# NVlabs/WarpConvNet

Hardware: AMD Instinct MI355X
Metric: M active voxels/sec fwd+bwd, SparseConv3d 64→128 k=3, 1/2/4/8 MI355X (higher is better)
Workload: dtype bf16; 1 GPU; configs[1]: one 1000000-voxel uniform (U) scene per GPU, SparseConv3d 64->128 k=3, bf16 autocast, kernel-map build + AB fwd + ABt dgrad + AtB wgrad per step; voxels_per_gpu=1000000, coord_order=generator, parallelism=dp1 (scene-sharded, grad all-reduce)

## Files before the change

### include/wcn.h

```cpp
#ifndef WCN_H_
#define WCN_H_

#include <stddef.h>
#include <stdint.h>

#ifdef __cplusplus
extern "C" {
#endif

typedef void* wcn_stream_t;

enum wcn_status {
  WCN_SUCCESS = 0,
  WCN_ERROR_PROBLEM_NOT_SUPPORTED = -1,
  WCN_ERROR_KERNEL_INITIALIZATION = -2,
  WCN_ERROR_KERNEL_EXECUTION = -3,
  WCN_ERROR_UNSUPPORTED_CONFIG = -4,
  WCN_ERROR_INVALID_PARAMETERS = -5,
  WCN_ERROR_MIXED_INPUT_UNSUPPORTED = -6
};

enum wcn_dtype { WCN_F32 = 0, WCN_F16 = 1, WCN_BF16 = 2 };

enum wcn_kmap_flag {
  WCN_FLAG_TABLE_FULL = 1,
  WCN_FLAG_COORD_RANGE = 2,
  WCN_FLAG_PAIR_OVERFLOW = 4,
  WCN_FLAG_DUPLICATE_COORD = 8,
  WCN_FLAG_NEED_STRICT = 16,
  WCN_FLAG_ROW_OVERFLOW = 32
};

int wcn_abi_version(void);
const char* wcn_status_string(int status);

int wcn_hash_prepare(void* slots, int64_t capacity, wcn_stream_t stream);
int wcn_hash_insert(void* slots, int64_t capacity, const int32_t* coords, int64_t n, int32_t* status,
                    wcn_stream_t stream);
int wcn_hash_search(const void* slots, int64_t capacity, const int32_t* queries, int64_t m,
                    int32_t* results, wcn_stream_t stream);

int32_t wcn_kmap_row_pitch(int32_t num_offsets);
int32_t wcn_kmap_mask_words(int32_t num_offsets);
int64_t wcn_kmap_num_blocks(int64_t m);
size_t wcn_kmap_counts_bytes(int64_t m, int32_t num_offsets);

int wcn_kmap_probe(const void* slots, int64_t capacity, const int32_t* query, int64_t m,
                   const int32_t ksize[3], const int32_t stride[3], const int32_t dilation[3],
                   int32_t* nbr, uint32_t* mask, wcn_stream_t stream);
int wcn_batch_indexed_coords(const int32_t* coords, int64_t n, int32_t num_dims, const int32_t* offsets,
                             int32_t num_batches, int32_t* out, wcn_stream_t stream);

int wcn_morton_code(const int32_t* coords, int64_t n, int32_t num_dims, const int32_t* origin, const int32_t axis[3],
                    int64_t* codes, wcn_stream_t stream);

size_t wcn_kmap_binned_workspace(int64_t n, int64_t max_blocks);
int wcn_kmap_binned_supported(const int32_t ksize[3], const int32_t dilation[3]);
int wcn_kmap_compact_supported(int32_t num_offsets);
int wcn_kmap_build_binned(const int32_t* coords, int64_t n, const int32_t ksize[3], const int32_t dilation[3],
                          int64_t max_blocks, int32_t strict, int32_t compact, void* workspace, size_t workspace_bytes,
                          int32_t* nbr, uint32_t* mask, int32_t* status, wcn_stream_t stream);
int wcn_kmap_densify(const int32_t* nbr_compact, int64_t m, int32_t num_offsets, int32_t* nbr, wcn_stream_t stream);
size_t wcn_kmap_tally_sort_workspace(int64_t m);
int wcn_kmap_tally_sort(uint32_t* mask, int32_t* nbr, int64_t m, int32_t num_offsets, int32_t* counts, int32_t* offsets,
                        int32_t* status, int32_t* host_mirror, int32_t* perm, void* sort_workspace,
                        size_t sort_workspace_bytes, const int32_t* coords, void* binned_workspace, int64_t binned_n,
                        int64_t max_blocks, int32_t compact, int32_t* in_maps, int32_t* out_maps, int64_t pair_capacity,
                        wcn_stream_t stream);
int wcn_kmap_count(const uint32_t* mask, int64_t m, int32_t num_offsets, int32_t* counts, wcn_stream_t stream);
int wcn_kmap_scan(int32_t* counts, int64_t num_blocks, int32_t num_offsets, int32_t* offsets,
                  wcn_stream_t stream);
int wcn_kmap_scan_to_host(int32_t* counts, int64_t num_blocks, int32_t num_offsets, int32_t* offsets, const int32_t* status,
                          int32_t* host_mirror, wcn_stream_t stream);
int wcn_kmap_scatter(const int32_t* nbr, const uint32_t* mask, int64_t m, int32_t num_offsets,
                     const int32_t* counts, const int32_t* offsets, int32_t* in_maps, int32_t* out_maps, int64_t pair_capacity,
                     int32_t* status, int32_t compact, wcn_stream_t stream);
int wcn_kmap_cells_build(const int32_t* coords, int64_t n, int64_t max_blocks, void* workspace, size_t workspace_bytes,
                         uint32_t* scratch, int32_t* status, wcn_stream_t stream);
int wcn_cells_stride_supported(const int32_t stride[3]);
int64_t wcn_cells_stride_tiles(int64_t n);
int wcn_cells_stride_count(const void* cells_workspace, int64_t n, int64_t max_blocks, const int32_t* coords,
                           const int32_t stride[3], uint64_t* flags, int32_t* counts, int32_t num_batches,
                           int32_t* out_offsets, wcn_stream_t stream);
int wcn_cells_stride_emit(const void* cells_workspace, int64_t n, int64_t max_blocks, const int32_t* coords,
                          const int32_t stride[3], const uint64_t* flags, const int32_t* counts, int32_t* out_coords,
                          int32_t* first_rows, int32_t* nbr, uint32_t* mask, wcn_stream_t stream);
int wcn_kmap_probe_cells(const void* cells_workspace, int64_t n_in, int64_t max_blocks, const int32_t* query, int64_t m,
                         const int32_t ksize[3], const int32_t stride[3], const int32_t dilation[3], int32_t* nbr,
                         uint32_t* mask, wcn_stream_t stream);
int wcn_kmap_transpose(const int32_t* nbr, int64_t m, int32_t num_offsets, int32_t* pair_table,
                       wcn_stream_t stream);
int wcn_kmap_reverse(const int32_t* in_maps, const int32_t* out_maps, const int32_t* offsets,
                     int32_t num_offsets, int64_t max_pairs, int64_t n_in, int32_t* rev_nbr,
                     uint32_t* rev_mask, wcn_stream_t stream);
int wcn_kmap_from_csr(const int32_t* in_maps, const int32_t* out_maps, const int32_t* offsets,
                      int32_t num_offsets, int64_t max_pairs, int64_t n_out, int32_t* nbr, uint32_t* mask,
                      wcn_stream_t stream);
size_t wcn_mask_argsort_workspace(int64_t n);
int wcn_mask_argsort(const uint32_t* mask, int32_t mask_words, int32_t num_bits, int64_t n, int32_t* perm,
                     void* workspace, size_t workspace_bytes, wcn_stream_t stream);
int wcn_mask_tile_order(const uint32_t* mask, int32_t mask_words, int32_t num_offsets, int64_t n, int32_t* perm,
                        void* workspace, size_t workspace_bytes, wcn_stream_t stream);

enum wcn_algo { WCN_ALGO_AUTO = 0, WCN_ALGO_REF = 1, WCN_ALGO_MFMA = 2 };

int wcn_mfma_gather_supported(int32_t cin, int32_t cout, int32_t num_offsets, int32_t dtype);
int wcn_mfma_wgrad_supported(int32_t cin, int32_t cout, int32_t dtype);
int wcn_conv_identity_supported(int32_t cin, int32_t cout, int32_t dtype);
int wcn_dense_rows_supported(int32_t cin, int32_t cout, int32_t dtype);
int wcn_dense_rows(const void* x, int32_t x_is_f32, const void* w, int32_t w_is_f32, int32_t w_transposed, const float* bias,
                   void* y, int64_t n, int32_t cin, int32_t cout, int32_t dtype, wcn_stream_t stream);

size_t wcn_packed_weight_bytes(int32_t num_offsets, int32_t cin, int32_t cout, int32_t dtype, int32_t transpose);
int wcn_pack_weight(const void* w, int32_t num_offsets, int32_t cin, int32_t cout, int32_t dtype,
                    int32_t transpose, int32_t flip, void* packed, size_t packed_bytes, wcn_stream_t stream);
int wcn_pack_weight_f32(const float* w, int32_t num_offsets, int32_t cin, int32_t cout, int32_t dtype, int32_t transpose,
                        int32_t flip, void* packed, size_t packed_bytes, wcn_stream_t stream);
int wcn_pack_weight_pair_supported(int32_t num_offsets, int32_t cin, int32_t cout, int32_t dtype);
int wcn_pack_weight_f32_pair(const float* w, int32_t num_offsets, int32_t cin, int32_t cout, int32_t dtype, int32_t flip_dgrad,
                             void* packed_fwd, size_t packed_fwd_bytes, void* packed_dgrad, size_t packed_dgrad_bytes,
                             wcn_stream_t stream);

int wcn_conv_compact_table_supported(int32_t cin, int32_t cout, int32_t num_offsets, int32_t dtype);
int wcn_conv_gather_gemm(const void* in, const void* w, void* out, const int32_t* nbr,
                         const uint32_t* mask, const int32_t* perm, const float* bias, int64_t n_in,
                         int64_t n_out, int32_t cin, int32_t cout, int32_t num_offsets, int32_t dtype,
                         int32_t algo, int32_t w_transposed, int32_t k_flip, wcn_stream_t stream);

int wcn_mfma_grouped_supported(int32_t cin_g, int32_t cout_g, int32_t num_offsets, int32_t dtype);
int wcn_pack_weight_grouped(const void* w, int32_t w_is_f32, int32_t num_offsets, int32_t groups, int32_t cin_g,
                            int32_t cout_g, int32_t dtype, int32_t transpose, int32_t flip, void* packed, wcn_stream_t stream);
int wcn_conv_gather_gemm_grouped(const void* in, const void* w_packed, void* out, const int32_t* nbr, const uint32_t* mask,
                                 const int32_t* perm, const float* bias, int64_t n_in, int64_t n_out, int32_t cin_g,
                                 int32_t cout_g, int32_t groups, int32_t num_offsets, int32_t dtype, wcn_stream_t stream);
int wcn_conv_gather_gemm_f32out(const void* in, const void* w_packed, float* out, const int32_t* nbr,
                                const uint32_t* mask, const int32_t* perm, const float* bias, int64_t n_in,
                                int64_t n_out, int32_t cin, int32_t cout, int32_t num_offsets, int32_t dtype,
                                wcn_stream_t stream);

int wcn_conv_gather_gemm_fused(const void* in, const void* w_packed, void* out, const int32_t* nbr, const uint32_t* mask,
                               const int32_t* perm, const float* bias, const float* scale, const float* shift,
                               const void* residual, int32_t relu, int64_t n_in, int64_t n_out, int32_t cin, int32_t cout,
                               int32_t num_offsets, int32_t dtype, wcn_stream_t stream);

size_t wcn_colsum_workspace(int32_t channels);
int wcn_colsum(const void* in, int64_t n, int32_t channels, int32_t dtype, float* out, void* workspace,
               size_t workspace_bytes, wcn_stream_t stream);

size_t wcn_conv_wgrad_workspace(int32_t num_offsets, int32_t cin, int32_t cout, int32_t algo);
int wcn_conv_wgrad(const void* x, const void* dy, float* dw, const int32_t* in_maps,
                   const int32_t* out_maps, const int32_t* offsets, int64_t n_in, int64_t n_out,
                   int32_t cin, int32_t cout, int32_t num_offsets, int32_t dtype, int32_t algo,
                   void* workspace, size_t workspace_bytes, wcn_stream_t stream);

int wcn_mfma_wgrad_bias_supported(int32_t cin, int32_t cout, int32_t dtype);
int wcn_conv_wgrad_bias(const void* x, const void* dy, float* dw, const int32_t* in_maps, const int32_t* out_maps,
                        const int32_t* offsets, int64_t n_in, int64_t n_out, int32_t cin, int32_t cout,
                        int32_t num_offsets, int32_t dtype, int32_t self_offset, float* bias_grad, void* workspace,
                        size_t workspace_bytes, wcn_stream_t stream);

int wcn_dwconv_gather(const void* in, const void* w, void* out, const int32_t* nbr, const float* bias, int64_t n_in,
                      int64_t n_out, int32_t channels, int32_t num_offsets, int32_t dtype, int32_t k_flip,
                      wcn_stream_t stream);
size_t wcn_dwconv_wgrad_workspace(int32_t num_offsets, int32_t channels);
int wcn_dwconv_wgrad(const void* x, const void* dy, float* dw, const int32_t* in_maps, const int32_t* out_maps,
                     const int32_t* offsets, int64_t n_in, int64_t n_out, int32_t channels, int32_t num_offsets,
                     int32_t dtype, void* workspace, size_t workspace_bytes, wcn_stream_t stream);

int wcn_knn_grid(const float* ref_sorted, const int32_t* ref_ids, const int32_t* cell_start, const float origin[3],
                 float cell_size, const int32_t dims[3], const float* query, int64_t num_query, int32_t k,
                 int64_t* out_index, float* out_dist2, wcn_stream_t stream);
int wcn_radius_grid_count(const float* ref_sorted, const int32_t* ref_ids, const int32_t* cell_start, const float origin[3],
                          float cell_size, const int32_t dims[3], const float* query, int64_t num_query, float radius,
                          int32_t* counts, wcn_stream_t stream);
int wcn_radius_grid_write(const float* ref_sorted, const int32_t* ref_ids, const int32_t* cell_start, const float origin[3],
                          float cell_size, const int32_t dims[3], const float* query, int64_t num_query, float radius,
                          const int64_t* splits, int32_t* out_index, float* out_dist, wcn_stream_t stream);
int wcn_segment_reduce(const void* in, const int64_t* row_splits, int64_t num_segments, int32_t channels, int32_t dtype,
                       int32_t op, void* out, int64_t* arg_rows, wcn_stream_t stream);

int wcn_pointconv_supported(int32_t cin, int32_t cq, int32_t nrel, int32_t hidden, int32_t cout, int32_t k,
                            int32_t linear_shortcut);
int64_t wcn_pointconv_packed_floats(int32_t ein, int32_t hidden, int32_t cout);
int64_t wcn_pointconv_grad_floats(int32_t ein, int32_t hidden, int32_t cout, int32_t linear_shortcut);
size_t wcn_pointconv_backward_workspace(int64_t n_query, int32_t k, int32_t ein, int32_t hidden, int32_t cout,
                                        int32_t linear_shortcut);
int wcn_pointconv_pack(const float* w1, const float* b1, const float* g1, const float* be1, const float* w2,
                       const float* b2, const float* g2, const float* be2, const float* ws, const float* bs, int32_t ein,
                       int32_t hidden, int32_t cout, float* packed, wcn_stream_t stream);
int wcn_pointconv_edge_forward(const float* in_feats, const float* q_feats, const float* in_xyz, const float* q_xyz,
                               const int32_t* nbr, int64_t n_query, int32_t k, int32_t cin, int32_t cq, int32_t nrel,
                               const float* packed, int32_t hidden, int32_t cout, float eps1, float eps2, int32_t mean,
                               int32_t linear_shortcut, float* out, wcn_stream_t stream);
int wcn_pointconv_edge_backward(const float* in_feats, const float* q_feats, const float* in_xyz, const float* q_xyz,
                                const int32_t* nbr, int64_t n_query, int32_t k, int32_t cin, int32_t cq, int32_t nrel,
                                const float* packed, int32_t hidden, int32_t cout, float eps1, float eps2, int32_t mean,
                                int32_t linear_shortcut, const float* grad_out, float* d_in, float* d_q, float* d_params,
                                void* workspace, size_t workspace_bytes, wcn_stream_t stream);
int wcn_pointconv_edge_backward_peredge(const float* in_feats, const float* q_feats, const float* in_xyz, const float* q_xyz,
                                        const int32_t* nbr, int64_t n_query, int32_t k, int32_t cin, int32_t cq, int32_t nrel,
                                        const float* packed, int32_t hidden, int32_t cout, float eps1, float eps2, int32_t mean,
                                        int32_t linear_shortcut, const float* grad_out, float* d_edge, float* d_q,
                                        float* d_params, void* workspace, size_t workspace_bytes, wcn_stream_t stream);

int wcn_pointconv_edge_forward_ragged(const float* in_feats, const float* q_feats, const float* in_xyz, const float* q_xyz,
                                      const int32_t* nbr, const int32_t* edge_q, const float* q_scale, int64_t n_edges,
                                      int64_t n_query, int32_t cin, int32_t cq, int32_t nrel, const float* packed,
                                      int32_t hidden, int32_t cout, float eps1, float eps2, int32_t linear_shortcut,
                                      float* out, wcn_stream_t stream);
int wcn_pointconv_edge_backward_ragged(const float* in_feats, const float* q_feats, const float* in_xyz, const float* q_xyz,
                                       const int32_t* nbr, const int32_t* edge_q, const float* q_scale, int64_t n_edges,
                                       int64_t n_query, int32_t cin, int32_t cq, int32_t nrel, const float* packed,
                                       int32_t hidden, int32_t cout, float eps1, float eps2, int32_t linear_shortcut,
                                       const float* grad_out, float* d_in, float* d_q, float* d_params, void* workspace,
                                       size_t workspace_bytes, wcn_stream_t stream);

int wcn_pool_gather(const void* in, const int32_t* tbl, int64_t n_in, int64_t n_out, int32_t channels, int32_t num_offsets,
                    int32_t dtype, int32_t op, void* out, int32_t* arg, int32_t* count, wcn_stream_t stream);
int wcn_pool_select(const void* dy, const int32_t* arg, const int32_t* tbl, int64_t n_in, int64_t n_out, int32_t channels,
                    int32_t num_offsets, int32_t dtype, void* dx, wcn_stream_t stream);

size_t wcn_bn_workspace(int32_t channels);
int wcn_bn_stats_fold(const void* x, int64_t n, int32_t channels, int32_t dtype, const float* gamma, const float* beta,
                      float* running_mean, float* running_var, float momentum, float eps, float* mean, float* var,
                      float* rstd, float* scale, float* shift, int64_t* num_batches_tracked, void* workspace,
                      size_t workspace_bytes, wcn_stream_t stream);
int wcn_bn_fold(const float* running_mean, const float* running_var, const float* gamma, const float* beta, float eps,
                int32_t channels, float* mean, float* rstd, float* scale, float* shift, wcn_stream_t stream);
int wcn_bn_stats(const void* x, int64_t n, int32_t channels, int32_t dtype, float* mean, float* var, void* workspace,
                 size_t workspace_bytes, wcn_stream_t stream);
int wcn_bn_apply(const void* x, int64_t n, int32_t channels, int32_t dtype, const float* scale, const float* shift,
                 int32_t relu, void* y, wcn_stream_t stream);
int wcn_bn_backward_reduce(const void* dy, const void* x, const float* relu_scale, const float* relu_shift, int64_t n,
                           int32_t channels, int32_t dtype, const float* mean, const float* rstd, float* sum_dy,
                           float* sum_dy_xhat, void* workspace, size_t workspace_bytes, wcn_stream_t stream);
int wcn_bn_backward_apply(const void* dy, const void* x, const float* relu_scale, const float* relu_shift, int64_t n,
                          int32_t channels, int32_t dtype, const float* mean, const float* rstd, const float* gamma,
                          const float* sum_dy, const float* sum_dy_xhat, void* dx, wcn_stream_t stream);
int wcn_bn_apply_residual(const void* x, const void* residual, int64_t n, int32_t channels, int32_t dtype, const float* scale,
                          const float* shift, int32_t relu, void* y, wcn_stream_t stream);
int wcn_bn_backward_reduce_masked(const void* dy, const void* x, const void* z, int64_t n, int32_t channels, int32_t dtype,
                                  const float* mean, const float* rstd, float* sum_dy, float* sum_dy_xhat, void* workspace,
                                  size_t workspace_bytes, wcn_stream_t stream);
int wcn_bn_backward_apply_masked(const void* dy, const void* x, const void* z, int64_t n, int32_t channels, int32_t dtype,
                                 const float* mean, const float* rstd, const float* gamma, const float* sum_dy,
                                 const float* sum_dy_xhat, void* dx, void* dres, wcn_stream_t stream);

int wcn_bn_train_forward(const void* x, const void* residual, int64_t n, int32_t channels, int32_t dtype, const float* gamma,
                         const float* beta, float* running_mean, float* running_var, float momentum, float eps,
                         int64_t* num_batches_tracked, int32_t relu, float* stats, void* y, void* workspace,
                         size_t workspace_bytes, wcn_stream_t stream);
int wcn_bn_train_backward(const void* dy, const void* x, const void* z, int32_t relu, int64_t n, int32_t channels, int32_t dtype,
                          const float* stats, const float* gamma, int32_t training, float* sums, void* dx, void* dres,
                          void* workspace, size_t workspace_bytes, wcn_stream_t stream);
int wcn_bn_train_backward_ld(const void* dy, int64_t dy_ld, const void* x, const void* z, int32_t relu, int64_t n, int32_t channels,
                             int32_t dtype, const float* stats, const float* gamma, int32_t training, float* sums, void* dx,
                             void* dres, void* workspace, size_t workspace_bytes, wcn_stream_t stream);

int wcn_conv_bn_backward(const void* grad_out, const void* x, const void* y, const void* z, int32_t relu, const float* stats,
                         const float* gamma, int32_t training, float* sums, void* dy_conv, void* dres, const void* w_packed_dgrad,
                         const int32_t* rev_nbr, const uint32_t* rev_mask, const int32_t* rev_perm, int32_t flip, void* dx,
                         const int32_t* in_maps, const int32_t* out_maps, const int32_t* offsets, float* dw, void* wgrad_workspace,
                         size_t wgrad_workspace_bytes, int64_t n_in, int64_t n_out, int32_t cin, int32_t cout, int32_t num_offsets,
                         int32_t dtype, void* bn_workspace, size_t bn_workspace_bytes, wcn_stream_t stream);
int wcn_conv_bn_backward_ld(const void* grad_out, int64_t grad_out_ld, const void* x, const void* y, const void* z, int32_t relu,
                            const float* stats, const float* gamma, int32_t training, float* sums, void* dy_conv, void* dres,
                            const void* w_packed_dgrad, const int32_t* rev_nbr, const uint32_t* rev_mask, const int32_t* rev_perm,
                            int32_t flip, void* dx, const int32_t* in_maps, const int32_t* out_maps, const int32_t* offsets,
                            float* dw, void* wgrad_workspace, size_t wgrad_workspace_bytes, int64_t n_in, int64_t n_out,
                            int32_t cin, int32_t cout, int32_t num_offsets, int32_t dtype, void* bn_workspace,
                            size_t bn_workspace_bytes, wcn_stream_t stream);

int wcn_attn_varlen_supported(int32_t head_dim, int32_t dtype);
size_t wcn_attn_varlen_workspace_bytes(int64_t total, int32_t heads);
int wcn_attn_varlen_fwd(const void* qkv, const int32_t* cu_seqlens, int64_t num_seqs, int64_t total, int32_t heads,
                        int32_t head_dim, int32_t max_seqlen, float softmax_scale, int32_t dtype, void* out, float* lse,
                        wcn_stream_t stream);
int wcn_attn_varlen_bwd(const void* dout, const void* qkv, const void* out, const float* lse, const int32_t* cu_seqlens,
                        int64_t num_seqs, int64_t total, int32_t heads, int32_t head_dim, int32_t max_seqlen,
                        float softmax_scale, int32_t dtype, void* dqkv, void* workspace, size_t workspace_bytes,
                        wcn_stream_t stream);

int32_t wcn_attn_varlen_kv_splits(int64_t num_seqs, int32_t max_seqlen_q, int32_t max_seqlen_k, int32_t heads);
size_t wcn_attn_varlen_kv_workspace_bytes(int64_t total_q, int64_t total_k, int32_t heads, int32_t head_dim, int32_t q_splits);
int wcn_attn_varlen_kv_fwd(const void* q, int64_t q_stride, const void* k, const void* v, int64_t kv_stride,
                           const int32_t* cu_q, const int32_t* cu_k, int64_t num_seqs, int64_t total_q, int64_t total_k,
                           int32_t heads, int32_t head_dim, int32_t max_seqlen_q, int32_t max_seqlen_k, float softmax_scale,
                           int32_t dtype, void* out, float* lse, wcn_stream_t stream);
int wcn_attn_varlen_kv_bwd(const void* dout, const void* q, int64_t q_stride, const void* k, const void* v, int64_t kv_stride,
                           const void* out, const float* lse, const int32_t* cu_q, const int32_t* cu_k, int64_t num_seqs,
                           int64_t total_q, int64_t total_k, int32_t heads, int32_t head_dim, int32_t max_seqlen_q,
                           int32_t max_seqlen_k, float softmax_scale, int32_t dtype, void* dq, int64_t dq_stride, void* dk,
                           void* dv, int64_t dkv_stride, int32_t q_splits, void* workspace, size_t workspace_bytes,
                           wcn_stream_t stream);

enum wcn_slot_order { WCN_SLOT_X_FASTEST = 0, WCN_SLOT_Z_FASTEST = 1 };
int wcn_resample_pack(const void* src, const int32_t* tbl, int64_t n_src, int64_t n_parent, int32_t channels, int32_t n_per,
                      int32_t factor, int32_t pitch, int32_t slot_order, int32_t dtype, void* dst, wcn_stream_t stream);
int wcn_resample_unpack(const void* src, const int32_t* tbl, int64_t n_parent, int64_t n_dst, int32_t channels, int32_t n_per,
                        int32_t factor, int32_t pitch, int32_t slot_order, int32_t broadcast, int32_t dtype, void* dst,
                        wcn_stream_t stream);
size_t wcn_resample_expand_workspace(int64_t n_parent);
int wcn_resample_expand(const int32_t* parents, const void* mask, int32_t mask_dtype, int64_t n_parent, int32_t n_per,
                        int32_t factor, int32_t slot_order, int32_t num_batches, void* workspace, size_t workspace_bytes,
                        int32_t* out_offsets, int64_t capacity, int32_t* child_coords, int32_t* tbl, int32_t pitch,
                        wcn_stream_t stream);

int wcn_rope_table(const void* coords, int32_t coords_float, int64_t total, const float* origin, float bias,
                   const float* freqs, int32_t num_freqs, float* table, wcn_stream_t stream);
int wcn_qk_prologue_supported(int32_t head_dim, int32_t in_dtype, int32_t out_dtype);
size_t wcn_qk_prologue_workspace_bytes(int64_t total, int32_t heads, int32_t head_dim);
int wcn_qk_prologue_fwd(const void* qkv, int32_t in_dtype, int64_t total, int32_t heads, int32_t head_dim, const float* table,
                        int32_t rot_pairs, int32_t conjugate, const float* gamma_q, const float* gamma_k, void* out,
                        int32_t out_dtype, float* inv_norm, wcn_stream_t stream);
int wcn_qk_prologue_bwd(const void* dout, int32_t dout_dtype, const void* qkv, int32_t in_dtype, int64_t total, int32_t heads,
                        int32_t head_dim, const float* table, int32_t rot_pairs, const float* gamma_q, const float* gamma_k,
                        const float* inv_norm, void* dqkv, float* dgamma_q, float* dgamma_k, void* workspace,
                        size_t workspace_bytes, wcn_stream_t stream);

int wcn_adaln_supported(int32_t channels, int32_t dtype);
size_t wcn_adaln_workspace_bytes(int64_t rows, int64_t num_segs, int32_t channels);
int wcn_adaln_fwd(const void* x, const void* h, const float* gate, const float* shift, const float* scale, int64_t mod_ld,
                  const int32_t* cu, int64_t num_segs, int64_t rows, int32_t channels, float eps, int32_t dtype, void* x1,
                  void* y, float* stats, wcn_stream_t stream);
int wcn_adaln_bwd(const void* dx1, const void* dy, const void* x, const void* h, const float* gate, const float* scale,
                  int64_t mod_ld, const float* stats, const int32_t* cu, int64_t num_segs, int64_t rows, int32_t channels,
                  int32_t dtype, void* dx, void* dh, float* dgate, float* dshift, float* dscale, int64_t dmod_ld,
                  void* workspace, size_t workspace_bytes, wcn_stream_t stream);

int wcn_ln_act_supported(int32_t channels, int32_t dtype);
size_t wcn_ln_act_workspace_bytes(int64_t rows, int32_t channels);
int wcn_ln_act_fwd(const void* x, const float* weight, const float* bias, int64_t rows, int32_t channels, float eps,
                   int32_t act, int32_t dtype, void* y, float* stats, wcn_stream_t stream);
int wcn_ln_act_bwd(const void* dy, const void* x, const float* weight, const float* bias, const float* stats, int64_t rows,
                   int32_t channels, int32_t act, int32_t dtype, void* dx, float* dweight, float* dbias, void* workspace,
                   size_t workspace_bytes, wcn_stream_t stream);
int wcn_channel_spread(const void* x, const void* h, int64_t rows, int32_t cx, int32_t r, float alpha, int32_t dtype,
                       void* out, wcn_stream_t stream);
int wcn_channel_fold(const void* x, const void* h, int64_t rows, int32_t cout, int32_t g, float alpha, int32_t dtype,
                     void* out, wcn_stream_t stream);

int32_t wcn_window_group_max_segment(void);
size_t wcn_window_group_workspace_bytes(int64_t n, int64_t num_bins);
int wcn_window_group(const int32_t* coords, int64_t n, const int32_t* batch_offsets, int32_t num_batches,
                     const int32_t window[3], const int32_t shift[3], const int32_t min_coord[3], const int32_t grid_shape[3],
                     int64_t* codes, int64_t* perm, int64_t* inverse_perm, int32_t* cu_seqlens, int64_t* counts,
                     int32_t* summary, void* workspace, size_t workspace_bytes, wcn_stream_t stream);

int32_t wcn_csr_chunk_rows(void);
int wcn_voxel_keys(const float* points, int64_t n, const int32_t* batch_offsets, int32_t num_batches, float inv_voxel_size,
                   int64_t* keys, int32_t* status, wcn_stream_t stream);
size_t wcn_voxel_map_workspace_bytes(int64_t n);
int wcn_voxel_map(const int64_t* sorted_keys, const int64_t* perm, int64_t n, int32_t num_batches, int64_t* unique_keys,
                  int32_t* unique_coords, int64_t* csr_offsets, int64_t* to_orig, int64_t* to_unique,
                  int32_t* batch_voxel_offsets, int32_t* summary, void* workspace, size_t workspace_bytes,
                  wcn_stream_t stream);
size_t wcn_csr_gather_reduce_workspace_bytes(int64_t nnz, int32_t c, int32_t op);
int wcn_csr_gather_reduce(const void* in, int64_t ld_in, int64_t n_in, const int64_t* indices, const int64_t* offsets,
                          int64_t m, int64_t nnz, int32_t c, int32_t dtype, int32_t op, int64_t max_segment, void* out,
                          int64_t* arg, void* workspace, size_t workspace_bytes, wcn_stream_t stream);
int wcn_row_spread(const void* src, const int64_t* to_orig, int64_t n, int64_t m, int32_t c, const void* skip, int32_t cs,
                   int64_t ld_out, int32_t mode, const int64_t* offsets, const int64_t* arg, int32_t dtype, void* out,
                   wcn_stream_t stream);

int32_t wcn_lattice_chunk_rows(void);
int wcn_hash128_insert(int64_t* table_keys, int32_t* table_values, int64_t capacity, const int32_t* coords, int64_t n,
                       int32_t key_dim, int32_t* status, wcn_stream_t stream);
int wcn_hash128_search(const int64_t* table_keys, const int32_t* table_values, int64_t capacity, const int32_t* queries,
                       const int32_t* offsets, int64_t m, int32_t k, int32_t key_dim, int32_t* out, wcn_stream_t stream);
int wcn_permuto_simplex(const float* positions, int64_t n, int32_t d, const float* scale, int64_t* key_hi, int64_t* key_lo,
                        int32_t* keys, float* bary, int32_t* status, wcn_stream_t stream);
int wcn_grid_corners(const float* positions, int64_t n, int32_t d, int64_t* floors, int64_t* key_hi, int64_t* key_lo,
                     int32_t* keys, float* weights, int32_t* status, wcn_stream_t stream);
size_t wcn_lattice_map_workspace_bytes(int64_t nnz);
int wcn_lattice_map(const int64_t* sorted_hi, const int64_t* sorted_lo, const int64_t* perm, int64_t nnz, int32_t key_dim,
                    int32_t* unique_keys, int64_t* inverse, int64_t* row_offsets, int32_t* summary, void* workspace,
                    size_t workspace_bytes, wcn_stream_t stream);
int64_t wcn_lattice_plan_items(int64_t nnz);
int64_t wcn_lattice_plan_ints(int64_t nnz);
int wcn_lattice_plan(const int64_t* row_offsets, int64_t v, int64_t nnz, int32_t* plan, wcn_stream_t stream);
int wcn_lattice_splat(const float* f, const float* w, const int64_t* row_offsets, const int64_t* row_entries, int64_t v,
                      int64_t nnz, int32_t k, int32_t pitch, float alpha, const int32_t* plan, float* partials, float* out,
                      wcn_stream_t stream);
int wcn_lattice_blur(const float* x, const int32_t* n1, const int32_t* n2, float s0, float s1, float s2, int64_t v,
                     int32_t pitch, float* y, wcn_stream_t stream);
int wcn_lattice_slice(const float* x, const int64_t* idx, const float* w, int64_t n, int32_t k, int64_t v, int32_t pitch,
                      float alpha, float* out, wcn_stream_t stream);

int32_t wcn_lattice_max_grid(void);
int32_t wcn_lattice_row_grid(int64_t rows, int32_t pitch);
int wcn_bilateral_matvec(const int32_t* neighbours, int32_t d, int64_t v, int32_t pitch, float tap_a, float tap_b, float tap_c,
                         const float* nvec, const float* dc, float lam, const float* p, float* spare, float* ap,
                         double* partials, wcn_stream_t stream);
int wcn_bilateral_pcg(const int32_t* neighbours, int32_t d, int64_t v, int32_t pitch, float tap_a, float tap_b, float tap_c,
                      const float* nvec, const float* dc, const float* minv, float lam, const float* tbar, float* y, float* work,
                      double* partials, double* state, int32_t max_iters, double tol, wcn_stream_t stream);
int wcn_bilateral_knn_weights(const float* src_xyz, const float* src_feat, const float* query_xyz, const float* query_feat,
                              const int64_t* nbr, int64_t n, int64_t m, int32_t k, int32_t dx, int32_t df, float sigma_xyz,
                              float sigma_feat, float* weights, wcn_stream_t stream);

#ifdef __cplusplus
}
#endif
#endif
```

### warpconvnet_amd/_lib.py

```python
import ctypes
import os
import subprocess
import threading
from ctypes import c_char_p, c_int, c_int32, c_int64, c_size_t, c_void_p
from typing import Optional

import torch

_CSRC = os.path.join(os.path.dirname(os.path.abspath(__file__)), "csrc")
LIB_PATH = os.environ.get("WARPCONVNET_AMD_LIB") or os.path.join(_CSRC, "libwcn_hip.so")

WCN_F32, WCN_F16, WCN_BF16 = 0, 1, 2
WCN_ALGO_AUTO, WCN_ALGO_REF, WCN_ALGO_MFMA = 0, 1, 2
WCN_FLAG_TABLE_FULL, WCN_FLAG_COORD_RANGE, WCN_FLAG_PAIR_OVERFLOW, WCN_FLAG_DUPLICATE_COORD = 1, 2, 4, 8
WCN_FLAG_NEED_STRICT = 16
WCN_FLAG_ROW_OVERFLOW = 32
WCN_SLOT_X_FASTEST, WCN_SLOT_Z_FASTEST = 0, 1
WCN_MASK_U8 = 3

_I32P = c_void_p
_3I = c_int32 * 3

SIGNATURES = {
    "wcn_abi_version": (c_int, []),
    "wcn_status_string": (c_char_p, [c_int]),
    "wcn_hash_prepare": (c_int, [c_void_p, c_int64, c_void_p]),
    "wcn_hash_insert": (c_int, [c_void_p, c_int64, c_void_p, c_int64, c_void_p, c_void_p]),
    "wcn_hash_search": (c_int, [c_void_p, c_int64, c_void_p, c_int64, c_void_p, c_void_p]),
    "wcn_kmap_row_pitch": (c_int32, [c_int32]),
    "wcn_kmap_mask_words": (c_int32, [c_int32]),
    "wcn_kmap_num_blocks": (c_int64, [c_int64]),
    "wcn_kmap_probe": (
        c_int,
        [c_void_p, c_int64, c_void_p, c_int64, _3I, _3I, _3I, c_void_p, c_void_p, c_void_p],
    ),
    "wcn_batch_indexed_coords": (c_int, [c_void_p, c_int64, c_int32, c_void_p, c_int32, c_void_p, c_void_p]),
    "wcn_bn_workspace": (c_size_t, [c_int32]),
    "wcn_bn_stats": (c_int, [c_void_p, c_int64, c_int32, c_int32, c_void_p, c_void_p, c_void_p, c_size_t, c_void_p]),
    "wcn_bn_stats_fold": (c_int, [c_void_p, c_int64, c_int32, c_int32, c_void_p, c_void_p, c_void_p, c_void_p, ctypes.c_float,
                                  ctypes.c_float, c_void_p, c_void_p, c_void_p, c_void_p, c_void_p, c_void_p, c_void_p, c_size_t,
                                  c_void_p]),
    "wcn_bn_fold": (c_int, [c_void_p, c_void_p, c_void_p, c_void_p, ctypes.c_float, c_int32, c_void_p, c_void_p, c_void_p,
                            c_void_p, c_void_p]),
    "wcn_bn_apply": (c_int, [c_void_p, c_int64, c_int32, c_int32, c_void_p, c_void_p, c_int32, c_void_p, c_void_p]),
    "wcn_bn_backward_reduce": (c_int, [c_void_p, c_void_p, c_void_p, c_void_p, c_int64, c_int32, c_int32, c_void_p, c_void_p,
                                       c_void_p, c_void_p, c_void_p, c_size_t, c_void_p]),
    "wcn_bn_backward_apply": (c_int, [c_void_p, c_void_p, c_void_p, c_void_p, c_int64, c_int32, c_int32, c_void_p, c_void_p,
                                      c_void_p, c_void_p, c_void_p, c_void_p, c_void_p]),
    "wcn_bn_apply_residual": (c_int, [c_void_p, c_void_p, c_int64, c_int32, c_int32, c_void_p, c_void_p, c_int32, c_void_p,
                                      c_void_p]),
    "wcn_bn_backward_reduce_masked": (c_int, [c_void_p, c_void_p, c_void_p, c_int64, c_int32, c_int32, c_void_p, c_void_p,
                                              c_void_p, c_void_p, c_void_p, c_size_t, c_void_p]),
    "wcn_bn_backward_apply_masked": (c_int, [c_void_p, c_void_p, c_void_p, c_int64, c_int32, c_int32, c_void_p, c_void_p,
                                             c_void_p, c_void_p, c_void_p, c_void_p, c_void_p, c_void_p]),
    "wcn_bn_train_forward": (c_int, [c_void_p, c_void_p, c_int64, c_int32, c_int32, c_void_p, c_void_p, c_void_p, c_void_p,
                                     ctypes.c_float, ctypes.c_float, c_void_p, c_int32, c_void_p, c_void_p, c_void_p, c_size_t,
                                     c_void_p]),
    "wcn_bn_train_backward": (c_int, [c_void_p, c_void_p, c_void_p, c_int32, c_int64, c_int32, c_int32, c_void_p, c_void_p,
                                      c_int32, c_void_p, c_void_p, c_void_p, c_void_p, c_size_t, c_void_p]),
    "wcn_bn_train_backward_ld": (c_int, [c_void_p, c_int64, c_void_p, c_void_p, c_int32, c_int64, c_int32, c_int32, c_void_p, c_void_p,
                                         c_int32, c_void_p, c_void_p, c_void_p, c_void_p, c_size_t, c_void_p]),
    "wcn_conv_bn_backward_ld": (c_int, [c_void_p, c_int64, c_void_p, c_void_p, c_void_p, c_int32, c_void_p, c_void_p, c_int32, c_void_p,
                                        c_void_p, c_void_p, c_void_p, c_void_p, c_void_p, c_void_p, c_int32, c_void_p, c_void_p, c_void_p,
                                        c_void_p, c_void_p, c_void_p, c_size_t, c_int64, c_int64, c_int32, c_int32, c_int32, c_int32,
                                        c_void_p, c_size_t, c_void_p]),
    "wcn_conv_bn_backward": (c_int, [c_void_p, c_void_p, c_void_p, c_void_p, c_int32, c_void_p, c_void_p, c_int32, c_void_p, c_void_p,
                                     c_void_p, c_void_p, c_void_p, c_void_p, c_void_p, c_int32, c_void_p, c_void_p, c_void_p, c_void_p,
                                     c_void_p, c_void_p, c_size_t, c_int64, c_int64, c_int32, c_int32, c_int32, c_int32, c_void_p,
                                     c_size_t, c_void_p]),
    "wcn_pool_gather": (c_int, [c_void_p, c_void_p, c_int64, c_int64, c_int32, c_int32, c_int32, c_int32, c_void_p, c_void_p,
                                c_void_p, c_void_p]),
    "wcn_pool_select": (c_int, [c_void_p, c_void_p, c_void_p, c_int64, c_int64, c_int32, c_int32, c_int32, c_void_p, c_void_p]),
    "wcn_morton_code": (c_int, [c_void_p, c_int64, c_int32, c_void_p, c_void_p, c_void_p, c_void_p]),
    "wcn_kmap_counts_bytes": (c_size_t, [c_int64, c_int32]),
    "wcn_kmap_binned_workspace": (c_size_t, [c_int64, c_int64]),
    "wcn_kmap_binned_supported": (c_int, [_3I, _3I]),
    "wcn_kmap_build_binned": (
        c_int,
        [c_void_p, c_int64, _3I, _3I, c_int64, c_int32, c_int32, c_void_p, c_size_t, c_void_p, c_void_p, c_void_p, c_void_p],
    ),
    "wcn_kmap_compact_supported": (c_int, [c_int32]),
    "wcn_kmap_densify": (c_int, [c_void_p, c_int64, c_int32, c_void_p, c_void_p]),
    "wcn_kmap_tally_sort_workspace": (c_size_t, [c_int64]),
    "wcn_kmap_tally_sort": (
        c_int,
        [c_void_p, c_void_p, c_int64, c_int32, c_void_p, c_void_p, c_void_p, c_void_p, c_void_p, c_void_p, c_size_t,
         c_void_p, c_void_p, c_int64, c_int64, c_int32, c_void_p, c_void_p, c_int64, c_void_p],
    ),
    "wcn_kmap_count": (c_int, [c_void_p, c_int64, c_int32, c_void_p, c_void_p]),
    "wcn_kmap_scan": (c_int, [c_void_p, c_int64, c_int32, c_void_p, c_void_p]),
    "wcn_kmap_scan_to_host": (c_int, [c_void_p, c_int64, c_int32, c_void_p, c_void_p, c_void_p, c_void_p]),
    "wcn_kmap_scatter": (
        c_int,
        [c_void_p, c_void_p, c_int64, c_int32, c_void_p, c_void_p, c_void_p, c_void_p, c_int64, c_void_p, c_int32, c_void_p],
    ),
    "wcn_kmap_cells_build": (c_int, [c_void_p, c_int64, c_int64, c_void_p, c_size_t, c_void_p, c_void_p, c_void_p]),
    "wcn_cells_stride_supported": (c_int, [_3I]),
    "wcn_cells_stride_tiles": (c_int64, [c_int64]),
    "wcn_cells_stride_count": (c_int, [c_void_p, c_int64, c_int64, c_void_p, _3I, c_void_p, c_void_p, c_int32, c_void_p,
                                       c_void_p]),
    "wcn_cells_stride_emit": (c_int, [c_void_p, c_int64, c_int64, c_void_p, _3I, c_void_p, c_void_p, c_void_p, c_void_p,
                                      c_void_p, c_void_p, c_void_p]),
    "wcn_kmap_probe_cells": (c_int, [c_void_p, c_int64, c_int64, c_void_p, c_int64, _3I, _3I, _3I, c_void_p, c_void_p,
                                     c_void_p]),
    "wcn_kmap_transpose": (c_int, [c_void_p, c_int64, c_int32, c_void_p, c_void_p]),
    "wcn_kmap_reverse": (
        c_int,
        [c_void_p, c_void_p, c_void_p, c_int32, c_int64, c_int64, c_void_p, c_void_p, c_void_p],
    ),
    "wcn_kmap_from_csr": (
        c_int,
        [c_void_p, c_void_p, c_void_p, c_int32, c_int64, c_int64, c_void_p, c_void_p, c_void_p],
    ),
    "wcn_mask_argsort_workspace": (c_size_t, [c_int64]),
    "wcn_mask_argsort": (c_int, [c_void_p, c_int32, c_int32, c_int64, c_void_p, c_void_p, c_size_t, c_void_p]),
    "wcn_mask_tile_order": (c_int, [c_void_p, c_int32, c_int32, c_int64, c_void_p, c_void_p, c_size_t, c_void_p]),
    "wcn_mfma_gather_supported": (c_int, [c_int32, c_int32, c_int32, c_int32]),
    "wcn_mfma_wgrad_supported": (c_int, [c_int32, c_int32, c_int32]),
    "wcn_conv_identity_supported": (c_int, [c_int32, c_int32, c_int32]),
    "wcn_dense_rows_supported": (c_int, [c_int32, c_int32, c_int32]),
    "wcn_dense_rows": (
        c_int,
        [c_void_p, c_int32, c_void_p, c_int32, c_int32, c_void_p, c_void_p, c_int64, c_int32, c_int32, c_int32, c_void_p],
    ),
    "wcn_packed_weight_bytes": (c_size_t, [c_int32, c_int32, c_int32, c_int32, c_int32]),
    "wcn_pack_weight": (
        c_int,
        [c_void_p, c_int32, c_int32, c_int32, c_int32, c_int32, c_int32, c_void_p, c_size_t, c_void_p],
    ),
    "wcn_pack_weight_f32": (
        c_int,
        [c_void_p, c_int32, c_int32, c_int32, c_int32, c_int32, c_int32, c_void_p, c_size_t, c_void_p],
    ),
    "wcn_pack_weight_pair_supported": (c_int, [c_int32, c_int32, c_int32, c_int32]),
    "wcn_conv_compact_table_supported": (c_int, [c_int32, c_int32, c_int32, c_int32]),
    "wcn_pack_weight_f32_pair": (c_int, [c_void_p, c_int32, c_int32, c_int32, c_int32, c_int32, c_void_p, c_size_t, c_void_p, c_size_t,
                                         c_void_p]),
    "wcn_conv_gather_gemm": (
        c_int,
        [c_void_p, c_void_p, c_void_p, c_void_p, c_void_p, c_void_p, c_void_p, c_int64, c_int64, c_int32, c_int32,
         c_int32, c_int32, c_int32, c_int32, c_int32, c_void_p],
    ),
    "wcn_mfma_grouped_supported": (c_int, [c_int32, c_int32, c_int32, c_int32]),
    "wcn_pack_weight_grouped": (
        c_int,
        [c_void_p, c_int32, c_int32, c_int32, c_int32, c_int32, c_int32, c_int32, c_int32, c_void_p, c_void_p],
    ),
    "wcn_conv_gather_gemm_grouped": (
        c_int,
        [c_void_p, c_void_p, c_void_p, c_void_p, c_void_p, c_void_p, c_void_p, c_int64, c_int64, c_int32, c_int32,
         c_int32, c_int32, c_int32, c_void_p],
    ),
    "wcn_conv_gather_gemm_f32out": (
        c_int,
        [c_void_p, c_void_p, c_void_p, c_void_p, c_void_p, c_void_p, c_void_p, c_int64, c_int64, c_int32, c_int32,
         c_int32, c_int32, c_void_p],
    ),
    "wcn_conv_gather_gemm_fused": (
        c_int,
        [c_void_p, c_void_p, c_void_p, c_void_p, c_void_p, c_void_p, c_void_p, c_void_p, c_void_p, c_void_p, c_int32,
         c_int64, c_int64, c_int32, c_int32, c_int32, c_int32, c_void_p],
    ),
    "wcn_colsum_workspace": (c_size_t, [c_int32]),
    "wcn_colsum": (c_int, [c_void_p, c_int64, c_int32, c_int32, c_void_p, c_void_p, c_size_t, c_void_p]),
    "wcn_conv_wgrad_workspace": (c_size_t, [c_int32, c_int32, c_int32, c_int32]),
    "wcn_conv_wgrad": (
        c_int,
        [c_void_p, c_void_p, c_void_p, c_void_p, c_void_p, c_void_p, c_int64, c_int64, c_int32, c_int32, c_int32,
         c_int32, c_int32, c_void_p, c_size_t, c_void_p],
    ),
    "wcn_dwconv_gather": (
        c_int,
        [c_void_p, c_void_p, c_void_p, c_void_p, c_void_p, c_int64, c_int64, c_int32, c_int32, c_int32, c_int32, c_void_p],
    ),
    "wcn_dwconv_wgrad_workspace": (c_size_t, [c_int32, c_int32]),
    "wcn_dwconv_wgrad": (
        c_int,
        [c_void_p, c_void_p, c_void_p, c_void_p, c_void_p, c_void_p, c_int64, c_int64, c_int32, c_int32, c_int32,
         c_void_p, c_size_t, c_void_p],
    ),
    "wcn_radius_grid_count": (
        c_int,
        [c_void_p, c_void_p, c_void_p, ctypes.c_float * 3, ctypes.c_float, c_int32 * 3, c_void_p, c_int64, ctypes.c_float,
         c_void_p, c_void_p],
    ),
    "wcn_radius_grid_write": (
        c_int,
        [c_void_p, c_void_p, c_void_p, ctypes.c_float * 3, ctypes.c_float, c_int32 * 3, c_void_p, c_int64, ctypes.c_float,
         c_void_p, c_void_p, c_void_p, c_void_p],
    ),
    "wcn_knn_grid": (
        c_int,
        [c_void_p, c_void_p, c_void_p, ctypes.c_float * 3, ctypes.c_float, c_int32 * 3, c_void_p, c_int64, c_int32, c_void_p,
         c_void_p, c_void_p],
    ),
    "wcn_segment_reduce": (c_int, [c_void_p, c_void_p, c_int64, c_int32, c_int32, c_int32, c_void_p, c_void_p, c_void_p]),
    "wcn_pointconv_supported": (c_int, [c_int32] * 7),
    "wcn_pointconv_packed_floats": (c_int64, [c_int32] * 3),
    "wcn_pointconv_grad_floats": (c_int64, [c_int32] * 4),
    "wcn_pointconv_backward_workspace": (c_size_t, [c_int64, c_int32, c_int32, c_int32, c_int32, c_int32]),
    "wcn_pointconv_pack": (c_int, [c_void_p] * 10 + [c_int32] * 3 + [c_void_p, c_void_p]),
    "wcn_pointconv_edge_forward": (
        c_int,
        [c_void_p] * 5 + [c_int64] + [c_int32] * 4 + [c_void_p, c_int32, c_int32, ctypes.c_float, ctypes.c_float, c_int32,
                                                      c_int32, c_void_p, c_void_p],
    ),
    "wcn_pointconv_edge_backward": (
        c_int,
        [c_void_p] * 5 + [c_int64] + [c_int32] * 4 + [c_void_p, c_int32, c_int32, ctypes.c_float, ctypes.c_float, c_int32,
                                                      c_int32, c_void_p, c_void_p, c_void_p, c_void_p, c_void_p, c_size_t,
                                                      c_void_p],
    ),
    "wcn_pointconv_edge_backward_peredge": (
        c_int,
        [c_void_p] * 5 + [c_int64] + [c_int32] * 4 + [c_void_p, c_int32, c_int32, ctypes.c_float, ctypes.c_float, c_int32,
                                                      c_int32, c_void_p, c_void_p, c_void_p, c_void_p, c_void_p, c_size_t,
                                                      c_void_p],
    ),
    "wcn_pointconv_edge_forward_ragged": (
        c_int,
        [c_void_p] * 7 + [c_int64, c_int64] + [c_int32] * 3 + [c_void_p, c_int32, c_int32, ctypes.c_float, ctypes.c_float,
                                                               c_int32, c_void_p, c_void_p],
    ),
    "wcn_pointconv_edge_backward_ragged": (
        c_int,
        [c_void_p] * 7 + [c_int64, c_int64] + [c_int32] * 3 + [c_void_p, c_int32, c_int32, ctypes.c_float, ctypes.c_float,
                                                               c_int32, c_void_p, c_void_p, c_void_p, c_void_p, c_void_p,
                                                               c_size_t, c_void_p],
    ),
    "wcn_attn_varlen_supported": (c_int, [c_int32, c_int32]),
    "wcn_attn_varlen_workspace_bytes": (c_size_t, [c_int64, c_int32]),
    "wcn_attn_varlen_fwd": (
        c_int,
        [c_void_p, c_void_p, c_int64, c_int64, c_int32, c_int32, c_int32, ctypes.c_float, c_int32, c_void_p, c_void_p,
         c_void_p],
    ),
    "wcn_attn_varlen_bwd": (
        c_int,
        [c_void_p, c_void_p, c_void_p, c_void_p, c_void_p, c_int64, c_int64, c_int32, c_int32, c_int32, ctypes.c_float,
         c_int32, c_void_p, c_void_p, c_size_t, c_void_p],
    ),
    "wcn_attn_varlen_kv_splits": (c_int32, [c_int64, c_int32, c_int32, c_int32]),
    "wcn_attn_varlen_kv_workspace_bytes": (c_size_t, [c_int64, c_int64, c_int32, c_int32, c_int32]),
    "wcn_attn_varlen_kv_fwd": (
        c_int,
        [c_void_p, c_int64, c_void_p, c_void_p, c_int64, c_void_p, c_void_p, c_int64, c_int64, c_int64, c_int32, c_int32,
         c_int32, c_int32, ctypes.c_float, c_int32, c_void_p, c_void_p, c_void_p],
    ),
    "wcn_attn_varlen_kv_bwd": (
        c_int,
        [c_void_p, c_void_p, c_int64, c_void_p, c_void_p, c_int64, c_void_p, c_void_p, c_void_p, c_void_p, c_int64, c_int64,
         c_int64, c_int32, c_int32, c_int32, c_int32, ctypes.c_float, c_int32, c_void_p, c_int64, c_void_p, c_void_p, c_int64,
         c_int32, c_void_p, c_size_t, c_void_p],
    ),
    "wcn_rope_table": (c_int, [c_void_p, c_int32, c_int64, c_void_p, ctypes.c_float, c_void_p, c_int32, c_void_p, c_void_p]),
    "wcn_qk_prologue_supported": (c_int, [c_int32, c_int32, c_int32]),
    "wcn_qk_prologue_workspace_bytes": (c_size_t, [c_int64, c_int32, c_int32]),
    "wcn_qk_prologue_fwd": (
        c_int,
        [c_void_p, c_int32, c_int64, c_int32, c_int32, c_void_p, c_int32, c_int32, c_void_p, c_void_p, c_void_p, c_int32,
         c_void_p, c_void_p],
    ),
    "wcn_qk_prologue_bwd": (
        c_int,
        [c_void_p, c_int32, c_void_p, c_int32, c_int64, c_int32, c_int32, c_void_p, c_int32, c_void_p, c_void_p, c_void_p,
         c_void_p, c_void_p, c_void_p, c_void_p, c_size_t, c_void_p],
    ),
    "wcn_adaln_supported": (c_int, [c_int32, c_int32]),
    "wcn_adaln_workspace_bytes": (c_size_t, [c_int64, c_int64, c_int32]),
    "wcn_adaln_fwd": (
        c_int,
        [c_void_p] * 5 + [c_int64, c_void_p, c_int64, c_int64, c_int32, ctypes.c_float, c_int32, c_void_p, c_void_p, c_void_p,
                          c_void_p],
    ),
    "wcn_adaln_bwd": (
        c_int,
        [c_void_p] * 6 + [c_int64, c_void_p, c_void_p, c_int64, c_int64, c_int32, c_int32] + [c_void_p] * 5 +
        [c_int64, c_void_p, c_size_t, c_void_p],
    ),
    "wcn_ln_act_supported": (c_int, [c_int32, c_int32]),
    "wcn_ln_act_workspace_bytes": (c_size_t, [c_int64, c_int32]),
    "wcn_ln_act_fwd": (c_int, [c_void_p] * 3 + [c_int64, c_int32, ctypes.c_float, c_int32, c_int32, c_void_p, c_void_p,
                                                 c_void_p]),
    "wcn_ln_act_bwd": (c_int, [c_void_p] * 5 + [c_int64, c_int32, c_int32, c_int32] + [c_void_p] * 4 + [c_size_t, c_void_p]),
    "wcn_channel_spread": (c_int, [c_void_p, c_void_p, c_int64, c_int32, c_int32, ctypes.c_float, c_int32, c_void_p,
                                   c_void_p]),
    "wcn_channel_fold": (c_int, [c_void_p, c_void_p, c_int64, c_int32, c_int32, ctypes.c_float, c_int32, c_void_p, c_void_p]),
    "wcn_window_group_max_segment": (c_int32, []),
    "wcn_window_group_workspace_bytes": (c_size_t, [c_int64, c_int64]),
    "wcn_window_group": (c_int, [c_void_p, c_int64, c_void_p, c_int32, _3I, _3I, _3I, _3I] + [c_void_p] * 7 +
                         [c_size_t, c_void_p]),
    "wcn_csr_chunk_rows": (c_int32, []),
    "wcn_voxel_keys": (c_int, [c_void_p, c_int64, c_void_p, c_int32, ctypes.c_float, c_void_p, c_void_p, c_void_p]),
    "wcn_voxel_map_workspace_bytes": (c_size_t, [c_int64]),
    "wcn_voxel_map": (c_int, [c_void_p, c_void_p, c_int64, c_int32] + [c_void_p] * 7 + [c_void_p, c_size_t, c_void_p]),
    "wcn_csr_gather_reduce_workspace_bytes": (c_size_t, [c_int64, c_int32, c_int32]),
    "wcn_csr_gather_reduce": (
        c_int,
        [c_void_p, c_int64, c_int64, c_void_p, c_void_p, c_int64, c_int64, c_int32, c_int32, c_int32, c_int64, c_void_p,
         c_void_p, c_void_p, c_size_t, c_void_p],
    ),
    "wcn_row_spread": (c_int, [c_void_p, c_void_p, c_int64, c_int64, c_int32, c_void_p, c_int32, c_int64, c_int32, c_void_p,
                               c_void_p, c_int32, c_void_p, c_void_p]),
    "wcn_resample_pack": (c_int, [c_void_p, c_void_p, c_int64, c_int64, c_int32, c_int32, c_int32, c_int32, c_int32, c_int32,
                                  c_void_p, c_void_p]),
    "wcn_resample_unpack": (c_int, [c_void_p, c_void_p, c_int64, c_int64, c_int32, c_int32, c_int32, c_int32, c_int32, c_int32,
                                    c_int32, c_void_p, c_void_p]),
    "wcn_resample_expand_workspace": (c_size_t, [c_int64]),
    "wcn_resample_expand": (c_int, [c_void_p, c_void_p, c_int32, c_int64, c_int32, c_int32, c_int32, c_int32, c_void_p, c_size_t,
                                    c_void_p, c_int64, c_void_p, c_void_p, c_int32, c_void_p]),
    "wcn_mfma_wgrad_bias_supported": (c_int, [c_int32, c_int32, c_int32]),
    "wcn_conv_wgrad_bias": (
        c_int,
        [c_void_p, c_void_p, c_void_p, c_void_p, c_void_p, c_void_p, c_int64, c_int64, c_int32, c_int32, c_int32,
         c_int32, c_int32, c_void_p, c_void_p, c_size_t, c_void_p],
    ),
    "wcn_lattice_chunk_rows": (c_int32, []),
    "wcn_hash128_insert": (c_int, [c_void_p, c_void_p, c_int64, c_void_p, c_int64, c_int32, c_void_p, c_void_p]),
    "wcn_hash128_search": (c_int, [c_void_p, c_void_p, c_int64, c_void_p, c_void_p, c_int64, c_int32, c_int32, c_void_p,
                                   c_void_p]),
    "wcn_permuto_simplex": (c_int, [c_void_p, c_int64, c_int32, ctypes.c_float * 6] + [c_void_p] * 6),
    "wcn_grid_corners": (c_int, [c_void_p, c_int64, c_int32] + [c_void_p] * 7),
    "wcn_lattice_map_workspace_bytes": (c_size_t, [c_int64]),
    "wcn_lattice_map": (c_int, [c_void_p, c_void_p, c_void_p, c_int64, c_int32] + [c_void_p] * 5 + [c_size_t, c_void_p]),
    "wcn_lattice_plan_items": (c_int64, [c_int64]),
    "wcn_lattice_plan_ints": (c_int64, [c_int64]),
    "wcn_lattice_plan": (c_int, [c_void_p, c_int64, c_int64, c_void_p, c_void_p]),
    "wcn_lattice_splat": (c_int, [c_void_p] * 4 + [c_int64, c_int64, c_int32, c_int32, ctypes.c_float] + [c_void_p] * 4),
    "wcn_lattice_blur": (c_int, [c_void_p] * 3 + [ctypes.c_float] * 3 + [c_int64, c_int32, c_void_p, c_void_p]),
    "wcn_lattice_slice": (c_int, [c_void_p] * 3 + [c_int64, c_int32, c_int64, c_int32, ctypes.c_float, c_void_p, c_void_p]),
    "wcn_lattice_max_grid": (c_int32, []),
    "wcn_lattice_row_grid": (c_int32, [c_int64, c_int32]),
    "wcn_bilateral_matvec": (c_int, [c_void_p, c_int32, c_int64, c_int32] + [ctypes.c_float] * 3 + [c_void_p, c_void_p,
                                                                                                   ctypes.c_float] + [c_void_p] * 5),
    "wcn_bilateral_pcg": (c_int, [c_void_p, c_int32, c_int64, c_int32] + [ctypes.c_float] * 3 + [c_void_p] * 3 + [ctypes.c_float] +
                          [c_void_p] * 5 + [c_int32, ctypes.c_double, c_void_p]),
    "wcn_bilateral_knn_weights": (c_int, [c_void_p] * 5 + [c_int64, c_int64, c_int32, c_int32, c_int32, ctypes.c_float,
                                                           ctypes.c_float, c_void_p, c_void_p]),
}

_LIB = None


class _GuardedLib:

    def __init__(self, handle: ctypes.CDLL):
        self._h = handle

    def __getattr__(self, name):
        fn = getattr(self._h, name)
        argtypes = fn.argtypes or []
        if not argtypes or argtypes[-1] is not c_void_p or name in _HOST_ONLY or _single_gpu():
            setattr(self, name, fn)
            return fn

        def guarded(*args, _fn=fn):
            dev = getattr(_CALL_DEVICE, "dev", None)
            if dev is None or dev == torch.cuda.current_device():
                return _fn(*args)
            with torch.cuda.device(dev):
                return _fn(*args)

        guarded.__name__ = name
        setattr(self, name, guarded)
        return guarded


def _single_gpu() -> bool:
    try:
        return torch.cuda.is_available() and torch.cuda.device_count() == 1
    except Exception:
        return False


_HOST_ONLY = {"wcn_status_string"}
_CALL_DEVICE = threading.local()


def build(verbose: bool = False) -> str:
    cmd = ["make", "-C", _CSRC, "-j", str(min(8, os.cpu_count() or 1))]
    res = subprocess.run(cmd, capture_output=True, text=True)
    if res.returncode != 0:
        raise RuntimeError(f"building libwcn_hip.so failed:\n{res.stdout[-4000:]}\n{res.stderr[-4000:]}")
    if verbose:
        print(res.stdout[-2000:])
    return LIB_PATH


def lib() -> ctypes.CDLL:
    global _LIB
    if _LIB is None:
        if not os.path.exists(LIB_PATH):
            raise RuntimeError(
                f"{LIB_PATH} not found: the HIP extension is not built. Run "
                "`python -c 'import __graft_entry__ as g; g.build()'` (or `make -C warpconvnet_amd/csrc`). "
                "There is no CPU fallback for the HIP paths."
            )
        handle = ctypes.CDLL(LIB_PATH)
        for name, (restype, argtypes) in SIGNATURES.items():
            fn = getattr(handle, name)
            fn.restype = restype
            fn.argtypes = argtypes
        _LIB = _GuardedLib(handle)
    return _LIB


def status_string(code: int) -> str:
    return lib().wcn_status_string(int(code)).decode()


def check(code: int, what: str) -> None:
    if code != 0:
        raise RuntimeError(f"{what} error: {status_string(code)} ({code})")


def ptr(t: Optional[torch.Tensor]) -> Optional[int]:
    if t is None:
        return None
    return t.data_ptr()


_RAW_STREAM = getattr(torch._C, "_cuda_getCurrentRawStream", None)


def stream_handle(device: torch.device) -> int:
    idx = device.index
    if idx is None:
        idx = torch.cuda.current_device()
    _CALL_DEVICE.dev = idx
    if _RAW_STREAM is not None:
        return _RAW_STREAM(idx)
    return torch.cuda.current_stream(device).cuda_stream


def dtype_code(dtype: torch.dtype) -> int:
    if dtype == torch.float32:
        return WCN_F32
    if dtype == torch.float16:
        return WCN_F16
    if dtype == torch.bfloat16:
        return WCN_BF16
    raise TypeError(f"unsupported feature dtype {dtype} (supported: float32, float16, bfloat16)")


def torch_dtype(code: int) -> torch.dtype:
    return {WCN_F32: torch.float32, WCN_F16: torch.float16, WCN_BF16: torch.bfloat16}[code]


def i3(v) -> "ctypes.Array":
    return _3I(int(v[0]), int(v[1]), int(v[2]))


def require_gpu_tensor(t: torch.Tensor, name: str) -> None:
    if not t.is_cuda:
        raise RuntimeError(f"{name} must live on a GPU for the HIP path (got {t.device}); there is no CPU fallback")
    if not t.is_contiguous():
        raise RuntimeError(f"{name} must be contiguous")
```

### warpconvnet_amd/csrc/kmap.hip

```cpp
#include "kmap_cells.h"

namespace wcn {

constexpr int kBlockRows = 256;
constexpr int kThreads = 256;

__global__ void hash_prepare_kernel(uint4* __restrict__ slots, int64_t capacity) {
  const int64_t i = (int64_t)blockIdx.x * blockDim.x + threadIdx.x;
  if (i < capacity) slots[i] = make_uint4(0u, 0u, 0xFFFFFFFFu, 0u);
}

__global__ void hash_insert_kernel(Slot* __restrict__ slots, uint32_t capacity_mask, const int4* __restrict__ coords,
                                   int64_t n, int32_t* __restrict__ status) {
  const int64_t i = (int64_t)blockIdx.x * blockDim.x + threadIdx.x;
  if (i >= n) return;
  const int4 c = coords[i];
  if (!coord_in_range(c.x, c.y, c.z, c.w)) {
    atomicOr(status, (int)WCN_FLAG_COORD_RANGE);
    return;
  }
  const uint64_t key = pack_key(c.x, c.y, c.z, c.w);
  uint32_t s = hash_slot(key, capacity_mask);
  for (uint32_t attempts = 0; attempts <= capacity_mask; ++attempts) {
    unsigned long long* kp = reinterpret_cast<unsigned long long*>(&slots[s].key);
    const unsigned long long prev = atomicCAS(kp, 0ull, (unsigned long long)key);
    if (prev == 0ull || prev == key) {
      atomicMin(reinterpret_cast<unsigned int*>(&slots[s].value), (unsigned int)i);
      if (prev == key) atomicOr(status, (int)WCN_FLAG_DUPLICATE_COORD);
      return;
    }
    s = (s + 1) & capacity_mask;
  }
  atomicOr(status, (int)WCN_FLAG_TABLE_FULL);
}

__global__ void hash_search_kernel(const Slot* __restrict__ slots, uint32_t capacity_mask,
                                   const int4* __restrict__ queries, int64_t m, int32_t* __restrict__ results) {
  const int64_t i = (int64_t)blockIdx.x * blockDim.x + threadIdx.x;
  if (i >= m) return;
  const int4 q = queries[i];
  results[i] = slot_lookup(slots, capacity_mask, pack_key(q.x, q.y, q.z, q.w));
}

struct HashLookup {
  const Slot* slots;
  uint32_t cmask;
  __device__ __forceinline__ int operator()(int b, int x, int y, int z) const {
    return slot_lookup(slots, cmask, pack_key(b, x, y, z));
  }
};

struct CellLookup {
  const BSlot* slots;
  uint32_t cmask;
  CellTable t;
  __device__ __forceinline__ int operator()(int b, int x, int y, int z) const {
    const int xx = (x << (32 - kCoordBits)) >> (32 - kCoordBits);
    const int yy = (y << (32 - kCoordBits)) >> (32 - kCoordBits);
    const int zz = (z << (32 - kCoordBits)) >> (32 - kCoordBits);
    const int id = block_id_of(slots, cmask, make_int4(b, xx, yy, zz));
    int found = -1;
    if (id >= 0)
      found = t.cells[(int64_t)id * kCells + (((xx & (kBlk - 1)) * kBlk + (yy & (kBlk - 1))) * kBlk + (zz & (kBlk - 1)))];
    return found;
  }
};

template <int LPR, typename Lookup>
__global__ __launch_bounds__(kThreads) void kmap_probe_kernel(Lookup lookup, const int4* __restrict__ query, int64_t m,
                                                              KernelGeom g, int K, int kp, int mw, int32_t* __restrict__ nbr,
                                                              uint32_t* __restrict__ mask) {
  const int tid = threadIdx.x;
  constexpr int kRowsPerIter = 64 / LPR;
  const int lane = tid & 63;
  const int wave = tid >> 6;
  const int sub = lane % LPR;
  const int rsel = lane / LPR;
  const int64_t wave_row0 = (int64_t)blockIdx.x * kBlockRows + wave * 64;
  const int num_chunks = (kp + LPR - 1) / LPR;

  for (int kc = 0; kc < num_chunks; ++kc) {
    const int k = kc * LPR + sub;
    const bool k_real = k < K;
    const bool k_store = k < kp;
    const int l = k % g.kz;
    const int j = (k / g.kz) % g.ky;
    const int i = k / (g.kz * g.ky);
    const int ox = (i - g.cx) * g.dx, oy = (j - g.cy) * g.dy, oz = (l - g.cz) * g.dz;
#pragma unroll 4
    for (int it = 0; it < 64 / kRowsPerIter; ++it) {
      const int64_t row = wave_row0 + it * kRowsPerIter + rsel;
      int found = -1;
      if (row < m && k_real) {
        const int4 q = query[row];
        found = lookup(q.x, q.y * g.sx + ox, q.z * g.sy + oy, q.w * g.sz + oz);
      }
      if (row < m && k_store) nbr[row * kp + k] = found;
      const unsigned long long ball = __ballot(found >= 0);
      if (row < m && sub == 0) {
        const unsigned long long bits = (LPR == 64) ? ball : ((ball >> (rsel * LPR)) & ((1ull << (LPR & 63)) - 1ull));
        const int w0 = (kc * LPR) >> 5;
        if (w0 < mw) mask[row * mw + w0] = (uint32_t)bits;
        if (LPR == 64 && w0 + 1 < mw) mask[row * mw + w0 + 1] = (uint32_t)(bits >> 32);
      }
    }
  }
}

template <typename Lookup>
static int launch_probe(const Lookup& lookup, const void* table, const int32_t* query, int64_t m, const int32_t ksize[3],
                        const int32_t stride[3], const int32_t dilation[3], int32_t* nbr, uint32_t* mask, hipStream_t s) {
  if (m < 0 || !ksize || !stride || !dilation) return WCN_ERROR_INVALID_PARAMETERS;
  for (int d = 0; d < 3; ++d)
    if (ksize[d] < 1 || stride[d] < 1 || dilation[d] < 1) return WCN_ERROR_INVALID_PARAMETERS;
  const int64_t K64 = (int64_t)ksize[0] * ksize[1] * ksize[2];
  if (!valid_k(K64)) return WCN_ERROR_PROBLEM_NOT_SUPPORTED;
  if (m == 0) return WCN_SUCCESS;
  if (!table || !query || !nbr || !mask) return WCN_ERROR_INVALID_PARAMETERS;
  const int K = (int)K64, kp = wcn_kmap_row_pitch(K), mw = wcn_kmap_mask_words(K);
  const KernelGeom g = make_kernel_geom(ksize, stride, dilation);
  const dim3 grid((unsigned)ceil_div(m, kBlockRows)), block(kThreads);
#define WCN_PROBE(L) \
  hipLaunchKernelGGL((kmap_probe_kernel<L, Lookup>), grid, block, 0, s, lookup, (const int4*)query, m, g, K, kp, mw, nbr, mask)
  switch (lanes_per_row(kp)) {
    case 8: WCN_PROBE(8); break;
    case 16: WCN_PROBE(16); break;
    case 32: WCN_PROBE(32); break;
    default: WCN_PROBE(64); break;
  }
#undef WCN_PROBE
  return launch_status();
}

__global__ __launch_bounds__(256) void batch_indexed_coords_kernel(const int32_t* __restrict__ coords, int64_t n, int d,
                                                                   const int32_t* __restrict__ offsets, int num_batches,
                                                                   int32_t* __restrict__ out) {
  const int64_t i = (int64_t)blockIdx.x * blockDim.x + threadIdx.x;
  if (i >= n) return;
  const int b = last_offset_not_above(offsets, num_batches, i);
  if (d == 3) {
    const int32_t* c = coords + i * 3;
    *reinterpret_cast<int4*>(out + i * 4) = make_int4(b, c[0], c[1], c[2]);
  } else {
    out[i * (d + 1)] = b;
    for (int j = 0; j < d; ++j) out[i * (d + 1) + 1 + j] = coords[i * d + j];
  }
}

__device__ __forceinline__ uint64_t spread3(uint64_t v) {
  v &= 0x1FFFFFull;
  v = (v | (v << 32)) & 0x001F00000000FFFFull;
  v = (v | (v << 16)) & 0x001F0000FF0000FFull;
  v = (v | (v << 8)) & 0x100F00F00F00F00Full;
  v = (v | (v << 4)) & 0x10C30C30C30C30C3ull;
  v = (v | (v << 2)) & 0x1249249249249249ull;
  return v;
}

__global__ __launch_bounds__(256) void morton_code_kernel(const int32_t* __restrict__ coords, int64_t n, int d,
                                                          const int32_t* __restrict__ origin, int a0, int a1, int a2,
                                                          int64_t* __restrict__ codes) {
  const int64_t i = (int64_t)blockIdx.x * blockDim.x + threadIdx.x;
  if (i >= n) return;
  const int32_t* c = coords + i * d;
  const int sp = d - 3;
  int64_t v[3];
  const int ax[3] = {a0, a1, a2};
#pragma unroll
  for (int j = 0; j < 3; ++j) v[j] = (int64_t)c[sp + ax[j]] - (origin ? (int64_t)origin[sp + ax[j]] : 0);
  uint64_t m = spread3((uint64_t)v[0]) | (spread3((uint64_t)v[1]) << 1) | (spread3((uint64_t)v[2]) << 2);
  if (d == 4) {
    const int64_t b = (int64_t)c[0] - (origin ? (int64_t)origin[0] : 0);
    m = (m & 0x0000FFFFFFFFFFFFull) | ((uint64_t)b << 48);
  }
  codes[i] = (int64_t)m;
}

__global__ __launch_bounds__(kThreads) void kmap_transpose_kernel(const int32_t* __restrict__ nbr, int64_t m, int K,
                                                                  int kp, int tr, int32_t* __restrict__ pair_table) {
  extern __shared__ int s_tile[];
  const int64_t row0 = (int64_t)blockIdx.x * tr;
  const int pitch = kp + 1;
  for (int e = threadIdx.x; e < tr * kp; e += kThreads) {
    const int r = e / kp, k = e % kp;
    s_tile[r * pitch + k] = (row0 + r < m) ? nbr[(row0 + r) * kp + k] : -1;
  }
  __syncthreads();
  for (int e = threadIdx.x; e < tr * K; e += kThreads) {
    const int k = e / tr, r = e % tr;
    if (row0 + r < m) pair_table[(int64_t)k * m + row0 + r] = s_tile[r * pitch + k];
  }
}

__global__ void fill_i32_kernel(int32_t* __restrict__ p, int64_t n, int32_t v) {
  const int64_t i = (int64_t)blockIdx.x * blockDim.x + threadIdx.x;
  if (i < n) p[i] = v;
}

__global__ void kmap_pairs_to_table_kernel(const int32_t* __restrict__ in_maps, const int32_t* __restrict__ out_maps,
                                           const int32_t* __restrict__ offsets, int K, int kp, int mw, int64_t max_pairs,
                                           int by_in, int32_t* __restrict__ tbl, uint32_t* __restrict__ mask) {
  const int64_t p = (int64_t)blockIdx.x * blockDim.x + threadIdx.x;
  if (p >= max_pairs || p >= offsets[K]) return;
  const int k = last_offset_not_above(offsets, K, p);
  const int i = in_maps[p], o = out_maps[p];
  const int64_t row = by_in ? i : o;
  tbl[row * kp + k] = by_in ? o : i;
  atomicOr(&mask[row * mw + (k >> 5)], 1u << (k & 31));
}

}

using namespace wcn;

extern "C" {

int wcn_abi_version(void) { return 14; }

const char* wcn_status_string(int status) {
  switch (status) {
    case WCN_SUCCESS: return "Success";
    case WCN_ERROR_PROBLEM_NOT_SUPPORTED: return "Problem size not supported";
    case WCN_ERROR_KERNEL_INITIALIZATION: return "Kernel initialization failed";
    case WCN_ERROR_KERNEL_EXECUTION: return "Kernel execution failed";
    case WCN_ERROR_UNSUPPORTED_CONFIG: return "Unsupported precision/configuration";
    case WCN_ERROR_INVALID_PARAMETERS: return "Invalid parameters";
    case WCN_ERROR_MIXED_INPUT_UNSUPPORTED: return "Mixed input precision unsupported";
    default: return "Unknown error";
  }
}

static inline bool is_pow2(int64_t v) { return v > 0 && (v & (v - 1)) == 0; }

int wcn_hash_prepare(void* slots, int64_t capacity, wcn_stream_t stream) {
  if (!slots || !is_pow2(capacity) || capacity > (1ll << 31)) return WCN_ERROR_INVALID_PARAMETERS;
  hipLaunchKernelGGL(hash_prepare_kernel, dim3((unsigned)ceil_div(capacity, 256)), dim3(256), 0, (hipStream_t)stream,
                     (uint4*)slots, capacity);
  return launch_status();
}

int wcn_hash_insert(void* slots, int64_t capacity, const int32_t* coords, int64_t n, int32_t* status,
                    wcn_stream_t stream) {
  if (!slots || !is_pow2(capacity) || capacity > (1ll << 31) || n < 0 || !status) return WCN_ERROR_INVALID_PARAMETERS;
  if (n == 0) return WCN_SUCCESS;
  if (!coords) return WCN_ERROR_INVALID_PARAMETERS;
  hipLaunchKernelGGL(hash_insert_kernel, dim3((unsigned)ceil_div(n, 256)), dim3(256), 0, (hipStream_t)stream,
                     (Slot*)slots, (uint32_t)(capacity - 1), (const int4*)coords, n, status);
  return launch_status();
}

int wcn_hash_search(const void* slots, int64_t capacity, const int32_t* queries, int64_t m, int32_t* results,
                    wcn_stream_t stream) {
  if (!slots || !is_pow2(capacity) || m < 0) return WCN_ERROR_INVALID_PARAMETERS;
  if (m == 0) return WCN_SUCCESS;
  if (!queries || !results) return WCN_ERROR_INVALID_PARAMETERS;
  hipLaunchKernelGGL(hash_search_kernel, dim3((unsigned)ceil_div(m, 256)), dim3(256), 0, (hipStream_t)stream,
                     (const Slot*)slots, (uint32_t)(capacity - 1), (const int4*)queries, m, results);
  return launch_status();
}

int32_t wcn_kmap_row_pitch(int32_t num_offsets) { return (num_offsets + 7) & ~7; }
int32_t wcn_kmap_mask_words(int32_t num_offsets) { return (num_offsets + 31) / 32; }
int wcn_kmap_probe(const void* slots, int64_t capacity, const int32_t* query, int64_t m, const int32_t ksize[3],
                   const int32_t stride[3], const int32_t dilation[3], int32_t* nbr, uint32_t* mask,
                   wcn_stream_t stream) {
  if (!slots || !is_pow2(capacity)) return WCN_ERROR_INVALID_PARAMETERS;
  return launch_probe(HashLookup{(const Slot*)slots, (uint32_t)(capacity - 1)}, slots, query, m, ksize, stride, dilation, nbr,
                      mask, (hipStream_t)stream);
}

int wcn_kmap_probe_cells(const void* cells_workspace, int64_t n_in, int64_t max_blocks, const int32_t* query, int64_t m,
                         const int32_t ksize[3], const int32_t stride[3], const int32_t dilation[3], int32_t* nbr,
                         uint32_t* mask, wcn_stream_t stream) {
  if (n_in < 0 || max_blocks < 1) return WCN_ERROR_INVALID_PARAMETERS;
  const CellTable t = carve_cells(const_cast<void*>(cells_workspace), n_in, max_blocks);
  return launch_probe(CellLookup{t.slots, (uint32_t)(t.capacity - 1), t}, cells_workspace, query, m, ksize, stride, dilation,
                      nbr, mask, (hipStream_t)stream);
}

int wcn_batch_indexed_coords(const int32_t* coords, int64_t n, int32_t num_dims, const int32_t* offsets,
                             int32_t num_batches, int32_t* out, wcn_stream_t stream) {
  if (n < 0 || num_dims < 1 || num_dims > 8 || num_batches < 1) return WCN_ERROR_INVALID_PARAMETERS;
  if (n == 0) return WCN_SUCCESS;
  if (!coords || !out || (num_batches > 1 && !offsets)) return WCN_ERROR_INVALID_PARAMETERS;
  hipLaunchKernelGGL(batch_indexed_coords_kernel, dim3((unsigned)ceil_div(n, 256)), dim3(256), 0, (hipStream_t)stream, coords,
                     n, (int)num_dims, offsets, (int)num_batches, out);
  return launch_status();
}

int wcn_morton_code(const int32_t* coords, int64_t n, int32_t num_dims, const int32_t* origin, const int32_t axis[3],
                    int64_t* codes, wcn_stream_t stream) {
  if (n < 0 || (num_dims != 3 && num_dims != 4) || !axis) return WCN_ERROR_INVALID_PARAMETERS;
  int seen = 0;
  for (int j = 0; j < 3; ++j) {
    if (axis[j] < 0 || axis[j] > 2) return WCN_ERROR_INVALID_PARAMETERS;
    seen |= 1 << axis[j];
  }
  if (seen != 7) return WCN_ERROR_INVALID_PARAMETERS;
  if (n == 0) return WCN_SUCCESS;
  if (!coords || !codes) return WCN_ERROR_INVALID_PARAMETERS;
  hipLaunchKernelGGL(morton_code_kernel, dim3((unsigned)ceil_div(n, 256)), dim3(256), 0, (hipStream_t)stream, coords, n,
                     (int)num_dims, origin, (int)axis[0], (int)axis[1], (int)axis[2], codes);
  return launch_status();
}

int wcn_kmap_transpose(const int32_t* nbr, int64_t m, int32_t num_offsets, int32_t* pair_table, wcn_stream_t stream) {
  if (m < 0 || !valid_k(num_offsets)) return WCN_ERROR_INVALID_PARAMETERS;
  if (m == 0) return WCN_SUCCESS;
  if (!nbr || !pair_table) return WCN_ERROR_INVALID_PARAMETERS;
  const int kp = wcn_kmap_row_pitch(num_offsets);
  int tr = 64;
  while (tr > 1 && (size_t)tr * (kp + 1) * sizeof(int) > 64 * 1024) tr >>= 1;
  hipLaunchKernelGGL(kmap_transpose_kernel, dim3((unsigned)ceil_div(m, tr)), dim3(kThreads),
                     (size_t)tr * (kp + 1) * sizeof(int), (hipStream_t)stream, nbr, m, (int)num_offsets, kp, tr, pair_table);
  return launch_status();
}

static int pairs_to_table(const int32_t* in_maps, const int32_t* out_maps, const int32_t* offsets, int32_t K,
                          int64_t max_pairs, int64_t rows, int by_in, int32_t* tbl, uint32_t* mask, hipStream_t s) {
  if (!valid_k(K) || rows < 0 || max_pairs < 0 || !offsets) return WCN_ERROR_INVALID_PARAMETERS;
  if (rows == 0) return WCN_SUCCESS;
  if (!tbl || !mask) return WCN_ERROR_INVALID_PARAMETERS;
  const int kp = wcn_kmap_row_pitch(K), mw = wcn_kmap_mask_words(K);
  hipLaunchKernelGGL(fill_i32_kernel, dim3((unsigned)ceil_div(rows * kp, 256)), dim3(256), 0, s, tbl, rows * kp, -1);
  hipLaunchKernelGGL(fill_i32_kernel, dim3((unsigned)ceil_div(rows * mw, 256)), dim3(256), 0, s, (int32_t*)mask,
                     rows * mw, 0);
  if (max_pairs > 0) {
    if (!in_maps || !out_maps) return WCN_ERROR_INVALID_PARAMETERS;
    hipLaunchKernelGGL(kmap_pairs_to_table_kernel, dim3((unsigned)ceil_div(max_pairs, 256)), dim3(256), 0, s, in_maps,
                       out_maps, offsets, (int)K, kp, mw, max_pairs, by_in, tbl, mask);
  }
  return launch_status();
}

int wcn_kmap_reverse(const int32_t* in_maps, const int32_t* out_maps, const int32_t* offsets, int32_t num_offsets,
                     int64_t max_pairs, int64_t n_in, int32_t* rev_nbr, uint32_t* rev_mask, wcn_stream_t stream) {
  return pairs_to_table(in_maps, out_maps, offsets, num_offsets, max_pairs, n_in, 1, rev_nbr, rev_mask,
                        (hipStream_t)stream);
}

int wcn_kmap_from_csr(const int32_t* in_maps, const int32_t* out_maps, const int32_t* offsets, int32_t num_offsets,
                      int64_t max_pairs, int64_t n_out, int32_t* nbr, uint32_t* mask, wcn_stream_t stream) {
  return pairs_to_table(in_maps, out_maps, offsets, num_offsets, max_pairs, n_out, 0, nbr, mask, (hipStream_t)stream);
}

}
```

### warpconvnet_amd/csrc/kmap_binned.hip

```cpp
#include "kmap_cells.h"

namespace wcn {

constexpr int kInsertSample = 8;
constexpr int kInsertThreads = 512;
constexpr int kRowBufPitch = 66;
constexpr int kRowBufInts = (kCompactPitch + 1) * kRowBufPitch;
#ifndef WCN_NB_WPE
#define WCN_NB_WPE 3
#endif
constexpr int kNbWavesPerSimd = WCN_NB_WPE;
constexpr int kNbThreads = 256;

__device__ __forceinline__ int wrap_blk(int v) {
  const int bits = kBlkCoordBits;
  v &= (1 << bits) - 1;
  return (v ^ (1 << (bits - 1))) - (1 << (bits - 1));
}

__global__ void cell_prepare_kernel(uint4* __restrict__ slots, int64_t capacity, int32_t* __restrict__ ctr,
                                    uint32_t* __restrict__ halo, CellGeom g, int32_t* __restrict__ status) {
  const int64_t i = (int64_t)blockIdx.x * blockDim.x + threadIdx.x;
  if (i < capacity) slots[i] = make_uint4(0u, 0u, 0xFFFFFFFFu, 0u);
  if (i < 64) ctr[i] = 0;
  if (i == 0) *status = 0;
  if (i < g.halo_cells) {
    const int h3[3] = {g.hx, g.hy, g.hz};
    int t = (int)i, dir = 0;
    int sx = 0, sy = 0, sz = 0;
    for (; dir < 27; ++dir) {
      if (dir == 13) continue;
      const int dd[3] = {dir / 9 - 1, (dir / 3) % 3 - 1, dir % 3 - 1};
      sx = dd[0] ? h3[0] : kBlk; sy = dd[1] ? h3[1] : kBlk; sz = dd[2] ? h3[2] : kBlk;
      const int cells = sx * sy * sz;
      if (t < cells) break;
      t -= cells;
    }
    const int ddx = dir / 9 - 1, ddy = (dir / 3) % 3 - 1, ddz = dir % 3 - 1;
    const int tz = t % sz, ty = (t / sz) % sy, tx = t / (sz * sy);
    const int lx = ddx < 0 ? kBlk - g.hx + tx : tx;
    const int ly = ddy < 0 ? kBlk - g.hy + ty : ty;
    const int lz = ddz < 0 ? kBlk - g.hz + tz : tz;
    const int X = lx + kBlk * ddx + g.hx, Y = ly + kBlk * ddy + g.hy, Z = lz + kBlk * ddz + g.hz;
    halo[i] = ((uint32_t)dir << 27) | ((uint32_t)cell_index(lx, ly, lz) << 16) | (uint32_t)(X * g.px + Y * g.py + Z);
  }
}

__device__ __forceinline__ void store_cell(int32_t* cell, int row, bool strict) {
  if (strict) __hip_atomic_fetch_min(reinterpret_cast<uint32_t*>(cell), (uint32_t)row, __ATOMIC_RELAXED, __HIP_MEMORY_SCOPE_AGENT);
  else *cell = row;
}

template <int PHASE>
__global__ __launch_bounds__(kInsertThreads) void cell_insert_kernel(BSlot* __restrict__ slots, uint32_t cmask,
                                                          const int4* __restrict__ coords, int64_t n, CellTable t,
                                                          int32_t* __restrict__ status, int kp, int mw,
                                                          int32_t* __restrict__ nbr, uint32_t* __restrict__ mask,
                                                          int strict) {
  const bool compact = kp < 0;
  kp &= 0x7FFFFFFF;
  const int64_t tid = (int64_t)blockIdx.x * blockDim.x + threadIdx.x;
  const int64_t i = PHASE == 0 ? tid * kInsertSample : tid;
  const int lane = threadIdx.x & 63;
  bool live = i < n;
  int4 c = make_int4(0, 0, 0, 0);
  if (live) {
    c = coords[i];
    if (!coord_in_range(c.x, c.y, c.z, c.w)) {
      live = false;
      if (PHASE == 1) {
        atomicOr(status, (int)WCN_FLAG_COORD_RANGE);
        for (int k = 0; k < kp; ++k) nbr[i * kp + k] = compact ? 0 : -1;
        for (int w = 0; w < mw; ++w) mask[i * mw + w] = 0u;
      }
    }
  }
  int found = -1;
  int id = -1;
  bool created = false;
  uint64_t key = 0;
  if (live) {
    key = pack_key(c.x, c.y >> kBlkShift, c.z >> kBlkShift, c.w >> kBlkShift);
    uint32_t s = hash_slot(key, cmask);
    int idv = -1;
    for (uint32_t a = 0; a <= cmask; ++a) {
      unsigned long long* kptr = reinterpret_cast<unsigned long long*>(&slots[s].key);
      const uint4 v = *reinterpret_cast<const uint4*>(slots + s);
      unsigned long long cur = ((unsigned long long)v.y << 32) | v.x;
      if (cur == key) { found = (int)s; idv = (int)v.z; break; }
      if (cur == 0ull) {
        if (PHASE == 1) cur = __hip_atomic_load(kptr, __ATOMIC_RELAXED, __HIP_MEMORY_SCOPE_AGENT);
        if (cur == 0ull) {
          cur = atomicCAS(kptr, 0ull, (unsigned long long)key);
          if (cur == 0ull) {
            created = true;
            found = (int)s;
            break;
          }
        }
        if (cur == key) { found = (int)s; break; }
      }
      s = (s + 1) & cmask;
    }
    if (found < 0) atomicOr(status, (int)WCN_FLAG_TABLE_FULL);
    if (PHASE == 1 && idv >= 0 && !(idv & kIdLateBit)) id = idv;
  }
  __shared__ int s_made[kInsertThreads / 64 + 1];
  const int wave = threadIdx.x >> 6;
  const unsigned long long makers = __ballot(created);
  if (PHASE == 0) {
    if (lane == 0) s_made[wave] = __popcll(makers);
    __syncthreads();
    if (threadIdx.x == 0) {
      int tot = 0;
      for (int w = 0; w < kInsertThreads / 64; ++w) {
        const int c = s_made[w];
        s_made[w] = tot;
        tot += c;
      }
      s_made[kInsertThreads / 64] = tot > 0 ? atomicAdd(&t.ctr[0], tot) : 0;
    }
    __syncthreads();
  }
  if (makers != 0ull) {
    int base;
    if (PHASE == 0) {
      base = s_made[kInsertThreads / 64] + s_made[wave];
    } else {
      const int leader = __ffsll((long long)makers) - 1;
      base = 0;
      if (lane == leader) base = atomicAdd(&t.ctr[0], __popcll(makers));
      base = __shfl(base, leader);
    }
    int my_id = base + __popcll(makers & ((1ull << lane) - 1ull));
    if (!created) my_id = -1;
    if (my_id >= t.max_blocks) {
      atomicOr(status, (int)WCN_FLAG_TABLE_FULL);
      my_id = -1;
    }
    if (my_id >= 0) {
      t.blk_key[my_id] = key;
      slots[found].id = my_id | (PHASE == 1 ? kIdLateBit : 0);
    }
    unsigned long long todo = makers;
    while (todo != 0ull) {
      const int src = __ffsll((long long)todo) - 1;
      todo &= todo - 1ull;
      const int bid = __shfl(my_id, src);
      if (bid >= 0) {
        int4* gcells = reinterpret_cast<int4*>(t.cells + (int64_t)bid * kCells);
        gcells[lane] = make_int4(-1, -1, -1, -1);
        gcells[lane + 64] = make_int4(-1, -1, -1, -1);
      }
    }
  }
  if (PHASE == 0) return;
  if (live) mask[i * mw + (mw - 1)] = (id >= 0 || found < 0) ? kMaskUnwritten : kMaskDeferred;
  if (id >= 0) store_cell(t.cells + (int64_t)id * kCells + cell_of(c), (int)i, strict != 0);
}

__global__ __launch_bounds__(256) void cell_finish_kernel(const BSlot* __restrict__ slots, uint32_t cmask,
                                                          const int4* __restrict__ coords, int64_t n, CellTable t,
                                                          CellGeom g, int mw, const uint32_t* __restrict__ mask,
                                                          int strict) {
  const int64_t tid = (int64_t)blockIdx.x * blockDim.x + threadIdx.x;
  const int64_t nthreads = (int64_t)gridDim.x * blockDim.x;
  for (int64_t i = tid; i < n; i += nthreads) {
    if (mask[i * mw + (mw - 1)] != kMaskDeferred) continue;
    const int4 c = coords[i];
    const int id = block_id_of(slots, cmask, c);
    if (id < 0) continue;
    store_cell(t.cells + (int64_t)id * kCells + cell_of(c), (int)i, strict != 0);
  }
  const int lane = threadIdx.x & 63;
  int nblocks = t.ctr[0];
  if (nblocks > t.max_blocks) nblocks = (int)t.max_blocks;
  for (int64_t seq = tid >> 6; seq < nblocks; seq += nthreads >> 6) {
    const int id = (int)seq;
    int nid = -1;
    if (lane < 27) {
      const int ddx = lane / 9 - 1, ddy = (lane / 3) % 3 - 1, ddz = lane % 3 - 1;
      const bool needed = (ddx == 0 || g.hx > 0) && (ddy == 0 || g.hy > 0) && (ddz == 0 || g.hz > 0);
      if (lane == 13) nid = id;
      else if (needed) {
        const uint64_t key = t.blk_key[id];
        const int b = (int)((key >> 54) & kBatchMask);
        const int bx = wrap_blk((int)((key >> 36) & kCoordMask));
        const int by = wrap_blk((int)((key >> 18) & kCoordMask));
        const int bz = wrap_blk((int)(key & kCoordMask));
        const int s = block_find(slots, cmask, pack_key(b, wrap_blk(bx + ddx), wrap_blk(by + ddy), wrap_blk(bz + ddz)));
        if (s >= 0) {
          nid = slots[s].id;
          if (nid >= 0) nid &= ~kIdLateBit;
        }
      }
    }
    if (lane < 32) t.nbtab[(int64_t)id * 32 + lane] = nid;
  }
}

#ifdef WCN_PROF
__device__ unsigned long long g_bprof[4096 * 12];
#define BSTAMP(i) do { const unsigned long long now_ = wall_clock64(); prof_acc[i] += now_ - prof_prev; prof_prev = now_; } while (0)
#else
#define BSTAMP(i)
#endif

template <int LPR, bool FAST, bool COMPACT>
__global__ __launch_bounds__(kNbThreads) __attribute__((amdgpu_waves_per_eu(kNbWavesPerSimd))) void cell_neighbors_kernel(CellTable t, const uint32_t* __restrict__ halo,
                                                                    CellGeom g, int K, int kp, int mw,
                                                                    int32_t* __restrict__ nbr,
                                                                    uint32_t* __restrict__ mask,
                                                                    int32_t* __restrict__ status) {
  extern __shared__ int s_mem[];
  const int lane = threadIdx.x & 63, wave = threadIdx.x >> 6;
  uint32_t* s_halo = reinterpret_cast<uint32_t*>(s_mem);
  const int rounds = (g.halo_cells + 63) >> 6;
  const bool halo_regs = COMPACT && rounds <= 8;
  const int halo_pad = halo_regs ? 0 : rounds * 64;
  const int per_wave = g.cells + 4 + kCells / 2 + 8 + (COMPACT ? kRowBufInts : 0);
  int* s_grid = s_mem + halo_pad + wave * per_wave;
  unsigned short* s_own = reinterpret_cast<unsigned short*>(s_grid + g.cells + 4);
  const int null_cell = g.cells;
  for (int h = threadIdx.x; h < halo_pad; h += blockDim.x) s_halo[h] = h < g.halo_cells ? halo[h] : 0xFFFFFFFFu;
  if (lane == 0) s_grid[null_cell] = -1;
  __syncthreads();

  int nblocks = t.ctr[0];
  if (nblocks > t.max_blocks) nblocks = (int)t.max_blocks;
  const int gwave = blockIdx.x * (blockDim.x / 64) + wave;
  const int nwaves = gridDim.x * (blockDim.x / 64);
  constexpr int kVoxPerIter = 64 / LPR;
  const int sub = lane % LPR, vsel = lane / LPR;
  const int num_chunks = (kp + LPR - 1) / LPR;
  uint32_t he[8];
#pragma unroll
  for (int u = 0; u < 8; ++u) {
    const int idx = u * 64 + lane;
    uint32_t e = COMPACT && idx < g.halo_cells ? halo[idx] : 0xFFFFFFFFu;
    if (e == 0xFFFFFFFFu) e = (31u << 27) | (uint32_t)(g.cells + 1);
    he[u] = e;
  }
  auto load_head = [&](int seq, int& nb, int4& v0, int4& v1) {
    nb = -1;
    v0 = make_int4(-1, -1, -1, -1);
    v1 = v0;
    if (seq < nblocks) {
      if (lane < 27) nb = t.nbtab[(int64_t)seq * 32 + lane];
      const int4* own = reinterpret_cast<const int4*>(t.cells + (int64_t)seq * kCells) + lane * 2;
      v0 = own[0];
      v1 = own[1];
    }
  };
  int seq = gwave;
  int nb_c, nb_n;
  int4 c0, c1, n0, n1;
  load_head(seq, nb_c, c0, c1);
  load_head(seq + nwaves, nb_n, n0, n1);
  int hv[8];
  auto gather = [&](int nb, int r0) {
#pragma unroll
    for (int u = 0; u < 8; ++u) {
      hv[u] = -1;
      if (r0 + u < rounds) {
        const uint32_t e = s_halo[(r0 + u) * 64 + lane];
        const int nid = __shfl(nb, (int)((e >> 27) & 31u));
        if (e != 0xFFFFFFFFu && nid >= 0) hv[u] = t.cells[(int64_t)nid * kCells + ((e >> 16) & (kCells - 1))];
      }
    }
  };
  int nidv[8];
  auto gather8 = [&](int nb) {
#pragma unroll
    for (int u = 0; u < 8; ++u) nidv[u] = __shfl(nb, (int)(he[u] >> 27));
#pragma unroll
    for (int u = 0; u < 8; ++u)
      if (u < rounds) {
        const int safe = nidv[u] < 0 ? 0 : nidv[u];
        hv[u] = t.cells[(int64_t)safe * kCells + ((he[u] >> 16) & (kCells - 1))];
      }
  };
  auto scatter8 = [&]() {
#pragma unroll
    for (int u = 0; u < 8; ++u)
      if (u < rounds) s_grid[he[u] & 0xFFFFu] = nidv[u] >= 0 ? hv[u] : -1;
  };
  auto scatter_halo = [&](int r0) {
#pragma unroll
    for (int u = 0; u < 8; ++u)
      if (r0 + u < rounds) {
        const uint32_t e = s_halo[(r0 + u) * 64 + lane];
        if (e != 0xFFFFFFFFu) s_grid[e & 0xFFFFu] = hv[u];
      }
  };
  int* s_rows = s_grid + g.cells + 4 + kCells / 2 + 8;
  int pend_row = -1;
  auto flush_rows = [&](int row) {
    __builtin_amdgcn_fence(__ATOMIC_RELEASE, "wavefront");
    __builtin_amdgcn_wave_barrier();
    if (row >= 0) mask[row] = (uint32_t)s_rows[lane];
    const int piece = lane & 3;
    int rid[4];
    int4 v[4];
#pragma unroll
    for (int q = 0; q < 4; ++q) rid[q] = __shfl(row, (lane >> 2) + 16 * q);
#pragma unroll
    for (int q = 0; q < 4; ++q) {
      const int r = (lane >> 2) + 16 * q;
      v[q].x = s_rows[(piece * 4 + 0) * kRowBufPitch + r];
      v[q].y = s_rows[(piece * 4 + 1) * kRowBufPitch + r];
      v[q].z = s_rows[(piece * 4 + 2) * kRowBufPitch + r];
      v[q].w = s_rows[(piece * 4 + 3) * kRowBufPitch + r];
    }
#pragma unroll
    for (int q = 0; q < 4; ++q)
      if (rid[q] >= 0 && __popc((uint32_t)s_rows[(lane >> 2) + 16 * q]) >= 4 * piece) {
        if (FAST)
          *reinterpret_cast<int4*>(reinterpret_cast<char*>(nbr) + (__umul24((uint32_t)rid[q], kCompactPitch * 4u) + (uint32_t)piece * 16u)) = v[q];
        else
          *reinterpret_cast<int4*>(nbr + (int64_t)rid[q] * kCompactPitch + piece * 4) = v[q];
      }
    __builtin_amdgcn_fence(__ATOMIC_ACQUIRE, "wavefront");
    __builtin_amdgcn_wave_barrier();
  };
#ifdef WCN_PROF
  if (lane == 0 && gwave < 4096) g_bprof[gwave * 12 + 9] = wall_clock64();
#endif
  if (seq < nblocks) {
    if (halo_regs) gather8(nb_c);
    else gather(nb_c, 0);
  }
#ifdef WCN_PROF
  unsigned long long prof_prev = wall_clock64(), prof_acc[8] = {0, 0, 0, 0, 0, 0, 0, 0}, prof_blocks = 0;
  const unsigned long long prof_loop0 = prof_prev;
#endif
  for (; seq < nblocks; seq += nwaves) {
    BSTAMP(0);
#ifdef WCN_PROF
    ++prof_blocks;
#endif
    if (halo_regs) scatter8();
    else scatter_halo(0);
    for (int r0 = 8; r0 < rounds; r0 += 8) {
      gather(nb_c, r0);
      scatter_halo(r0);
    }
    BSTAMP(1);
    const int vals[8] = {c0.x, c0.y, c0.z, c0.w, c1.x, c1.y, c1.z, c1.w};
    const int cell0 = ((lane >> 3) + g.hx) * g.px + ((lane & 7) + g.hy) * g.py + g.hz;
    int mine = 0;
#pragma unroll
    for (int z = 0; z < 8; ++z) {
      s_grid[cell0 + z] = vals[z];
      mine += vals[z] >= 0;
    }
    int incl = mine;
#pragma unroll
    for (int d = 1; d < 64; d <<= 1) {
      const int up = __shfl_up(incl, d);
      if (lane >= d) incl += up;
    }
    const int own_cnt = __shfl(incl, 63);
    int at = incl - mine;
#pragma unroll
    for (int z = 0; z < 8; ++z)
      if (vals[z] >= 0) s_own[at++] = (unsigned short)((cell0 + z) * 4);
    if (lane < 2 * kVoxPerIter) s_own[own_cnt + lane] = (unsigned short)(null_cell * 4);
    BSTAMP(4);
    if (COMPACT) {
      flush_rows(pend_row);
      pend_row = -1;
    }
    BSTAMP(5);
    nb_c = nb_n; c0 = n0; c1 = n1;
    if (seq + nwaves < nblocks) {
      if (halo_regs) gather8(nb_c);
      else gather(nb_c, 0);
    }
    BSTAMP(6);
    load_head(seq + 2 * nwaves, nb_n, n0, n1);
    __builtin_amdgcn_fence(__ATOMIC_RELEASE, "wavefront");
    __builtin_amdgcn_wave_barrier();
    BSTAMP(2);
    const char* grid_bytes = reinterpret_cast<const char*>(s_grid);
    if (COMPACT) {
      int delta_lane = 0;
      if (lane < K) {
        const int l = lane % g.kz, j = (lane / g.kz) % g.ky, i = lane / (g.kz * g.ky);
        delta_lane = ((i - g.cx) * g.dx * g.px + (j - g.cy) * g.dy * g.py + (l - g.cz) * g.dz) * 4;
      }
      bool over = false;
      char* rows_bytes = reinterpret_cast<char*>(s_rows);
      const int origin4 = (g.hx * g.px + g.hy * g.py + g.hz) * 4;
      const uint32_t wp0 = (uint32_t)(kRowBufPitch + lane) * 4u, wp_max = (uint32_t)(kCompactPitch * kRowBufPitch + lane) * 4u;
      for (int e0 = 0; e0 < own_cnt; e0 += 64) {
        const bool live = e0 + lane < own_cnt;
        const int cell = live ? (int)s_own[e0 + lane] : origin4;
        const int row = live ? *reinterpret_cast<const int*>(grid_bytes + cell) : -1;
        uint32_t wp = wp0, rev = 0;
        auto answer = [&](int f) {
          *reinterpret_cast<int*>(rows_bytes + wp) = f;
          const uint32_t h = f >= 0 ? 1u : 0u;
          rev = (rev << 1) | h;
          wp = min(wp + h * (uint32_t)(kRowBufPitch * 4), wp_max);
        };
        int k = 0;
        for (; k + 4 <= K; k += 4) {
          int f[4];
#pragma unroll
          for (int u = 0; u < 4; ++u)
            f[u] = *reinterpret_cast<const int*>(grid_bytes + cell + __builtin_amdgcn_readlane(delta_lane, k + u));
#pragma unroll
          for (int u = 0; u < 4; ++u) answer(f[u]);
        }
        for (; k < K; ++k) answer(*reinterpret_cast<const int*>(grid_bytes + cell + __builtin_amdgcn_readlane(delta_lane, k)));
        const uint32_t m = __brev(rev) >> (32 - K);
        over = over || (live && __popc(m) > kCompactIds);
        s_rows[lane] = (int)m;
        if (e0 + 64 < own_cnt) flush_rows(row);
        else pend_row = row;
      }
      if (__any(over) && lane == 0) atomicOr(status, (int)WCN_FLAG_ROW_OVERFLOW);
    } else
    for (int kc = 0; kc < num_chunks; ++kc) {
      const int k = kc * LPR + sub;
      const bool k_real = k < K, k_store = k < kp;
      const int l = k % g.kz, j = (k / g.kz) % g.ky, i = k / (g.kz * g.ky);
      const int ox = (i - g.cx) * g.dx, oy = (j - g.cy) * g.dy, oz = (l - g.cz) * g.dz;
      const int delta4 = k_real ? (ox * g.px + oy * g.py + oz) * 4 : 0;
      const int w0 = (kc * LPR) >> 5;
      for (int e0 = 0; e0 < own_cnt; e0 += 2 * kVoxPerIter) {
        const int cell_a = s_own[e0 + vsel], cell_b = s_own[e0 + kVoxPerIter + vsel];
        const int row_a = *reinterpret_cast<const int*>(grid_bytes + cell_a);
        const int row_b = *reinterpret_cast<const int*>(grid_bytes + cell_b);
        int found_a = *reinterpret_cast<const int*>(grid_bytes + cell_a + delta4);
        int found_b = *reinterpret_cast<const int*>(grid_bytes + cell_b + delta4);
        if (!k_real) { found_a = -1; found_b = -1; }
        const unsigned long long ball_a = __ballot(found_a >= 0), ball_b = __ballot(found_b >= 0);
        uint32_t bits_a, bits_b, hi_a = 0, hi_b = 0;
        if (LPR == 64) {
          bits_a = (uint32_t)ball_a; hi_a = (uint32_t)(ball_a >> 32);
          bits_b = (uint32_t)ball_b; hi_b = (uint32_t)(ball_b >> 32);
        } else if (LPR == 32) {
          bits_a = vsel ? (uint32_t)(ball_a >> 32) : (uint32_t)ball_a;
          bits_b = vsel ? (uint32_t)(ball_b >> 32) : (uint32_t)ball_b;
        } else {
          bits_a = (uint32_t)(ball_a >> (vsel * LPR)) & ((1u << LPR) - 1u);
          bits_b = (uint32_t)(ball_b >> (vsel * LPR)) & ((1u << LPR) - 1u);
        }
        if (FAST) {
          char* nbr_b = reinterpret_cast<char*>(nbr);
          char* mask_b = reinterpret_cast<char*>(mask);
          const uint32_t kp4 = (uint32_t)kp * 4u, mw4 = (uint32_t)mw * 4u, k4 = (uint32_t)k * 4u, w4 = (uint32_t)w0 * 4u;
          if (row_a >= 0 && k_store) *reinterpret_cast<int*>(nbr_b + (__umul24((uint32_t)row_a, kp4) + k4)) = found_a;
          if (row_b >= 0 && k_store) *reinterpret_cast<int*>(nbr_b + (__umul24((uint32_t)row_b, kp4) + k4)) = found_b;
          if (sub == 0 && w0 < mw) {
            if (row_a >= 0) *reinterpret_cast<uint32_t*>(mask_b + (__umul24((uint32_t)row_a, mw4) + w4)) = bits_a;
            if (row_b >= 0) *reinterpret_cast<uint32_t*>(mask_b + (__umul24((uint32_t)row_b, mw4) + w4)) = bits_b;
            if (LPR == 64 && w0 + 1 < mw) {
              if (row_a >= 0) *reinterpret_cast<uint32_t*>(mask_b + (__umul24((uint32_t)row_a, mw4) + w4 + 4u)) = hi_a;
              if (row_b >= 0) *reinterpret_cast<uint32_t*>(mask_b + (__umul24((uint32_t)row_b, mw4) + w4 + 4u)) = hi_b;
            }
          }
        } else {
          if (row_a >= 0 && k_store) nbr[(int64_t)row_a * kp + k] = found_a;
          if (row_b >= 0 && k_store) nbr[(int64_t)row_b * kp + k] = found_b;
          if (sub == 0 && w0 < mw) {
            if (row_a >= 0) mask[(int64_t)row_a * mw + w0] = bits_a;
            if (row_b >= 0) mask[(int64_t)row_b * mw + w0] = bits_b;
            if (LPR == 64 && w0 + 1 < mw) {
              if (row_a >= 0) mask[(int64_t)row_a * mw + w0 + 1] = hi_a;
              if (row_b >= 0) mask[(int64_t)row_b * mw + w0 + 1] = hi_b;
            }
          }
        }
      }
    }
    BSTAMP(3);

    __builtin_amdgcn_fence(__ATOMIC_ACQUIRE, "wavefront");
    __builtin_amdgcn_wave_barrier();
  }
  if (COMPACT) flush_rows(pend_row);
#ifdef WCN_PROF
  if (lane == 0 && gwave < 4096) {
    for (int i = 0; i < 8; ++i) g_bprof[gwave * 12 + i] = prof_acc[i];
    g_bprof[gwave * 12 + 8] = prof_blocks;
    g_bprof[gwave * 12 + 10] = prof_loop0;
    g_bprof[gwave * 12 + 11] = wall_clock64();
  }
#endif
}

static void launch_cell_table(const CellTable& t, const CellGeom& g, const int4* coords, int64_t n, int kp, int mw, int32_t* nbr,
                              uint32_t* mask, int32_t* status, int strict, hipStream_t s) {
  const int64_t capacity = t.capacity;
  const uint32_t cmask = (uint32_t)(capacity - 1);
  const int64_t max_blocks = t.max_blocks;
  const int64_t prep = capacity > g.halo_cells ? capacity : g.halo_cells;
  hipLaunchKernelGGL(cell_prepare_kernel, dim3((unsigned)ceil_div(prep, 256)), dim3(256), 0, s, (uint4*)t.slots, capacity,
                     t.ctr, t.halo, g, status);
  const int64_t n_first = ceil_div(n, kInsertSample);
  hipLaunchKernelGGL(cell_insert_kernel<0>, dim3((unsigned)ceil_div(n_first, kInsertThreads)), dim3(kInsertThreads), 0, s, t.slots, cmask,
                     coords, n, t, status, kp, mw, nbr, mask, strict);
  hipLaunchKernelGGL(cell_insert_kernel<1>, dim3((unsigned)ceil_div(n, kInsertThreads)), dim3(kInsertThreads), 0, s, t.slots, cmask,
                     coords, n, t, status, kp, mw, nbr, mask, strict);
  {
    const int64_t work = n > 64 * max_blocks ? n : 64 * max_blocks;
    int64_t wgs = ceil_div(work, 256);
    if (wgs > 8192) wgs = 8192;
    hipLaunchKernelGGL(cell_finish_kernel, dim3((unsigned)wgs), dim3(256), 0, s, (const BSlot*)t.slots, cmask,
                       coords, n, t, g, mw, (const uint32_t*)mask, strict);
  }
}

}

using namespace wcn;

extern "C" {

size_t wcn_kmap_binned_workspace(int64_t n, int64_t max_blocks) {
  if (n < 0) n = 0;
  if (max_blocks < 1) max_blocks = 1;
  return carve_cells(nullptr, n, max_blocks).bytes;
}

int wcn_kmap_binned_supported(const int32_t ksize[3], const int32_t dilation[3]) {
  if (!ksize || !dilation) return 0;
  for (int d = 0; d < 3; ++d) {
    if (ksize[d] < 1 || dilation[d] < 1) return 0;
  }
  const int32_t unit[3] = {1, 1, 1};
  const KernelGeom g = make_kernel_geom(ksize, unit, dilation);
  if (kernel_halo(g.kx, g.cx, g.dx) > kMaxHalo || kernel_halo(g.ky, g.cy, g.dy) > kMaxHalo ||
      kernel_halo(g.kz, g.cz, g.dz) > kMaxHalo)
    return 0;
  const int64_t K = (int64_t)ksize[0] * ksize[1] * ksize[2];
  return (valid_k(K) && (K & 31) != 0) ? 1 : 0;
}

int wcn_kmap_compact_supported(int32_t num_offsets) {
  return (num_offsets >= 17 && num_offsets <= 31) ? 1 : 0;
}

int wcn_kmap_build_binned(const int32_t* coords, int64_t n, const int32_t ksize[3], const int32_t dilation[3],
                          int64_t max_blocks, int32_t strict, int32_t compact, void* workspace, size_t workspace_bytes,
                          int32_t* nbr, uint32_t* mask, int32_t* status, wcn_stream_t stream) {
  if (n < 0 || !status || max_blocks < 1 || max_blocks > (1ll << 29)) return WCN_ERROR_INVALID_PARAMETERS;
  if (!wcn_kmap_binned_supported(ksize, dilation)) return WCN_ERROR_PROBLEM_NOT_SUPPORTED;
  if (compact && (!ksize || !wcn_kmap_compact_supported(ksize[0] * ksize[1] * ksize[2]))) return WCN_ERROR_PROBLEM_NOT_SUPPORTED;
  if (n == 0) return WCN_SUCCESS;
  if (n >= (1ll << 31) || !coords || !nbr || !mask || !workspace ||
      workspace_bytes < wcn_kmap_binned_workspace(n, max_blocks))
    return WCN_ERROR_INVALID_PARAMETERS;
  hipStream_t s = (hipStream_t)stream;
  const CellTable t = carve_cells(workspace, n, max_blocks);
  const int K = ksize[0] * ksize[1] * ksize[2];
  const int kp = wcn_kmap_row_pitch(K), mw = wcn_kmap_mask_words(K);
  const CellGeom g = make_cell_geom(ksize, dilation);
  const int64_t capacity = t.capacity;
  const uint32_t cmask = (uint32_t)(capacity - 1);

  launch_cell_table(t, g, (const int4*)coords, n, compact ? (kCompactPitch | kCompactFlag) : kp, mw, nbr, mask, status, (int)strict, s);
  const int halo_rounds = (g.halo_cells + 63) >> 6;
  const int halo_pad = compact && halo_rounds <= 8 ? 0 : halo_rounds * 64;
  int nb_waves = kNbThreads / 64;
  auto shm_for = [&](int waves) {
    return ((size_t)halo_pad + (size_t)waves * (g.cells + 4 + kCells / 2 + 8 + (compact ? kRowBufInts : 0))) * 4;
  };
  while (nb_waves > 1 && shm_for(nb_waves) > 156 * 1024) nb_waves >>= 1;
  const size_t shm = shm_for(nb_waves);
  if (shm > 160 * 1024) return WCN_ERROR_PROBLEM_NOT_SUPPORTED;
  int per_cu = (int)((160 * 1024) / (shm + 512));
  if (per_cu > 8) per_cu = 8;
  if (compact && per_cu * nb_waves > 4 * kNbWavesPerSimd) per_cu = 4 * kNbWavesPerSimd / nb_waves;
  if (per_cu < 1) per_cu = 1;
  int64_t want = ceil_div(max_blocks < n ? max_blocks : n, nb_waves);
  if (want > 256 * per_cu) want = 256 * per_cu;
  const dim3 grid((unsigned)want), block(nb_waves * 64);
  if (shm > 64 * 1024) {
    static unsigned long long attr_done = 0ull;
    const int rc = once_per_device(attr_done, [] {
      bool ok = true;
      for (const void* f : {reinterpret_cast<const void*>(cell_neighbors_kernel<8, true, false>), reinterpret_cast<const void*>(cell_neighbors_kernel<8, false, false>),
                            reinterpret_cast<const void*>(cell_neighbors_kernel<16, true, false>), reinterpret_cast<const void*>(cell_neighbors_kernel<16, false, false>),
                            reinterpret_cast<const void*>(cell_neighbors_kernel<32, true, false>), reinterpret_cast<const void*>(cell_neighbors_kernel<32, false, false>),
                            reinterpret_cast<const void*>(cell_neighbors_kernel<32, true, true>), reinterpret_cast<const void*>(cell_neighbors_kernel<32, false, true>),
                            reinterpret_cast<const void*>(cell_neighbors_kernel<64, true, false>), reinterpret_cast<const void*>(cell_neighbors_kernel<64, false, false>)})
        ok = ok && hipFuncSetAttribute(f, hipFuncAttributeMaxDynamicSharedMemorySize, 160 * 1024) == hipSuccess;
      return ok;
    });
    if (rc != WCN_SUCCESS) return rc;
  }
  const bool fast = n < (1ll << 24) && n * kp * 4 < (1ll << 31);
#define WCN_CELL_NB(L, C)                                                                                                 \
  do {                                                                                                                    \
    if (fast)                                                                                                             \
      hipLaunchKernelGGL((cell_neighbors_kernel<L, true, C>), grid, block, shm, s, t, (const uint32_t*)t.halo, g, K, kp,  \
                         mw, nbr, mask, status);                                                                          \
    else                                                                                                                  \
      hipLaunchKernelGGL((cell_neighbors_kernel<L, false, C>), grid, block, shm, s, t, (const uint32_t*)t.halo, g, K, kp, \
                         mw, nbr, mask, status);                                                                          \
  } while (0)
  if (compact) {
    WCN_CELL_NB(32, true);
  } else {
    switch (lanes_per_row(kp)) {
      case 8: WCN_CELL_NB(8, false); break;
      case 16: WCN_CELL_NB(16, false); break;
      case 32: WCN_CELL_NB(32, false); break;
      default: WCN_CELL_NB(64, false); break;
    }
  }
#undef WCN_CELL_NB
  return launch_status();
}

int wcn_kmap_cells_build(const int32_t* coords, int64_t n, int64_t max_blocks, void* workspace, size_t workspace_bytes,
                         uint32_t* scratch, int32_t* status, wcn_stream_t stream) {
  if (n < 0 || !status || max_blocks < 1 || max_blocks > (1ll << 29)) return WCN_ERROR_INVALID_PARAMETERS;
  if (n == 0) return WCN_SUCCESS;
  if (n >= (1ll << 31) || !coords || !scratch || !workspace || workspace_bytes < wcn_kmap_binned_workspace(n, max_blocks))
    return WCN_ERROR_INVALID_PARAMETERS;
  const CellTable t = carve_cells(workspace, n, max_blocks);
  const int32_t one[3] = {1, 1, 1};
  const CellGeom g = make_cell_geom(one, one);
  launch_cell_table(t, g, (const int4*)coords, n, 0, 1, nullptr, scratch, status, 1, (hipStream_t)stream);
  return launch_status();
}

}

#ifdef WCN_PROF
extern "C" int wcn_debug_read_bprof(void* dst, size_t bytes) {
  return (int)hipMemcpyFromSymbol(dst, HIP_SYMBOL(wcn::g_bprof), bytes);
}
#endif
```

### warpconvnet_amd/csrc/kmap_bucket.hip

```cpp
#include "kmap_cells.h"
#include "mask_sort.h"

namespace wcn {

constexpr int kTileRows = 256;
constexpr int kBkThreads = 256;
constexpr int kTallyThreads = (kRsTile / kTileRows) * 64;
constexpr int kStageCap = 3072;

static_assert(kRsTile % kTileRows == 0, "a sort tile is a whole number of bucket tiles");
static_assert(kBkThreads == kRsThreads, "the scan launch runs rs_scan_body (mask_sort.h) in its digit workgroups");

__device__ __noinline__ void repair_row(int64_t row, const int4* __restrict__ coords, const CellTable& t, uint32_t cmask,
                                        int kp, int mw, int32_t* __restrict__ nbr, uint32_t* __restrict__ mask,
                                        int32_t* __restrict__ status) {
  const int4 c = coords[row];
  const int id = block_id_of(t.slots, cmask, c);
  const int w = id >= 0 ? t.cells[(int64_t)id * kCells + cell_of(c)] : -1;
  const bool compact = kp < 0;
  kp &= 0x7FFFFFFF;
  if (w >= 0 && w != row && !(mask[(int64_t)w * mw + (mw - 1)] & kMaskUnwritten)) {
    atomicOr(status, (int)(WCN_FLAG_DUPLICATE_COORD | (w > row ? WCN_FLAG_NEED_STRICT : 0)));
    for (int k = 0; k < kp; ++k) nbr[row * kp + k] = nbr[(int64_t)w * kp + k];
    for (int q = 0; q < mw; ++q) mask[row * mw + q] = mask[(int64_t)w * mw + q];
  } else {
    for (int k = 0; k < kp; ++k) nbr[row * kp + k] = compact ? 0 : -1;
    for (int q = 0; q < mw; ++q) mask[row * mw + q] = 0u;
  }
}

template <bool HIST, bool REPAIR>
__global__ __launch_bounds__(kTallyThreads) void kmap_tally_kernel(uint32_t* __restrict__ mask, int32_t* __restrict__ nbr,
                                                                int64_t m, int K, int kp, int mw, int64_t ntile,
                                                                int32_t* __restrict__ counts, int32_t* __restrict__ ticket,
                                                                int nblk_sort, int32_t* __restrict__ dcounts,
                                                                const int4* __restrict__ coords, CellTable t,
                                                                uint32_t cmask, int32_t* __restrict__ status, int kc,
                                                                int sort_shift, int sort_bits) {
  __shared__ int s_hist[kRsMaxBins];
  const int sort_bins = 1 << sort_bits;
  const int tid = threadIdx.x, lane = tid & 63, wave = tid >> 6;
  if (HIST) {
    for (int i = tid; i < sort_bins; i += kTallyThreads) s_hist[i] = 0;
    __syncthreads();
  }
  if (blockIdx.x == 0 && tid == 0) *ticket = 0;
  constexpr int kTilesPerBlock = kRsTile / kTileRows;
  for (int tt = 0; tt < 1; ++tt) {
    const int64_t tile = (int64_t)blockIdx.x * kTilesPerBlock + wave;
    if (tile >= ntile) break;
    const int64_t row0 = tile * kTileRows;
    uint32_t last[kTileRows / 64];
#pragma unroll
    for (int sb = 0; sb < kTileRows / 64; ++sb) {
      const int64_t row = row0 + sb * 64 + lane;
      last[sb] = row < m ? mask[row * mw + (mw - 1)] : 0u;
    }
    if (REPAIR) {
#pragma unroll
      for (int sb = 0; sb < kTileRows / 64; ++sb) {
        const int64_t row = row0 + sb * 64 + lane;
        if (last[sb] & kMaskUnwritten) {
          repair_row(row, coords, t, cmask, kp, mw, nbr, mask, status);
          last[sb] = mask[row * mw + (mw - 1)];
        }
      }
    }
    for (int w = 0; w < mw; ++w) {
      const int kend = (K - w * 32) < 32 ? (K - w * 32) : 32;
      int mine = 0;
#pragma unroll
      for (int sb = 0; sb < kTileRows / 64; ++sb) {
        const int64_t row = row0 + sb * 64 + lane;
        const uint32_t bits = (w == mw - 1) ? last[sb] : (row < m ? mask[row * mw + w] : 0u);
        if (HIST && w == 0 && row < m) atomicAdd(&s_hist[rs_digit(tile_key(bits, kc), sort_shift, sort_bits)], 1);
        for (int b = 0; b < kend; ++b) {
          const int c = __popcll(__ballot((bits >> b) & 1u));
          if (lane == b) mine += c;
        }
      }
      if (lane < kend) counts[(int64_t)(w * 32 + lane) * ntile + tile] = mine;
    }
  }
  if (HIST) {
    __syncthreads();
    if ((int)blockIdx.x < nblk_sort)
      for (int i = tid; i < sort_bins; i += kTallyThreads) dcounts[(int64_t)blockIdx.x * sort_bins + i] = s_hist[i];
  }
}

__global__ __launch_bounds__(kBkThreads) void kmap_scan_kernel(int32_t* __restrict__ counts, int64_t ntile, int K,
                                                               int32_t* __restrict__ totals, int32_t* __restrict__ ticket,
                                                               int32_t* __restrict__ offsets,
                                                               const int32_t* __restrict__ status,
                                                               int32_t* __restrict__ mirror, int32_t* __restrict__ dcounts,
                                                               int nblk_sort, int32_t* __restrict__ dtotals, int sort_bins) {
  __shared__ int s_wave[kBkThreads / 64];
  __shared__ int s_last;
  const int tid = threadIdx.x;
  if ((int)blockIdx.x >= K) {
    __shared__ int s_cols[kBkThreads];
    rs_scan_body(dcounts, dtotals, nblk_sort, sort_bins, (int)blockIdx.x - K, reinterpret_cast<char*>(s_cols));
    return;
  }
  const int total = scan_counts_in_place<kBkThreads, 16>(counts + (int64_t)blockIdx.x * ntile, ntile, s_wave);
  if (tid == 0) {
    __hip_atomic_store(&totals[blockIdx.x], total, __ATOMIC_RELAXED, __HIP_MEMORY_SCOPE_AGENT);
    __threadfence();
    s_last = (atomicAdd(ticket, 1) == K - 1);
  }
  __syncthreads();
  if (!s_last) return;
  __threadfence();
  int carry = 0;
  for (int base = 0; base < K; base += kBkThreads) {
    const int k = base + tid;
    const int v = k < K ? __hip_atomic_load(&totals[k], __ATOMIC_RELAXED, __HIP_MEMORY_SCOPE_AGENT) : 0;
    int trip;
    const int o = carry + block_excl_scan<kBkThreads>(v, s_wave, &trip) + v;
    if (k < K) {
      offsets[k + 1] = o;
      if (mirror) mirror[k + 1] = o;
    }
    carry += trip;
    __syncthreads();
  }
  if (tid == 0) {
    offsets[0] = 0;
    if (mirror) {
      mirror[0] = 0;
      mirror[K + 1] = status ? __hip_atomic_load(status, __ATOMIC_RELAXED, __HIP_MEMORY_SCOPE_AGENT) : 0;
      __threadfence_system();
      __hip_atomic_store(&mirror[K + 2], 1, __ATOMIC_RELEASE, __HIP_MEMORY_SCOPE_SYSTEM);
    }
  }
}

struct KsArgs {
  const int32_t* nbr;
  const uint32_t* mask;
  int64_t m;
  int K, kp, mw;
  int64_t ntile;
  const int32_t* counts;
  const int32_t* offsets;
  int32_t* in_maps;
  int32_t* out_maps;
  int64_t pair_capacity;
  int32_t* status;
  int compact;
};
static KsArgs ks_args(const int32_t* nbr, const uint32_t* mask, int64_t m, int32_t K, const int32_t* counts,
                      const int32_t* offsets, int32_t* in_maps, int32_t* out_maps, int64_t pair_capacity, int32_t* status,
                      int compact) {
  KsArgs q;
  q.compact = compact;
  q.nbr = nbr; q.mask = mask; q.m = m; q.K = K; q.kp = wcn_kmap_row_pitch(K); q.mw = wcn_kmap_mask_words(K);
  q.ntile = wcn_kmap_num_blocks(m); q.counts = counts; q.offsets = offsets; q.in_maps = in_maps; q.out_maps = out_maps;
  q.pair_capacity = pair_capacity; q.status = status;
  return q;
}

__device__ __forceinline__ void place_pair(int32_t* __restrict__ in_maps, int32_t* __restrict__ out_maps, int64_t pos,
                                           int64_t pair_capacity, int in_row, int out_row, bool& overflow) {
  if (pos < pair_capacity) {
    in_maps[pos] = in_row;
    out_maps[pos] = out_row;
  } else {
    overflow = true;
  }
}

constexpr size_t kKsLds = (size_t)2 * kStageCap * 4 + 32 * 8 + (size_t)(kBkThreads / 64) * 32 * 12 + 36 * 4 + kStageCap;

__device__ __forceinline__ void kmap_scatter_body(const KsArgs& q, int64_t tile_id, char* smem) {
  const int32_t* __restrict__ nbr = q.nbr;
  const uint32_t* __restrict__ mask = q.mask;
  const int64_t m = q.m, ntile = q.ntile, pair_capacity = q.pair_capacity;
  const int K = q.K, kp = q.kp, mw = q.mw;
  const int32_t* __restrict__ counts = q.counts;
  const int32_t* __restrict__ offsets = q.offsets;
  int32_t* __restrict__ in_maps = q.in_maps;
  int32_t* __restrict__ out_maps = q.out_maps;
  int32_t* s_in = reinterpret_cast<int32_t*>(smem);
  int32_t* s_out = s_in + kStageCap;
  int64_t* s_gbase = reinterpret_cast<int64_t*>(s_out + kStageCap);
  unsigned long long(*s_ball)[32] = reinterpret_cast<unsigned long long(*)[32]>(s_gbase + 32);
  int(*s_cnt)[32] = reinterpret_cast<int(*)[32]>(s_ball + kBkThreads / 64);
  int* s_seg = reinterpret_cast<int*>(s_cnt + kBkThreads / 64);
  unsigned char* s_bk = reinterpret_cast<unsigned char*>(s_seg + 36);
  const int tid = threadIdx.x, lane = tid & 63, wave = tid >> 6;
  const int64_t row0 = tile_id * kTileRows + wave * 64;
  const int64_t row = row0 + lane;
  bool overflow = false;
  for (int w = 0; w < mw; ++w) {
    const int kend = (K - w * 32) < 32 ? (K - w * 32) : 32;
    const int cols4 = ((kp - w * 32) < 32 ? (kp - w * 32) : 32) >> 2;
    int4 piece[8];
#pragma unroll
    for (int j = 0; j < 8; ++j) {
      const int e = lane + 64 * j;
      const int r = e / cols4, c = e - r * cols4;
      piece[j] = make_int4(-1, -1, -1, -1);
      if (j < cols4 && row0 + r < m) piece[j] = *reinterpret_cast<const int4*>(nbr + (row0 + r) * kp + w * 32 + c * 4);
    }
    const uint32_t bits = row < m ? mask[row * mw + w] : 0u;
    unsigned long long mine = 0ull;
    for (int b = 0; b < kend; ++b) {
      const unsigned long long ball = __ballot((bits >> b) & 1u);
      if (lane == b) mine = ball;
    }
    if (lane < 32) {
      s_ball[wave][lane] = mine;
      s_cnt[wave][lane] = __popcll(mine);
    }
    __syncthreads();
    if (wave == 0) {
      int tot = 0;
      if (lane < 32) {
#pragma unroll
        for (int q = 0; q < kBkThreads / 64; ++q) {
          const int c = s_cnt[q][lane];
          s_cnt[q][lane] = tot;
          tot += c;
        }
      }
      const int incl = wave_incl_scan<32>(tot);
      if (lane < 32) s_seg[lane] = incl - tot;
      if (lane == 31) s_seg[32] = incl;
      if (lane < kend) s_gbase[lane] = (int64_t)offsets[w * 32 + lane] + counts[(int64_t)(w * 32 + lane) * ntile + tile_id];
    }
    __syncthreads();
    const int total = s_seg[32];
    const bool staged = total <= kStageCap;
    auto place = [&](int val, int r, int b, int local, const int& seg, const int64_t& gbase) {
      if (staged) {
        s_in[seg + local] = val;
        s_out[seg + local] = (int32_t)(row0 + r);
        s_bk[seg + local] = (unsigned char)b;
      } else {
        place_pair(in_maps, out_maps, gbase + local, pair_capacity, val, (int32_t)(row0 + r), overflow);
      }
    };
    if ((64 % cols4) == 0) {
      const int c = lane % cols4, r0 = lane / cols4, rstep = 64 / cols4;
      int cnt_q[4], seg_q[4];
      unsigned long long ball_q[4];
      int64_t gb_q[4];
#pragma unroll
      for (int t = 0; t < 4; ++t) {
        const int b = (c * 4 + t) & 31;
        cnt_q[t] = s_cnt[wave][b];
        ball_q[t] = s_ball[wave][b];
        seg_q[t] = s_seg[b];
        gb_q[t] = s_gbase[b];
      }
#pragma unroll
      for (int j = 0; j < 8; ++j) {
        if (j >= cols4) break;
        const int r = r0 + j * rstep;
        const unsigned long long below = (1ull << r) - 1ull;
        const int vals[4] = {piece[j].x, piece[j].y, piece[j].z, piece[j].w};
#pragma unroll
        for (int t = 0; t < 4; ++t) {
          const int b = c * 4 + t;
          if (vals[t] < 0 || b >= kend) continue;
          place(vals[t], r, b, cnt_q[t] + __popcll(ball_q[t] & below), seg_q[t], gb_q[t]);
        }
      }
    } else {
#pragma unroll
      for (int j = 0; j < 8; ++j) {
        if (j >= cols4) break;
        const int e = lane + 64 * j;
        const int r = e / cols4, c = e - r * cols4;
        const int vals[4] = {piece[j].x, piece[j].y, piece[j].z, piece[j].w};
#pragma unroll
        for (int q = 0; q < 4; ++q) {
          const int b = c * 4 + q;
          if (vals[q] < 0 || b >= kend) continue;
          place(vals[q], r, b, s_cnt[wave][b] + __popcll(s_ball[wave][b] & ((1ull << r) - 1ull)), s_seg[b], s_gbase[b]);
        }
      }
    }
    __syncthreads();
    if (staged) {
      for (int e = tid; e < total; e += kBkThreads) {
        const int b = s_bk[e];
        place_pair(in_maps, out_maps, s_gbase[b] + (e - s_seg[b]), pair_capacity, s_in[e], s_out[e], overflow);
      }
    }
    __syncthreads();
  }
  if (overflow) atomicOr(q.status, (int)WCN_FLAG_PAIR_OVERFLOW);
}

struct __attribute__((aligned(16))) KcSlot {
  unsigned long long ball;
  int base;
  int pad;
};
constexpr size_t kKcLds = (size_t)kStageCap * 8 + (size_t)(kBkThreads / 64) * 32 * sizeof(KcSlot) + 32 * 8 + 36 * 4 + kBkThreads * 4;

__global__ __launch_bounds__(kBkThreads) void kmap_scatter_compact_kernel(KsArgs q) {
  extern __shared__ __attribute__((aligned(16))) char s_kc[];
  uint2* s_pair = reinterpret_cast<uint2*>(s_kc);
  KcSlot(*s_wb)[32] = reinterpret_cast<KcSlot(*)[32]>(s_pair + kStageCap);
  int64_t* s_delta = reinterpret_cast<int64_t*>(s_wb + kBkThreads / 64);
  int* s_seg = reinterpret_cast<int*>(s_delta + 32);
  uint32_t* s_rowmask = reinterpret_cast<uint32_t*>(s_seg + 36);
  const int32_t* __restrict__ nbr = q.nbr;
  const int64_t m = q.m, pair_capacity = q.pair_capacity;
  const int K = q.K;
  int32_t* __restrict__ in_maps = q.in_maps;
  int32_t* __restrict__ out_maps = q.out_maps;
  const int tid = threadIdx.x, lane = tid & 63, wave = tid >> 6;
  const int64_t tile_row0 = (int64_t)blockIdx.x * kTileRows;
  const int64_t row0 = tile_row0 + wave * 64;
  const int64_t row = row0 + lane;
  int4 piece[4];
#pragma unroll
  for (int j = 0; j < 4; ++j) {
    const int r = (lane >> 2) + 16 * j;
    piece[j] = make_int4(0, 0, 0, 0);
    if (row0 + r < m) piece[j] = *reinterpret_cast<const int4*>(nbr + (row0 + r) * kCompactPitch + (lane & 3) * 4);
  }
  uint32_t bits = row < m ? q.mask[row] : 0u;
  if (__popc(bits) > kCompactIds) bits = 0u;
  s_rowmask[tid] = bits;
  unsigned long long mine = 0ull;
  for (int b = 0; b < K; ++b) {
    const unsigned long long ball = __ballot((bits >> b) & 1u);
    if (lane == b) mine = ball;
  }
  if (lane < 32) {
    s_wb[wave][lane].ball = mine;
    s_wb[wave][lane].base = __popcll(mine);
  }
  __syncthreads();
  if (wave == 0) {
    int tot = 0, cw[kBkThreads / 64];
    if (lane < 32) {
#pragma unroll
      for (int w2 = 0; w2 < kBkThreads / 64; ++w2) {
        cw[w2] = tot;
        tot += s_wb[w2][lane].base;
      }
    }
    const int incl = wave_incl_scan<32>(tot);
    if (lane < 32) {
      const int seg = incl - tot;
      s_seg[lane] = seg;
#pragma unroll
      for (int w2 = 0; w2 < kBkThreads / 64; ++w2) s_wb[w2][lane].base = seg + cw[w2];
      int64_t g = 0;
      if (lane < K) g = (int64_t)q.offsets[lane] + q.counts[(int64_t)lane * q.ntile + blockIdx.x];
      s_delta[lane] = g - seg;
    }
    if (lane == 31) s_seg[32] = incl;
  }
  __syncthreads();
  const int total = s_seg[32];
  const bool staged = total <= kStageCap;
  bool overflow = false;
  const int c = lane & 3;
#pragma unroll
  for (int j = 0; j < 4; ++j) {
    const int r = (lane >> 2) + 16 * j;
    uint32_t rem = s_rowmask[wave * 64 + r];
    for (int sk = 4 * c - 1; sk > 0; --sk) rem &= rem - 1u;
    const unsigned long long below = (1ull << r) - 1ull;
    const int vals[4] = {piece[j].x, piece[j].y, piece[j].z, piece[j].w};
#pragma unroll
    for (int t = 0; t < 4; ++t) {
      if (c == 0 && t == 0) continue;
      if (rem == 0u) break;
      const int b = __builtin_ctz(rem);
      rem &= rem - 1u;
      const uint4 slot = *reinterpret_cast<const uint4*>(&s_wb[wave][b]);
      const unsigned long long ball = ((unsigned long long)slot.y << 32) | slot.x;
      const int at = (int)slot.z + __popcll(ball & below);
      if (staged) {
        s_pair[at] = make_uint2((uint32_t)vals[t], (uint32_t)(((wave * 64 + r) << 8) | b));
      } else {
        place_pair(in_maps, out_maps, s_delta[b] + at, pair_capacity, vals[t], (int32_t)(row0 + r), overflow);
      }
    }
  }
  __syncthreads();
  if (staged) {
    for (int e = tid; e < total; e += kBkThreads) {
      const uint2 pr = s_pair[e];
      const int64_t pos = s_delta[pr.y & 31u] + e;
      if (pos < pair_capacity) {
        in_maps[pos] = (int32_t)pr.x;
        out_maps[pos] = (int32_t)(tile_row0 + (pr.y >> 8));
      } else {
        overflow = true;
      }
    }
  }
  if (overflow) atomicOr(q.status, (int)WCN_FLAG_PAIR_OVERFLOW);
}

__global__ __launch_bounds__(kBkThreads) void kmap_scatter_kernel(KsArgs q) {
  extern __shared__ char s_ks[];
  kmap_scatter_body(q, blockIdx.x, s_ks);
}

static void launch_scatter(const KsArgs& q, hipStream_t s) {
  const dim3 grid((unsigned)ceil_div(q.m, kTileRows)), block(kBkThreads);
  if (q.compact) hipLaunchKernelGGL(kmap_scatter_compact_kernel, grid, block, kKcLds, s, q);
  else hipLaunchKernelGGL(kmap_scatter_kernel, grid, block, kKsLds, s, q);
}

__global__ __launch_bounds__(256) void kmap_densify_kernel(const int32_t* __restrict__ nbrc, int64_t m, int kp,
                                                           int32_t* __restrict__ nbr) {
  const int cols4 = kp >> 2;
  const int64_t e = (int64_t)blockIdx.x * blockDim.x + threadIdx.x;
  if (e >= m * cols4) return;
  const int64_t row = e / cols4;
  const int c = (int)(e - row * cols4);
  const int32_t* src = nbrc + row * kCompactPitch;
  uint32_t bits = (uint32_t)src[0];
  if (__popc(bits) > kCompactIds) bits = 0u;
  int at = 1 + __popc(bits & ((1u << (4 * c)) - 1u));
  int v[4];
#pragma unroll
  for (int t = 0; t < 4; ++t) {
    const bool has = (bits >> (4 * c + t)) & 1u;
    v[t] = has ? src[at] : -1;
    at += has ? 1 : 0;
  }
  *reinterpret_cast<int4*>(nbr + row * kp + 4 * c) = make_int4(v[0], v[1], v[2], v[3]);
}

}

using namespace wcn;

extern "C" {

int64_t wcn_kmap_num_blocks(int64_t m) { return (ceil_div(m > 0 ? m : 0, kTileRows) + 3) & ~(int64_t)3; }

size_t wcn_kmap_counts_bytes(int64_t m, int32_t num_offsets) {
  return ((size_t)num_offsets * (size_t)(wcn_kmap_num_blocks(m) + 1) + 64) * 4;
}

static void launch_tally(uint32_t* mask, int32_t* nbr, int64_t m, int K, int32_t* counts, bool hist, int nblk_sort,
                         int32_t* dcounts, const int32_t* coords, const CellTable* cells, int32_t* status, int kc, int sort_shift,
                         int sort_bits, hipStream_t s, bool compact = false) {
  const int kp = compact ? (kCompactPitch | kCompactFlag) : wcn_kmap_row_pitch(K), mw = wcn_kmap_mask_words(K);
  const int64_t ntile = wcn_kmap_num_blocks(m);
  int32_t* ticket = counts + (int64_t)K * (ntile + 1);
  const dim3 grid((unsigned)ceil_div(m, kRsTile)), block(kTallyThreads);
  CellTable none{};
  const CellTable& t = cells ? *cells : none;
  const uint32_t cmask = cells ? (uint32_t)(cells->capacity - 1) : 0u;
#define WCN_TALLY(H, R)                                                                                                \
  hipLaunchKernelGGL((kmap_tally_kernel<H, R>), grid, block, 0, s, mask, nbr, m, K, kp, mw, ntile, counts, ticket,       \
                     nblk_sort, dcounts, (const int4*)coords, t, cmask, status, kc, sort_shift, sort_bits)
  if (hist && cells) WCN_TALLY(true, true);
  else if (hist) WCN_TALLY(true, false);
  else if (cells) WCN_TALLY(false, true);
  else WCN_TALLY(false, false);
#undef WCN_TALLY
}

static void launch_scan(int32_t* counts, int64_t ntile, int K, int32_t* offsets, const int32_t* status, int32_t* mirror,
                        int nblk_sort, int32_t* dcounts, int32_t* dtotals, int sort_bins, hipStream_t s) {
  int32_t* totals = counts + (int64_t)K * ntile;
  int32_t* ticket = totals + K;
  hipLaunchKernelGGL(kmap_scan_kernel, dim3((unsigned)(K + (nblk_sort > 0 ? (sort_bins + kRsScanCols - 1) / kRsScanCols : 0))), dim3(kBkThreads), 0,
                     s, counts, ntile, K, totals, ticket, offsets, status, mirror, dcounts, nblk_sort, dtotals, sort_bins);
}

int wcn_kmap_count(const uint32_t* mask, int64_t m, int32_t num_offsets, int32_t* counts, wcn_stream_t stream) {
  if (m < 0 || !valid_k(num_offsets)) return WCN_ERROR_INVALID_PARAMETERS;
  if (m == 0) return WCN_SUCCESS;
  if (!mask || !counts) return WCN_ERROR_INVALID_PARAMETERS;
  launch_tally(const_cast<uint32_t*>(mask), nullptr, m, num_offsets, counts, false, 0, nullptr, nullptr, nullptr, nullptr, 0, 0,
               kRsBits, (hipStream_t)stream);
  return launch_status();
}

static int scan_impl(int32_t* counts, int64_t num_blocks, int32_t K, int32_t* offsets, const int32_t* status,
                     int32_t* mirror, wcn_stream_t stream) {
  if (num_blocks < 0 || (num_blocks & 3) || !valid_k(K) || !offsets || !counts) return WCN_ERROR_INVALID_PARAMETERS;
  launch_scan(counts, num_blocks, K, offsets, status, mirror, 0, nullptr, nullptr, 0, (hipStream_t)stream);
  return launch_status();
}

int wcn_kmap_scan(int32_t* counts, int64_t num_blocks, int32_t num_offsets, int32_t* offsets, wcn_stream_t stream) {
  return scan_impl(counts, num_blocks, num_offsets, offsets, nullptr, nullptr, stream);
}

int wcn_kmap_scan_to_host(int32_t* counts, int64_t num_blocks, int32_t num_offsets, int32_t* offsets, const int32_t* status,
                          int32_t* host_mirror, wcn_stream_t stream) {
  if (!host_mirror) return WCN_ERROR_INVALID_PARAMETERS;
  return scan_impl(counts, num_blocks, num_offsets, offsets, status, host_mirror, stream);
}

size_t wcn_kmap_tally_sort_workspace(int64_t m) { return wcn_mask_argsort_workspace(m); }

int wcn_kmap_tally_sort(uint32_t* mask, int32_t* nbr, int64_t m, int32_t num_offsets, int32_t* counts, int32_t* offsets,
                        int32_t* status, int32_t* host_mirror, int32_t* perm, void* sort_workspace,
                        size_t sort_workspace_bytes, const int32_t* coords, void* binned_workspace, int64_t binned_n,
                        int64_t max_blocks, int32_t compact, int32_t* in_maps, int32_t* out_maps, int64_t pair_capacity,
                        wcn_stream_t stream) {
  if (m < 0 || !valid_k(num_offsets) || !counts || !offsets || !status) return WCN_ERROR_INVALID_PARAMETERS;
  if (pair_capacity < 0 || ((in_maps == nullptr) != (out_maps == nullptr))) return WCN_ERROR_INVALID_PARAMETERS;
  if (compact && !wcn_kmap_compact_supported(num_offsets)) return WCN_ERROR_INVALID_PARAMETERS;
  hipStream_t s = (hipStream_t)stream;
  if (m == 0) {
    if (hipMemsetAsync(offsets, 0, (size_t)(num_offsets + 1) * 4, s) != hipSuccess) return WCN_ERROR_KERNEL_EXECUTION;
    if (host_mirror) {
      if (hipMemsetAsync(host_mirror, 0, (size_t)(num_offsets + 1) * 4, s) != hipSuccess ||
          hipMemcpyAsync(host_mirror + num_offsets + 1, status, 4, hipMemcpyDeviceToHost, s) != hipSuccess)
        return WCN_ERROR_KERNEL_EXECUTION;
    }
    return WCN_SUCCESS;
  }
  if (m >= (1ll << 31) || !mask || !nbr || !perm || !sort_workspace ||
      sort_workspace_bytes < wcn_kmap_tally_sort_workspace(m))
    return WCN_ERROR_INVALID_PARAMETERS;
  if (binned_workspace && (!coords || binned_n != m || max_blocks < 1)) return WCN_ERROR_INVALID_PARAMETERS;
  const int kc = tile_key_centre(num_offsets, wcn_kmap_mask_words(num_offsets));
  const SortPlan plan = sort_plan(sort_workspace, m, num_offsets < 32 ? num_offsets : 32, kc > 0);
  CellTable cells{};
  if (binned_workspace) cells = carve_cells(binned_workspace, binned_n, max_blocks);
  launch_tally(mask, nbr, m, num_offsets, counts, true, plan.nblk, plan.counts, coords, binned_workspace ? &cells : nullptr,
               status, kc, plan.shift0, plan.bits, s, compact != 0);
  launch_scan(counts, wcn_kmap_num_blocks(m), num_offsets, offsets, status, host_mirror, plan.nblk, plan.counts,
              plan.totals, 1 << plan.bits, s);
  RsLaunch l[12];
  const int count = sort_launches(plan, mask, wcn_kmap_mask_words(num_offsets), m, perm, true, kc, l);
  sort_run_range(l, 0, count, s);
  if (in_maps && pair_capacity > 0) {
    const KsArgs q = ks_args(nbr, mask, m, num_offsets, counts, offsets, in_maps, out_maps, pair_capacity, status, compact ? 1 : 0);
    launch_scatter(q, s);
  }
  return launch_status();
}

int wcn_kmap_densify(const int32_t* nbr_compact, int64_t m, int32_t num_offsets, int32_t* nbr, wcn_stream_t stream) {
  if (m < 0 || !wcn_kmap_compact_supported(num_offsets)) return WCN_ERROR_INVALID_PARAMETERS;
  if (m == 0) return WCN_SUCCESS;
  if (!nbr_compact || !nbr) return WCN_ERROR_INVALID_PARAMETERS;
  const int kp = wcn_kmap_row_pitch(num_offsets);
  hipLaunchKernelGGL(kmap_densify_kernel, dim3((unsigned)ceil_div(m * (kp >> 2), 256)), dim3(256), 0, (hipStream_t)stream,
                     nbr_compact, m, kp, nbr);
  return launch_status();
}

int wcn_kmap_scatter(const int32_t* nbr, const uint32_t* mask, int64_t m, int32_t num_offsets, const int32_t* counts,
                     const int32_t* offsets, int32_t* in_maps, int32_t* out_maps, int64_t pair_capacity, int32_t* status,
                     int32_t compact, wcn_stream_t stream) {
  if (m < 0 || !valid_k(num_offsets) || pair_capacity < 0 || !status) return WCN_ERROR_INVALID_PARAMETERS;
  if (compact && !wcn_kmap_compact_supported(num_offsets)) return WCN_ERROR_INVALID_PARAMETERS;
  if (m == 0) return WCN_SUCCESS;
  if (!nbr || !mask || !counts || !offsets || (pair_capacity > 0 && (!in_maps || !out_maps)))
    return WCN_ERROR_INVALID_PARAMETERS;
  const KsArgs q = ks_args(nbr, mask, m, num_offsets, counts, offsets, in_maps, out_maps, pair_capacity, status, compact ? 1 : 0);
  launch_scatter(q, (hipStream_t)stream);
  return launch_status();
}

}
```

### warpconvnet_amd/csrc/kmap_cells.h

```cpp
#pragma once

#include "wcn_common.h"

namespace wcn {

constexpr int kBlkShift = 3;
constexpr int kBlk = 1 << kBlkShift;
constexpr int kCells = kBlk * kBlk * kBlk;
constexpr int kMaxHalo = 8;
constexpr int kBlkCoordBits = kCoordBits - kBlkShift;
constexpr uint32_t kMaskUnwritten = 0x80000000u;
constexpr uint32_t kMaskDeferred = 0x80000001u;

constexpr int kCompactPitch = 16;
constexpr int kCompactIds = kCompactPitch - 1;
constexpr int kCompactFlag = (int)0x80000000;

constexpr int kIdLateBit = 1 << 30;

struct __attribute__((aligned(16))) BSlot {
  uint64_t key;
  int32_t id;
  int32_t pad;
};

struct CellTable {
  BSlot* slots;
  int64_t capacity;
  int32_t* ctr;
  uint32_t* halo;
  uint64_t* blk_key;
  int32_t* nbtab;
  int32_t* cells;
  int64_t max_blocks;
  size_t bytes;
};

struct KernelGeom {
  int kx, ky, kz;
  int cx, cy, cz;
  int sx, sy, sz;
  int dx, dy, dz;
};

static inline KernelGeom make_kernel_geom(const int32_t ksize[3], const int32_t stride[3], const int32_t dilation[3]) {
  auto centre = [](int ks) { return (ks & 1) ? ks / 2 : 0; };
  return KernelGeom{ksize[0],  ksize[1],  ksize[2],  centre(ksize[0]), centre(ksize[1]), centre(ksize[2]),
                    stride[0], stride[1], stride[2], dilation[0],      dilation[1],      dilation[2]};
}

static inline int kernel_halo(int ks, int c, int d) {
  const int lo = c * d, hi = (ks - 1 - c) * d;
  return lo > hi ? lo : hi;
}

static inline int lanes_per_row(int kp) {
  int l = 8;
  while (l < kp && l < 64) l <<= 1;
  return l;
}

struct CellGeom {
  int kx, ky, kz, cx, cy, cz, dx, dy, dz;
  int hx, hy, hz;
  int px, py;
  int cells;
  int halo_cells;
};

static inline int64_t cell_capacity(int64_t max_blocks) {
  int64_t c = 1024;
  while (c < 2 * max_blocks) c <<= 1;
  return c;
}

static inline CellTable carve_cells(void* ws, int64_t n, int64_t max_blocks) {
  CellTable t;
  char* p = (char*)ws;
  size_t off = 0;
  auto take = [&](size_t bytes) { char* q = p ? p + off : nullptr; off += align256(bytes); return q; };
  (void)n;
  t.max_blocks = max_blocks;
  t.capacity = cell_capacity(max_blocks);
  t.ctr = (int32_t*)take(256);
  t.halo = (uint32_t*)take((size_t)16384 * 4);
  t.slots = (BSlot*)take((size_t)t.capacity * sizeof(BSlot));
  t.blk_key = (uint64_t*)take((size_t)max_blocks * 8);
  t.nbtab = (int32_t*)take((size_t)max_blocks * 32 * 4);
  t.cells = (int32_t*)take((size_t)max_blocks * kCells * 4);
  t.bytes = off;
  return t;
}

static inline CellGeom make_cell_geom(const int32_t ksize[3], const int32_t dilation[3]) {
  const int32_t unit[3] = {1, 1, 1};
  const KernelGeom k = make_kernel_geom(ksize, unit, dilation);
  CellGeom g;
  g.kx = k.kx; g.ky = k.ky; g.kz = k.kz;
  g.cx = k.cx; g.cy = k.cy; g.cz = k.cz;
  g.dx = k.dx; g.dy = k.dy; g.dz = k.dz;
  g.hx = kernel_halo(g.kx, g.cx, g.dx); g.hy = kernel_halo(g.ky, g.cy, g.dy); g.hz = kernel_halo(g.kz, g.cz, g.dz);
  const int gx = kBlk + 2 * g.hx, gy = kBlk + 2 * g.hy, gz = kBlk + 2 * g.hz;
  g.py = gz | 1;
  g.px = gy * g.py;
  g.cells = gx * g.px;
  g.halo_cells = gx * gy * gz - kCells;
  return g;
}

__device__ __forceinline__ int block_find(const BSlot* __restrict__ slots, uint32_t cmask, uint64_t key) {
  uint32_t s = hash_slot(key, cmask);
  for (uint32_t a = 0; a <= cmask; ++a) {
    const uint64_t k = slots[s].key;
    if (k == 0ull) return -1;
    if (k == key) return (int)s;
    s = (s + 1) & cmask;
  }
  return -1;
}

__device__ __forceinline__ int block_id_of(const BSlot* __restrict__ slots, uint32_t cmask, const int4& c) {
  const int s = block_find(slots, cmask, pack_key(c.x, c.y >> kBlkShift, c.z >> kBlkShift, c.w >> kBlkShift));
  if (s < 0) return -1;
  const int id = slots[s].id;
  return id < 0 ? -1 : (id & ~kIdLateBit);
}

__device__ __forceinline__ int cell_index(int x, int y, int z) { return (x * kBlk + y) * kBlk + z; }
__device__ __forceinline__ int cell_of(const int4& c) {
  return ((c.y & (kBlk - 1)) * kBlk + (c.z & (kBlk - 1))) * kBlk + (c.w & (kBlk - 1));
}

}
```

### warpconvnet_amd/geometry/coords/search/torch_discrete.py

```python
import ctypes
import os
from typing import Literal, Optional, Sequence, Tuple

import numpy as np
import torch

from warpconvnet_amd.utils.compile_guard import eager_unless_compiling
from torch import Tensor

from warpconvnet_amd import _lib
from warpconvnet_amd.geometry.coords.search.cell_handle import attach_cells, cells_of, stride_map_of
from warpconvnet_amd.geometry.coords.search.packed_hashmap import PackedHashTable, _next_power_of_2
from warpconvnet_amd.geometry.coords.search.search_results import IntSearchResult
from warpconvnet_amd.utils.ntuple import ntuple


@torch.no_grad()
def kernel_offsets_from_size(
    kernel_size: Tuple[int, ...],
    kernel_dilation: Tuple[int, ...],
    center_offset: Optional[Tuple[int, ...]] = None,
    device: Optional[torch.device] = None,
) -> Tensor:
    assert len(kernel_size) == len(kernel_dilation)
    if center_offset is None:
        center_offset = [(s - 1) // 2 if s % 2 == 1 else 0 for s in kernel_size]
    assert len(center_offset) == len(kernel_size)
    grids = np.indices(tuple(int(s) for s in kernel_size)).reshape(len(kernel_size), -1)
    cols = [np.zeros(grids.shape[1], dtype=np.int64)]
    for d in range(len(kernel_size)):
        cols.append((grids[d] - int(center_offset[d])) * int(kernel_dilation[d]))
    out = torch.from_numpy(np.stack(cols, axis=1).astype(np.int32))
    return out.to(device) if device is not None else out


@torch.no_grad()
def nbr_to_pair_table(nbr: Tensor, num_offsets: int) -> Tensor:
    M = nbr.shape[0]
    out = torch.empty((num_offsets, M), dtype=torch.int32, device=nbr.device)
    _lib.check(
        _lib.lib().wcn_kmap_transpose(_lib.ptr(nbr), M, num_offsets, _lib.ptr(out), _lib.stream_handle(nbr.device)),
        "wcn_kmap_transpose",
    )
    return out


@torch.no_grad()
def mask_argsort(mask: Tensor, num_offsets: int = 32) -> Tensor:
    n, mw = mask.shape
    perm = torch.empty(n, dtype=torch.int32, device=mask.device)
    if n == 0:
        return perm
    L = _lib.lib()
    ws_bytes = L.wcn_mask_argsort_workspace(n)
    ws = torch.empty(ws_bytes, dtype=torch.uint8, device=mask.device)
    _lib.check(
        L.wcn_mask_tile_order(_lib.ptr(mask), mw, int(num_offsets), n, _lib.ptr(perm), _lib.ptr(ws), ws_bytes,
                              _lib.stream_handle(mask.device)),
        "wcn_mask_tile_order",
    )
    return perm


@torch.no_grad()
def argsort_u32_ascending(keys: Tensor, num_bits: int) -> Tensor:
    n = keys.shape[0]
    perm = torch.empty(n, dtype=torch.int32, device=keys.device)
    if n == 0:
        return perm
    num_bits = max(1, min(int(num_bits), 31))
    flipped = (((1 << num_bits) - 1) - keys.to(torch.int32)).contiguous()
    L = _lib.lib()
    ws_bytes = L.wcn_mask_argsort_workspace(n)
    ws = torch.empty(ws_bytes, dtype=torch.uint8, device=keys.device)
    _lib.check(
        L.wcn_mask_argsort(_lib.ptr(flipped), 1, num_bits, n, _lib.ptr(perm), _lib.ptr(ws), ws_bytes, _lib.stream_handle(keys.device)),
        "wcn_mask_argsort",
    )
    return perm


@torch.no_grad()
def attach_tables_from_csr(kmap: IntSearchResult, num_in: int, num_out: int) -> IntSearchResult:
    kmap.validate()
    if kmap.has_tables:
        return kmap
    twin = kmap._twin
    if twin is not None and not twin._has_duplicates:
        twin.validate()
        if twin.has_tables and twin._num_out == num_in:
            kmap._nbr, kmap._mask, kmap._perm = reverse_tables(twin, num_out)
            kmap._offsets_dev = twin._offsets_dev
            kmap._num_in, kmap._num_out = num_in, num_out
            return kmap
    dev = kmap.in_maps_device.device
    K = len(kmap)
    L = _lib.lib()
    kp, mw = L.wcn_kmap_row_pitch(K), L.wcn_kmap_mask_words(K)
    nbr = torch.empty((num_out, kp), dtype=torch.int32, device=dev)
    mask = torch.empty((num_out, mw), dtype=torch.int32, device=dev)
    offsets_dev = kmap._offsets_dev if kmap._offsets_dev is not None else kmap.offsets.to(device=dev, dtype=torch.int32)
    _lib.check(
        L.wcn_kmap_from_csr(_lib.ptr(kmap.in_maps_device), _lib.ptr(kmap.out_maps_device), _lib.ptr(offsets_dev), K,
                            kmap.in_maps_device.shape[0], num_out, _lib.ptr(nbr), _lib.ptr(mask), _lib.stream_handle(dev)),
        "wcn_kmap_from_csr",
    )
    kmap._nbr, kmap._mask, kmap._offsets_dev = nbr, mask, offsets_dev
    kmap._perm = mask_argsort(mask, K)
    kmap._num_in, kmap._num_out = num_in, num_out
    return kmap


@torch.no_grad()
def reverse_tables(kmap: IntSearchResult, num_in: int) -> Tuple[Tensor, Tensor, Tensor]:
    kmap.validate()
    twin = kmap._twin
    if kmap._rev is None and twin is not None and not twin._has_duplicates:
        twin.validate()
        if twin.has_tables and twin._num_out == num_in:
            kmap._rev = (twin._nbr, twin._mask, twin._perm)
    if kmap._rev is None:
        dev = kmap.in_maps_device.device
        K = len(kmap)
        L = _lib.lib()
        kp, mw = L.wcn_kmap_row_pitch(K), L.wcn_kmap_mask_words(K)
        rev_nbr = torch.empty((num_in, kp), dtype=torch.int32, device=dev)
        rev_mask = torch.empty((num_in, mw), dtype=torch.int32, device=dev)
        if kmap._offsets_dev is None:
            kmap._offsets_dev = kmap.offsets.to(device=dev, dtype=torch.int32)
        _lib.check(
            L.wcn_kmap_reverse(_lib.ptr(kmap.in_maps_device), _lib.ptr(kmap.out_maps_device), _lib.ptr(kmap._offsets_dev), K,
                               kmap.in_maps_device.shape[0], num_in, _lib.ptr(rev_nbr), _lib.ptr(rev_mask),
                               _lib.stream_handle(dev)),
            "wcn_kmap_reverse",
        )
        if (kmap._stride_window and int(kmap.offsets[-1]) == num_in
                and kmap.in_maps_device.shape[0] == num_in):
            rev_perm = kmap.in_maps_device
        else:
            rev_perm = mask_argsort(rev_mask, K)
        kmap._rev = (rev_nbr, rev_mask, rev_perm)
    return kmap._rev


def _first_half(full: IntSearchResult) -> IntSearchResult:
    c = len(full) // 2
    offs = full.offsets[: c + 1].clone()
    n = int(offs[-1])
    return IntSearchResult(full.in_maps_device[:n].clone(), full.out_maps_device[:n].clone(), offs, identity_map_index=c)


_SPIN_POLLS = 4000


class BuildHints:

    def __init__(self, div: int = 16, pairs_per_row: float = 12.0):
        self.div = int(div)
        self.pairs_per_row = float(pairs_per_row)
        self._by_volume = {}
        self._dense_volumes = set()
        self.stats = {"builds": 0, "rebuilds": 0, "pair_rewrites": 0}

    def compact_rows(self, num_offsets: int) -> bool:
        return int(num_offsets) not in self._dense_volumes

    def observe_row_overflow(self, num_offsets: int) -> None:
        self._dense_volumes.add(int(num_offsets))

    def reset(self) -> None:
        self.__init__()

    def max_blocks(self, n: int) -> int:
        return max(1024, n // self.div) if self.div > 1 else max(n, 1)

    def pair_capacity(self, rows: int, num_offsets: int) -> int:
        per_row = self._by_volume.get(int(num_offsets), self.pairs_per_row)
        return int(min(num_offsets * rows, rows * per_row * 1.25 + 4096))

    def observe_pairs(self, rows: int, pairs: int, num_offsets: int = 0) -> None:
        if rows > 0:
            seen = pairs / rows
            self.pairs_per_row = seen if seen > self.pairs_per_row else 0.5 * (self.pairs_per_row + seen)
            if num_offsets > 0:
                cur = self._by_volume.get(int(num_offsets))
                self._by_volume[int(num_offsets)] = seen if cur is None or seen > cur else 0.5 * (cur + seen)


_DEFAULT_HINTS = BuildHints()


def default_hints() -> BuildHints:
    return _DEFAULT_HINTS


@eager_unless_compiling
@torch.no_grad()
def generate_kernel_map(
    batch_indexed_in_coords: Tensor,
    batch_indexed_out_coords: Tensor,
    in_to_out_stride_ratio: Tuple[int, ...],
    kernel_size: Tuple[int, ...],
    kernel_dilation: Optional[Tuple[int, ...]] = None,
    kernel_center_offset: Optional[Tuple[int, ...]] = None,
    method: Literal["offset", "size"] = "size",
    skip_symmetric_kernel_map: bool = False,
    need_pairs: bool = True,
    optimistic: bool = False,
    hints: Optional[BuildHints] = None,
    **kwargs,
) -> IntSearchResult:
    dev = batch_indexed_in_coords.device
    assert dev == batch_indexed_out_coords.device
    assert batch_indexed_in_coords.dtype == torch.int32 and batch_indexed_out_coords.dtype == torch.int32
    if not batch_indexed_in_coords.is_cuda:
        raise RuntimeError(
            "generate_kernel_map runs on the GPU through libwcn_hip.so; got CPU coordinates (no CPU fallback)"
        )
    if method not in ("offset", "size"):
        raise ValueError(f"Invalid method: {method}. Choose 'offset', or 'size'.")
    odd_kernel = all(int(k) % 2 == 1 for k in kernel_size)
    if skip_symmetric_kernel_map:
        assert len(batch_indexed_in_coords) == len(batch_indexed_out_coords), (
            "You can only skip symmetric kernel map if the input and output coordinates are the same.")
        assert odd_kernel, "Kernel size must be odd for symmetric skipping."
    if method == "size":
        assert kernel_center_offset is None, (
            "Custom kernel_center_offset is not supported with method='size'. Use method='offset' instead.")
    half_map = (skip_symmetric_kernel_map or method == "offset") and odd_kernel and (
        len(batch_indexed_in_coords) == len(batch_indexed_out_coords))
    if kernel_center_offset is not None:
        nd = len(kernel_size)
        dil = ntuple(kernel_dilation if kernel_dilation is not None else 1, nd)
        c_def = [(int(k) - 1) // 2 if int(k) % 2 == 1 else 0 for k in kernel_size]
        delta = [(cd - int(cu)) * int(d) for cd, cu, d in zip(c_def, kernel_center_offset, dil)]
        shift = torch.tensor([0] + delta, dtype=torch.int32, device=dev)
        full = generate_kernel_map(batch_indexed_in_coords - shift, batch_indexed_out_coords, in_to_out_stride_ratio,
                                   kernel_size, kernel_dilation, None, "size", False)
        return _first_half(full) if half_map else full
    if half_map:
        return _first_half(generate_kernel_map(batch_indexed_in_coords, batch_indexed_out_coords, in_to_out_stride_ratio,
                                               kernel_size, kernel_dilation, None, "size", False))
    same_tensor = (
        batch_indexed_in_coords.data_ptr() == batch_indexed_out_coords.data_ptr()
        and batch_indexed_in_coords.shape == batch_indexed_out_coords.shape
    )
    if batch_indexed_in_coords.shape[1] == 3:
        batch_indexed_in_coords = torch.nn.functional.pad(batch_indexed_in_coords, (0, 1), value=0)
        batch_indexed_out_coords = (
            batch_indexed_in_coords if same_tensor else torch.nn.functional.pad(batch_indexed_out_coords, (0, 1), value=0)
        )
        kernel_size = tuple(kernel_size) + (1,)
        in_to_out_stride_ratio = tuple(in_to_out_stride_ratio) + (1,)
        if kernel_dilation is not None:
            kernel_dilation = tuple(kernel_dilation) + (1,)
    assert batch_indexed_in_coords.shape[1] == 4, "expected batch-indexed 3-D coordinates [N, 4]"
    ksize = ntuple(kernel_size, 3)
    stride = ntuple(in_to_out_stride_ratio, 3)
    dilation = ntuple(kernel_dilation if kernel_dilation is not None else 1, 3)
    K = ksize[0] * ksize[1] * ksize[2]

    in_coords = batch_indexed_in_coords.contiguous()
    out_coords = in_coords if same_tensor else batch_indexed_out_coords.contiguous()
    N, M = in_coords.shape[0], out_coords.shape[0]
    L = _lib.lib()
    stream = _lib.stream_handle(dev)
    kp, mw = L.wcn_kmap_row_pitch(K), L.wcn_kmap_mask_words(K)
    nblk = L.wcn_kmap_num_blocks(M)

    unit_stride = all(s == 1 for s in stride)
    method_env = os.environ.get("WARPCONVNET_AMD_KMAP_METHOD", "auto").strip().lower()
    use_binned = (
        method_env != "hash" and same_tensor and unit_stride and N > 0
        and bool(L.wcn_kmap_binned_supported(_lib.i3(ksize), _lib.i3(dilation)))
    )
    if method_env == "binned" and not use_binned and N > 0:
        raise RuntimeError("WARPCONVNET_AMD_KMAP_METHOD=binned needs a submanifold map (same coordinate tensor, stride 1, "
                           "halo <= 8, K % 32 != 0)")
    hints = hints if hints is not None else _DEFAULT_HINTS
    table_capacity = _next_power_of_2(max(16, 2 * N))
    compact_ok = use_binned and bool(L.wcn_kmap_compact_supported(K)) and os.environ.get("WARPCONVNET_AMD_KMAP_COMPACT", "1") != "0"
    state = {"max_blocks": hints.max_blocks(N), "strict": 0, "compact": bool(compact_ok and hints.compact_rows(K))}
    odd = all(k % 2 == 1 for k in ksize)
    cells = prebuilt = None
    if not use_binned and N > 0 and M > 0 and os.environ.get("WARPCONVNET_AMD_KMAP_METHOD", "auto").strip().lower() != "hash":
        cells = cells_of(batch_indexed_in_coords)
        pm = stride_map_of(batch_indexed_out_coords, batch_indexed_in_coords, in_coords)
        if (pm is not None and pm[0] == tuple(stride) == tuple(ksize) and all(d == 1 for d in dilation)
                and pm[1].shape[0] == M):
            prebuilt = (pm[1], pm[2])

    def launch(spec_capacity: int = 0):
        max_blocks, strict, compact = state["max_blocks"], state["strict"], state["compact"]
        nbr = torch.empty((M, 16 if compact else kp), dtype=torch.int32, device=dev)
        mask = torch.empty((M, mw), dtype=torch.int32, device=dev)
        block_counts = torch.empty(L.wcn_kmap_counts_bytes(M, K) // 4, dtype=torch.int32, device=dev)
        perm = torch.empty(M, dtype=torch.int32, device=dev)
        meta = (torch.empty if use_binned else torch.zeros)(K + 2, dtype=torch.int32, device=dev)
        table, bin_ws = None, None
        stream = _lib.stream_handle(dev)
        if use_binned:
            ws_bytes = L.wcn_kmap_binned_workspace(N, max_blocks)
            bin_ws = torch.empty(ws_bytes, dtype=torch.uint8, device=dev)
            _lib.check(
                L.wcn_kmap_build_binned(_lib.ptr(in_coords), N, _lib.i3(ksize), _lib.i3(dilation), max_blocks, strict, int(compact),
                                        _lib.ptr(bin_ws), ws_bytes, _lib.ptr(nbr), _lib.ptr(mask), _lib.ptr(meta[K + 1 :]),
                                        stream),
                "wcn_kmap_build_binned",
            )
        elif prebuilt is not None:
            nbr, mask = prebuilt
        elif cells is not None:
            _lib.check(
                L.wcn_kmap_probe_cells(_lib.ptr(cells[0]), N, cells[2], _lib.ptr(out_coords), M, _lib.i3(ksize), _lib.i3(stride),
                                       _lib.i3(dilation), _lib.ptr(nbr), _lib.ptr(mask), stream),
                "wcn_kmap_probe_cells",
            )
        else:
            table = PackedHashTable(max(16, 2 * N), device=dev)
            table._launch_insert(in_coords, meta[K + 1 :])
            _lib.check(
                L.wcn_kmap_probe(_lib.ptr(table.slots_tensor), table.capacity, _lib.ptr(out_coords), M, _lib.i3(ksize),
                                 _lib.i3(stride), _lib.i3(dilation), _lib.ptr(nbr), _lib.ptr(mask), stream),
                "wcn_kmap_probe",
            )
        meta_host = torch.empty(K + 3, dtype=torch.int32, pin_memory=True)
        ready = ctypes.c_int32.from_address(meta_host.data_ptr() + 4 * (K + 2))
        ready.value = 0
        sort_bytes = L.wcn_kmap_tally_sort_workspace(M)
        sort_ws = torch.empty(sort_bytes, dtype=torch.uint8, device=dev)
        spec_capacity = max(int(spec_capacity), 0) if M > 0 else 0
        spec_in = torch.empty(spec_capacity, dtype=torch.int32, device=dev) if spec_capacity else None
        spec_out = torch.empty(spec_capacity, dtype=torch.int32, device=dev) if spec_capacity else None
        _lib.check(
            L.wcn_kmap_tally_sort(_lib.ptr(mask), _lib.ptr(nbr), M, K, _lib.ptr(block_counts), _lib.ptr(meta),
                                  _lib.ptr(meta[K + 1 :]), ctypes.c_void_p(meta_host.data_ptr()), _lib.ptr(perm),
                                  _lib.ptr(sort_ws), sort_bytes, _lib.ptr(in_coords) if use_binned else None,
                                  _lib.ptr(bin_ws), N if use_binned else 0, max_blocks if use_binned else 0, int(compact),
                                  _lib.ptr(spec_in), _lib.ptr(spec_out), spec_capacity, stream),
            "wcn_kmap_tally_sort",
        )
        event = torch.cuda.Event()
        event.record(torch.cuda.current_stream(dev))
        return dict(nbr=nbr, mask=mask, perm=perm, block_counts=block_counts, meta=meta, meta_host=meta_host, ready=ready,
                    event=event, table=table, keep=(bin_ws, sort_ws, cells), max_blocks=max_blocks, compact=compact,
                    spec_pairs=(spec_in, spec_out, spec_capacity) if spec_capacity else None)

    def scatter(b, capacity):
        capacity = max(int(capacity), 0)
        in_maps = torch.empty(capacity, dtype=torch.int32, device=dev)
        out_maps = torch.empty(capacity, dtype=torch.int32, device=dev)
        _lib.check(
            L.wcn_kmap_scatter(_lib.ptr(b["nbr"]), _lib.ptr(b["mask"]), M, K, _lib.ptr(b["block_counts"]), _lib.ptr(b["meta"]),
                               _lib.ptr(in_maps), _lib.ptr(out_maps), capacity, _lib.ptr(b["meta"][K + 1 :]), int(b["compact"]),
                               _lib.stream_handle(dev)),
            "wcn_kmap_scatter",
        )
        return in_maps, out_maps, capacity

    def settle(b):
        rebuilt = False
        while True:
            if M > 0:
                for _ in range(_SPIN_POLLS):
                    if b["ready"].value:
                        break
            if not b["ready"].value:
                b["event"].synchronize()
            flags = int(b["meta_host"][K + 1])
            if use_binned and (flags & _lib.WCN_FLAG_TABLE_FULL) and state["max_blocks"] < N:
                hints.div = 4 if hints.div > 4 else 1
                state["max_blocks"] = max(1024, N // 4) if hints.div == 4 and state["max_blocks"] < max(1024, N // 4) else N
            elif use_binned and (flags & _lib.WCN_FLAG_ROW_OVERFLOW) and state["compact"]:
                hints.observe_row_overflow(K)
                state["compact"] = False
            elif use_binned and (flags & _lib.WCN_FLAG_NEED_STRICT) and not state["strict"]:
                state["strict"] = 1
            else:
                return b, flags, rebuilt
            hints.stats["rebuilds"] += 1
            b, rebuilt = launch(), True

    def attach_tables(result, b):
        result._nbr, result._mask, result._perm = None, b["mask"], b["perm"]
        if b["compact"]:
            result._nbrc = b["nbr"]
        else:
            result._nbr = b["nbr"]
        result._offsets_dev = b["meta"][: K + 1]
        result._hashtable = b["table"]
        result._keepalive = b

    def finalize(result, b, flags):
        PackedHashTable.raise_for_flags(flags, N, table_capacity)
        offsets_host = torch.from_numpy(b["meta_host"].numpy()[: K + 1].copy())
        pair_capacity = int(offsets_host[-1])
        has_duplicates = bool(flags & _lib.WCN_FLAG_DUPLICATE_COORD)
        identity = K // 2 if (odd and unit_stride and N == M) else None
        if has_duplicates and same_tensor:
            identity = None
        hints.observe_pairs(M, pair_capacity, K)
        if use_binned and not (flags & (_lib.WCN_FLAG_TABLE_FULL | _lib.WCN_FLAG_NEED_STRICT | _lib.WCN_FLAG_ROW_OVERFLOW)):
            attach_cells(in_coords, b["keep"][0], N, b["max_blocks"])
            if batch_indexed_in_coords is not in_coords and batch_indexed_in_coords.data_ptr() == in_coords.data_ptr():
                attach_cells(batch_indexed_in_coords, b["keep"][0], N, b["max_blocks"])
        attach_tables(result, b)
        result._offsets = offsets_host
        result.identity_map_index = identity
        result._device = torch.device(dev)
        spec = b.get("spec_pairs")
        if spec is not None and spec[2] < pair_capacity:
            spec = None
            hints.stats["pair_rewrites"] += 1
        if spec is not None:
            in_full, out_full, cap = spec
            if cap > 2 * pair_capacity + 65536:
                in_full, out_full = in_full[:pair_capacity].clone(), out_full[:pair_capacity].clone()
            result._in_maps, result._out_maps = in_full[:pair_capacity], out_full[:pair_capacity]
            result._lazy_pairs = None
            b["spec_pairs"] = None
        elif need_pairs:
            result._in_maps, result._out_maps = scatter(b, pair_capacity)[:2]
            result._lazy_pairs = None
        else:
            result._in_maps = result._out_maps = None
            result._lazy_pairs = lambda: scatter(b, pair_capacity)[:2]
        result._symmetric = bool(same_tensor and odd and unit_stride and not has_duplicates)
        result._self_exact = result._symmetric
        result._has_duplicates = bool(same_tensor and has_duplicates)
        result._dup_symmetric = bool(result._has_duplicates and odd and unit_stride)

    result = IntSearchResult._blank(K, dev)
    result._num_in, result._num_out = N, M
    result._kernel_size = ksize
    result._stride_window = prebuilt is not None
    spec = 0
    if optimistic and need_pairs and M > 0:
        spec = min(N, K * M) if prebuilt is not None else hints.pair_capacity(M, K)
    hints.stats["builds"] += 1
    first = launch(spec)
    if optimistic:
        if need_pairs and first.get("spec_pairs") is None:
            first["spec_pairs"] = scatter(first, 0)
        attach_tables(result, first)

        def validate_fn(res, b=first):
            b2, flags, rebuilt = settle(b)
            finalize(res, b2, flags)
            return rebuilt

        result._validate_fn = validate_fn
        return result
    b, flags, _ = settle(first)
    finalize(result, b, flags)
    return result
```

Measured before the change: 1078 M voxels/s.

## Build binned kernel map over a cached dense block bounding box

Remembers the block-coordinate bounding box seen in earlier kernel-map builds of similar size. When a box is known, blocks get dense ids from box coordinates, so neighbour tables are filled directly instead of being allocated through a hash insert and a finish pass. Any point outside the box sets a miss flag: the box is widened and the build is run again. The finish kernel and tally-sort now report the observed box to a pinned host buffer so the hint can be updated. This adds extra reductions, host bookkeeping and a possible rebuild when scenes change shape.

```diff
diff --git a/include/wcn.h b/include/wcn.h
--- a/include/wcn.h
+++ b/include/wcn.h
@@ -28,7 +28,8 @@
   WCN_FLAG_PAIR_OVERFLOW = 4,
   WCN_FLAG_DUPLICATE_COORD = 8,
   WCN_FLAG_NEED_STRICT = 16,
-  WCN_FLAG_ROW_OVERFLOW = 32
+  WCN_FLAG_ROW_OVERFLOW = 32,
+  WCN_FLAG_BOX_MISS = 64
 };
 
 int wcn_abi_version(void);
@@ -55,18 +56,19 @@
                     int64_t* codes, wcn_stream_t stream);
 
 size_t wcn_kmap_binned_workspace(int64_t n, int64_t max_blocks);
+int wcn_kmap_box_usable(const int32_t box[8], int64_t max_blocks);
 int wcn_kmap_binned_supported(const int32_t ksize[3], const int32_t dilation[3]);
 int wcn_kmap_compact_supported(int32_t num_offsets);
 int wcn_kmap_build_binned(const int32_t* coords, int64_t n, const int32_t ksize[3], const int32_t dilation[3],
                           int64_t max_blocks, int32_t strict, int32_t compact, void* workspace, size_t workspace_bytes,
-                          int32_t* nbr, uint32_t* mask, int32_t* status, wcn_stream_t stream);
+                          int32_t* nbr, uint32_t* mask, int32_t* status, const int32_t* box, wcn_stream_t stream);
 int wcn_kmap_densify(const int32_t* nbr_compact, int64_t m, int32_t num_offsets, int32_t* nbr, wcn_stream_t stream);
 size_t wcn_kmap_tally_sort_workspace(int64_t m);
 int wcn_kmap_tally_sort(uint32_t* mask, int32_t* nbr, int64_t m, int32_t num_offsets, int32_t* counts, int32_t* offsets,
                         int32_t* status, int32_t* host_mirror, int32_t* perm, void* sort_workspace,
                         size_t sort_workspace_bytes, const int32_t* coords, void* binned_workspace, int64_t binned_n,
                         int64_t max_blocks, int32_t compact, int32_t* in_maps, int32_t* out_maps, int64_t pair_capacity,
-                        wcn_stream_t stream);
+                        int32_t* host_box, wcn_stream_t stream);
 int wcn_kmap_count(const uint32_t* mask, int64_t m, int32_t num_offsets, int32_t* counts, wcn_stream_t stream);
 int wcn_kmap_scan(int32_t* counts, int64_t num_blocks, int32_t num_offsets, int32_t* offsets,
                   wcn_stream_t stream);
diff --git a/warpconvnet_amd/_lib.py b/warpconvnet_amd/_lib.py
--- a/warpconvnet_amd/_lib.py
+++ b/warpconvnet_amd/_lib.py
@@ -15,6 +15,7 @@
 WCN_FLAG_TABLE_FULL, WCN_FLAG_COORD_RANGE, WCN_FLAG_PAIR_OVERFLOW, WCN_FLAG_DUPLICATE_COORD = 1, 2, 4, 8
 WCN_FLAG_NEED_STRICT = 16
 WCN_FLAG_ROW_OVERFLOW = 32
+WCN_FLAG_BOX_MISS = 64
 WCN_SLOT_X_FASTEST, WCN_SLOT_Z_FASTEST = 0, 1
 WCN_MASK_U8 = 3
 
@@ -77,15 +78,17 @@
     "wcn_kmap_binned_supported": (c_int, [_3I, _3I]),
     "wcn_kmap_build_binned": (
         c_int,
-        [c_void_p, c_int64, _3I, _3I, c_int64, c_int32, c_int32, c_void_p, c_size_t, c_void_p, c_void_p, c_void_p, c_void_p],
-    ),
+        [c_void_p, c_int64, _3I, _3I, c_int64, c_int32, c_int32, c_void_p, c_size_t, c_void_p, c_void_p, c_void_p, c_void_p,
+         c_void_p],
+    ),
+    "wcn_kmap_box_usable": (c_int, [c_int32 * 8, c_int64]),
     "wcn_kmap_compact_supported": (c_int, [c_int32]),
     "wcn_kmap_densify": (c_int, [c_void_p, c_int64, c_int32, c_void_p, c_void_p]),
     "wcn_kmap_tally_sort_workspace": (c_size_t, [c_int64]),
     "wcn_kmap_tally_sort": (
         c_int,
         [c_void_p, c_void_p, c_int64, c_int32, c_void_p, c_void_p, c_void_p, c_void_p, c_void_p, c_void_p, c_size_t,
-         c_void_p, c_void_p, c_int64, c_int64, c_int32, c_void_p, c_void_p, c_int64, c_void_p],
+         c_void_p, c_void_p, c_int64, c_int64, c_int32, c_void_p, c_void_p, c_int64, c_void_p, c_void_p],
     ),
     "wcn_kmap_count": (c_int, [c_void_p, c_int64, c_int32, c_void_p, c_void_p]),
     "wcn_kmap_scan": (c_int, [c_void_p, c_int64, c_int32, c_void_p, c_void_p]),
diff --git a/warpconvnet_amd/csrc/kmap.hip b/warpconvnet_amd/csrc/kmap.hip
--- a/warpconvnet_amd/csrc/kmap.hip
+++ b/warpconvnet_amd/csrc/kmap.hip
@@ -215,7 +215,7 @@
 
 extern "C" {
 
-int wcn_abi_version(void) { return 14; }
+int wcn_abi_version(void) { return 15; }
 
 const char* wcn_status_string(int status) {
   switch (status) {
diff --git a/warpconvnet_amd/csrc/kmap_binned.hip b/warpconvnet_amd/csrc/kmap_binned.hip
--- a/warpconvnet_amd/csrc/kmap_binned.hip
+++ b/warpconvnet_amd/csrc/kmap_binned.hip
@@ -18,15 +18,9 @@
   return (v ^ (1 << (bits - 1))) - (1 << (bits - 1));
 }
 
-__global__ void cell_prepare_kernel(uint4* __restrict__ slots, int64_t capacity, int32_t* __restrict__ ctr,
-                                    uint32_t* __restrict__ halo, CellGeom g, int32_t* __restrict__ status) {
-  const int64_t i = (int64_t)blockIdx.x * blockDim.x + threadIdx.x;
-  if (i < capacity) slots[i] = make_uint4(0u, 0u, 0xFFFFFFFFu, 0u);
-  if (i < 64) ctr[i] = 0;
-  if (i == 0) *status = 0;
-  if (i < g.halo_cells) {
+__device__ __forceinline__ uint32_t halo_entry(const CellGeom& g, int i) {
     const int h3[3] = {g.hx, g.hy, g.hz};
-    int t = (int)i, dir = 0;
+    int t = i, dir = 0;
     int sx = 0, sy = 0, sz = 0;
     for (; dir < 27; ++dir) {
       if (dir == 13) continue;
@@ -42,13 +36,65 @@
     const int ly = ddy < 0 ? kBlk - g.hy + ty : ty;
     const int lz = ddz < 0 ? kBlk - g.hz + tz : tz;
     const int X = lx + kBlk * ddx + g.hx, Y = ly + kBlk * ddy + g.hy, Z = lz + kBlk * ddz + g.hz;
-    halo[i] = ((uint32_t)dir << 27) | ((uint32_t)cell_index(lx, ly, lz) << 16) | (uint32_t)(X * g.px + Y * g.py + Z);
-  }
+    return ((uint32_t)dir << 27) | ((uint32_t)cell_index(lx, ly, lz) << 16) | (uint32_t)(X * g.px + Y * g.py + Z);
+}
+
+__device__ __forceinline__ int ctr_clear_value(int i) {
+  return (i >= kBoxCtr && i < kBoxCtr + 4) ? INT_MAX : (i >= kBoxCtr + 4 && i < kBoxCtr + 8) ? INT_MIN : 0;
+}
+
+__global__ void cell_prepare_kernel(uint4* __restrict__ slots, int64_t capacity, int32_t* __restrict__ ctr,
+                                    uint32_t* __restrict__ halo, CellGeom g, int32_t* __restrict__ status) {
+  const int64_t i = (int64_t)blockIdx.x * blockDim.x + threadIdx.x;
+  if (i < capacity) slots[i] = make_uint4(0u, 0u, 0xFFFFFFFFu, 0u);
+  if (i < 64) ctr[i] = ctr_clear_value((int)i);
+  if (i == 0) *status = 0;
+  if (i < g.halo_cells) halo[i] = halo_entry(g, (int)i);
+}
+
+__global__ __launch_bounds__(256) void cell_box_prepare_kernel(uint4* __restrict__ slots, int64_t capacity, CellTable t,
+                                                               uint32_t* __restrict__ halo, CellGeom g,
+                                                               int32_t* __restrict__ status, BlockBox q, int volume) {
+  const int64_t i = (int64_t)blockIdx.x * blockDim.x + threadIdx.x;
+  if (i < capacity) slots[i] = make_uint4(0u, 0u, 0xFFFFFFFFu, 0u);
+  if (i < 64) {
+    const int lo[4] = {q.b0, q.x0, q.y0, q.z0}, ext[4] = {q.nb, q.nx, q.ny, q.nz};
+    int v = 0;
+    if (i == 0) v = volume;
+    else if (i >= kBoxCtr && i < kBoxCtr + 4) v = lo[i - kBoxCtr];
+    else if (i >= kBoxCtr + 4 && i < kBoxCtr + 8) v = lo[i - kBoxCtr - 4] + ext[i - kBoxCtr - 4] - 1;
+    t.ctr[i] = v;
+  }
+  if (i == 0) *status = 0;
+  if (i < g.halo_cells) halo[i] = halo_entry(g, (int)i);
+  const int64_t id64 = i >> 6;
+  if (id64 >= volume) return;
+  const int id = (int)id64, lane = threadIdx.x & 63;
+  if (lane == 0) t.blk_key[id] = box_key(q, id);
+  if (lane < 32) {
+    int nid = -1;
+    if (lane < 27) {
+      const int ddx = lane / 9 - 1, ddy = (lane / 3) % 3 - 1, ddz = lane % 3 - 1;
+      const bool needed = (ddx == 0 || g.hx > 0) && (ddy == 0 || g.hy > 0) && (ddz == 0 || g.hz > 0);
+      if (lane == 13) nid = id;
+      else if (needed) nid = box_neighbor(q, id, lane);
+    }
+    t.nbtab[(int64_t)id * 32 + lane] = nid;
+  }
+  int4* gcells = reinterpret_cast<int4*>(t.cells + (int64_t)id * kCells);
+  gcells[lane] = make_int4(-1, -1, -1, -1);
+  gcells[lane + 64] = make_int4(-1, -1, -1, -1);
 }
 
 __device__ __forceinline__ void store_cell(int32_t* cell, int row, bool strict) {
   if (strict) __hip_atomic_fetch_min(reinterpret_cast<uint32_t*>(cell), (uint32_t)row, __ATOMIC_RELAXED, __HIP_MEMORY_SCOPE_AGENT);
   else *cell = row;
+}
+
+__device__ __forceinline__ void write_empty_row(int32_t* __restrict__ nbr, uint32_t* __restrict__ mask, int64_t i, int kp, int mw,
+                                                bool compact) {
+  for (int k = 0; k < kp; ++k) nbr[i * kp + k] = compact ? 0 : -1;
+  for (int w = 0; w < mw; ++w) mask[i * mw + w] = 0u;
 }
 
 template <int PHASE>
@@ -70,8 +116,7 @@
       live = false;
       if (PHASE == 1) {
         atomicOr(status, (int)WCN_FLAG_COORD_RANGE);
-        for (int k = 0; k < kp; ++k) nbr[i * kp + k] = compact ? 0 : -1;
-        for (int w = 0; w < mw; ++w) mask[i * mw + w] = 0u;
+        write_empty_row(nbr, mask, i, kp, mw, compact);
       }
     }
   }
@@ -159,6 +204,68 @@
   if (id >= 0) store_cell(t.cells + (int64_t)id * kCells + cell_of(c), (int)i, strict != 0);
 }
 
+__global__ __launch_bounds__(kInsertThreads) void cell_box_insert_kernel(BSlot* __restrict__ slots, uint32_t cmask,
+                                                                         const int4* __restrict__ coords, int64_t n, CellTable t,
+                                                                         int32_t* __restrict__ status, int kp, int mw,
+                                                                         int32_t* __restrict__ nbr, uint32_t* __restrict__ mask,
+                                                                         int strict, BlockBox q, int volume) {
+  const bool compact = kp < 0;
+  kp &= 0x7FFFFFFF;
+  const int64_t i = (int64_t)blockIdx.x * blockDim.x + threadIdx.x;
+  const int lane = threadIdx.x & 63;
+  if (i < volume) {
+    const uint64_t key = box_key(q, (int)i);
+    uint32_t s = hash_slot(key, cmask);
+    for (uint32_t a = 0; a <= cmask; ++a) {
+      const unsigned long long cur = atomicCAS(reinterpret_cast<unsigned long long*>(&slots[s].key), 0ull, (unsigned long long)key);
+      if (cur == 0ull) {
+        slots[s].id = (int)i;
+        break;
+      }
+      s = (s + 1) & cmask;
+    }
+  }
+  bool miss = false;
+  int blk4[4] = {0, 0, 0, 0};
+  if (i < n) {
+    const int4 c = coords[i];
+    if (!coord_in_range(c.x, c.y, c.z, c.w)) {
+      atomicOr(status, (int)WCN_FLAG_COORD_RANGE);
+      write_empty_row(nbr, mask, i, kp, mw, compact);
+    } else {
+      blk4[0] = c.x; blk4[1] = c.y >> kBlkShift; blk4[2] = c.z >> kBlkShift; blk4[3] = c.w >> kBlkShift;
+      if (box_contains(q, blk4[0], blk4[1], blk4[2], blk4[3])) {
+        mask[i * mw + (mw - 1)] = kMaskUnwritten;
+        store_cell(t.cells + (int64_t)box_id(q, blk4[0], blk4[1], blk4[2], blk4[3]) * kCells + cell_of(c), (int)i, strict != 0);
+      } else {
+        miss = true;
+        write_empty_row(nbr, mask, i, kp, mw, compact);
+      }
+    }
+  }
+  const unsigned long long missers = __ballot(miss);
+  if (missers == 0ull) return;
+  int lo[4], hi[4];
+#pragma unroll
+  for (int a = 0; a < 4; ++a) {
+    lo[a] = miss ? blk4[a] : INT_MAX;
+    hi[a] = miss ? blk4[a] : INT_MIN;
+#pragma unroll
+    for (int d = 1; d < 64; d <<= 1) {
+      lo[a] = min(lo[a], __shfl_xor(lo[a], d));
+      hi[a] = max(hi[a], __shfl_xor(hi[a], d));
+    }
+  }
+  if (lane == 0) {
+    atomicOr(status, (int)WCN_FLAG_BOX_MISS);
+#pragma unroll
+    for (int a = 0; a < 4; ++a) {
+      atomicMin(&t.ctr[kBoxCtr + a], lo[a]);
+      atomicMax(&t.ctr[kBoxCtr + 4 + a], hi[a]);
+    }
+  }
+}
+
 __global__ __launch_bounds__(256) void cell_finish_kernel(const BSlot* __restrict__ slots, uint32_t cmask,
                                                           const int4* __restrict__ coords, int64_t n, CellTable t,
                                                           CellGeom g, int mw, const uint32_t* __restrict__ mask,
@@ -172,11 +279,25 @@
     if (id < 0) continue;
     store_cell(t.cells + (int64_t)id * kCells + cell_of(c), (int)i, strict != 0);
   }
+  __shared__ int s_box[8];
+  if (threadIdx.x < 8) s_box[threadIdx.x] = threadIdx.x < 4 ? INT_MAX : INT_MIN;
+  __syncthreads();
+  int lo4[4] = {INT_MAX, INT_MAX, INT_MAX, INT_MAX}, hi4[4] = {INT_MIN, INT_MIN, INT_MIN, INT_MIN};
   const int lane = threadIdx.x & 63;
   int nblocks = t.ctr[0];
   if (nblocks > t.max_blocks) nblocks = (int)t.max_blocks;
   for (int64_t seq = tid >> 6; seq < nblocks; seq += nthreads >> 6) {
     const int id = (int)seq;
+    {
+      const uint64_t bkey = t.blk_key[id];
+      const int b4[4] = {(int)((bkey >> 54) & kBatchMask), wrap_blk((int)((bkey >> 36) & kCoordMask)),
+                         wrap_blk((int)((bkey >> 18) & kCoordMask)), wrap_blk((int)(bkey & kCoordMask))};
+#pragma unroll
+      for (int a = 0; a < 4; ++a) {
+        lo4[a] = min(lo4[a], b4[a]);
+        hi4[a] = max(hi4[a], b4[a]);
+      }
+    }
     int nid = -1;
     if (lane < 27) {
       const int ddx = lane / 9 - 1, ddy = (lane / 3) % 3 - 1, ddz = lane % 3 - 1;
@@ -196,6 +317,19 @@
       }
     }
     if (lane < 32) t.nbtab[(int64_t)id * 32 + lane] = nid;
+  }
+  if (lane == 0 && lo4[0] != INT_MAX) {
+#pragma unroll
+    for (int a = 0; a < 4; ++a) {
+      atomicMin(&s_box[a], lo4[a]);
+      atomicMax(&s_box[4 + a], hi4[a]);
+    }
+  }
+  __syncthreads();
+  if (threadIdx.x < 8) t.boxpart[(int64_t)blockIdx.x * 8 + threadIdx.x] = s_box[threadIdx.x];
+  if (tid == 0) {
+    const int64_t used = ((int64_t)nblocks + blockDim.x / 64 - 1) / (blockDim.x / 64);
+    t.ctr[kBoxRows] = (int)(used < (int64_t)gridDim.x ? used : (int64_t)gridDim.x);
   }
 }
 
@@ -493,10 +627,22 @@
 }
 
 static void launch_cell_table(const CellTable& t, const CellGeom& g, const int4* coords, int64_t n, int kp, int mw, int32_t* nbr,
-                              uint32_t* mask, int32_t* status, int strict, hipStream_t s) {
+                              uint32_t* mask, int32_t* status, int strict, hipStream_t s, const BlockBox* box = nullptr) {
   const int64_t capacity = t.capacity;
   const uint32_t cmask = (uint32_t)(capacity - 1);
   const int64_t max_blocks = t.max_blocks;
+  if (box) {
+    const int volume = (int)box_volume(*box);
+    int64_t prep = 64 * (int64_t)volume;
+    if (prep < capacity) prep = capacity;
+    if (prep < g.halo_cells) prep = g.halo_cells;
+    hipLaunchKernelGGL(cell_box_prepare_kernel, dim3((unsigned)ceil_div(prep, 256)), dim3(256), 0, s, (uint4*)t.slots, capacity, t,
+                       t.halo, g, status, *box, volume);
+    const int64_t work = n > volume ? n : (int64_t)volume;
+    hipLaunchKernelGGL(cell_box_insert_kernel, dim3((unsigned)ceil_div(work, kInsertThreads)), dim3(kInsertThreads), 0, s, t.slots,
+                       cmask, coords, n, t, status, kp, mw, nbr, mask, strict, *box, volume);
+    return;
+  }
   const int64_t prep = capacity > g.halo_cells ? capacity : g.halo_cells;
   hipLaunchKernelGGL(cell_prepare_kernel, dim3((unsigned)ceil_div(prep, 256)), dim3(256), 0, s, (uint4*)t.slots, capacity,
                      t.ctr, t.halo, g, status);
@@ -508,7 +654,7 @@
   {
     const int64_t work = n > 64 * max_blocks ? n : 64 * max_blocks;
     int64_t wgs = ceil_div(work, 256);
-    if (wgs > 8192) wgs = 8192;
+    if (wgs > kBoxPartRows) wgs = kBoxPartRows;
     hipLaunchKernelGGL(cell_finish_kernel, dim3((unsigned)wgs), dim3(256), 0, s, (const BSlot*)t.slots, cmask,
                        coords, n, t, g, mw, (const uint32_t*)mask, strict);
   }
@@ -524,6 +670,11 @@
   if (n < 0) n = 0;
   if (max_blocks < 1) max_blocks = 1;
   return carve_cells(nullptr, n, max_blocks).bytes;
+}
+
+int wcn_kmap_box_usable(const int32_t box[8], int64_t max_blocks) {
+  if (!box) return 0;
+  return box_usable(BlockBox{box[0], box[1], box[2], box[3], box[4], box[5], box[6], box[7]}, max_blocks) ? 1 : 0;
 }
 
 int wcn_kmap_binned_supported(const int32_t ksize[3], const int32_t dilation[3]) {
@@ -546,7 +697,7 @@
 
 int wcn_kmap_build_binned(const int32_t* coords, int64_t n, const int32_t ksize[3], const int32_t dilation[3],
                           int64_t max_blocks, int32_t strict, int32_t compact, void* workspace, size_t workspace_bytes,
-                          int32_t* nbr, uint32_t* mask, int32_t* status, wcn_stream_t stream) {
+                          int32_t* nbr, uint32_t* mask, int32_t* status, const int32_t* box, wcn_stream_t stream) {
   if (n < 0 || !status || max_blocks < 1 || max_blocks > (1ll << 29)) return WCN_ERROR_INVALID_PARAMETERS;
   if (!wcn_kmap_binned_supported(ksize, dilation)) return WCN_ERROR_PROBLEM_NOT_SUPPORTED;
   if (compact && (!ksize || !wcn_kmap_compact_supported(ksize[0] * ksize[1] * ksize[2]))) return WCN_ERROR_PROBLEM_NOT_SUPPORTED;
@@ -562,7 +713,11 @@
   const int64_t capacity = t.capacity;
   const uint32_t cmask = (uint32_t)(capacity - 1);
 
-  launch_cell_table(t, g, (const int4*)coords, n, compact ? (kCompactPitch | kCompactFlag) : kp, mw, nbr, mask, status, (int)strict, s);
+  BlockBox q{};
+  if (box) q = BlockBox{box[0], box[1], box[2], box[3], box[4], box[5], box[6], box[7]};
+  const bool use_box = box && box_usable(q, max_blocks);
+  launch_cell_table(t, g, (const int4*)coords, n, compact ? (kCompactPitch | kCompactFlag) : kp, mw, nbr, mask, status, (int)strict, s,
+                    use_box ? &q : nullptr);
   const int halo_rounds = (g.halo_cells + 63) >> 6;
   const int halo_pad = compact && halo_rounds <= 8 ? 0 : halo_rounds * 64;
   int nb_waves = kNbThreads / 64;
diff --git a/warpconvnet_amd/csrc/kmap_bucket.hip b/warpconvnet_amd/csrc/kmap_bucket.hip
--- a/warpconvnet_amd/csrc/kmap_bucket.hip
+++ b/warpconvnet_amd/csrc/kmap_bucket.hip
@@ -94,7 +94,9 @@
                                                                int32_t* __restrict__ offsets,
                                                                const int32_t* __restrict__ status,
                                                                int32_t* __restrict__ mirror, int32_t* __restrict__ dcounts,
-                                                               int nblk_sort, int32_t* __restrict__ dtotals, int sort_bins) {
+                                                               int nblk_sort, int32_t* __restrict__ dtotals, int sort_bins,
+                                                               const int32_t* __restrict__ box_src, const int32_t* __restrict__ box_rows,
+                                                               int32_t* __restrict__ box_dst) {
   __shared__ int s_wave[kBkThreads / 64];
   __shared__ int s_last;
   const int tid = threadIdx.x;
@@ -125,11 +127,49 @@
     carry += trip;
     __syncthreads();
   }
+  __shared__ int s_bx[8];
+  const bool fold_box = mirror && box_src && box_rows && box_dst;
+  if (fold_box) {
+    if (tid < 8) s_bx[tid] = box_src[kBoxCtr + tid];
+    __syncthreads();
+    int rows = box_src[kBoxRows];
+    if (rows > kBoxPartRows) rows = kBoxPartRows;
+    int lo[4] = {INT_MAX, INT_MAX, INT_MAX, INT_MAX}, hi[4] = {INT_MIN, INT_MIN, INT_MIN, INT_MIN};
+    for (int r0 = tid; r0 < rows; r0 += 8 * kBkThreads) {
+      int4 rl[8], rh[8];
+#pragma unroll
+      for (int u = 0; u < 8; ++u) {
+        const int r = r0 + u * kBkThreads;
+        rl[u] = make_int4(INT_MAX, INT_MAX, INT_MAX, INT_MAX);
+        rh[u] = make_int4(INT_MIN, INT_MIN, INT_MIN, INT_MIN);
+        if (r < rows) {
+          rl[u] = *reinterpret_cast<const int4*>(box_rows + (int64_t)r * 8);
+          rh[u] = *reinterpret_cast<const int4*>(box_rows + (int64_t)r * 8 + 4);
+        }
+      }
+#pragma unroll
+      for (int u = 0; u < 8; ++u) {
+        lo[0] = min(lo[0], rl[u].x); lo[1] = min(lo[1], rl[u].y); lo[2] = min(lo[2], rl[u].z); lo[3] = min(lo[3], rl[u].w);
+        hi[0] = max(hi[0], rh[u].x); hi[1] = max(hi[1], rh[u].y); hi[2] = max(hi[2], rh[u].z); hi[3] = max(hi[3], rh[u].w);
+      }
+    }
+#pragma unroll
+    for (int a = 0; a < 4; ++a) {
+      if (lo[a] != INT_MAX) atomicMin(&s_bx[a], lo[a]);
+      if (hi[a] != INT_MIN) atomicMax(&s_bx[4 + a], hi[a]);
+    }
+    __syncthreads();
+  }
   if (tid == 0) {
     offsets[0] = 0;
     if (mirror) {
       mirror[0] = 0;
       mirror[K + 1] = status ? __hip_atomic_load(status, __ATOMIC_RELAXED, __HIP_MEMORY_SCOPE_AGENT) : 0;
+      if (fold_box) {
+#pragma unroll
+        for (int a = 0; a < 8; ++a) box_dst[a] = s_bx[a];
+        box_dst[8] = box_src[0];
+      }
       __threadfence_system();
       __hip_atomic_store(&mirror[K + 2], 1, __ATOMIC_RELEASE, __HIP_MEMORY_SCOPE_SYSTEM);
     }
@@ -468,11 +508,13 @@
 }
 
 static void launch_scan(int32_t* counts, int64_t ntile, int K, int32_t* offsets, const int32_t* status, int32_t* mirror,
-                        int nblk_sort, int32_t* dcounts, int32_t* dtotals, int sort_bins, hipStream_t s) {
+                        int nblk_sort, int32_t* dcounts, int32_t* dtotals, int sort_bins, hipStream_t s,
+                        const int32_t* box_src = nullptr, const int32_t* box_rows = nullptr, int32_t* box_dst = nullptr) {
   int32_t* totals = counts + (int64_t)K * ntile;
   int32_t* ticket = totals + K;
   hipLaunchKernelGGL(kmap_scan_kernel, dim3((unsigned)(K + (nblk_sort > 0 ? (sort_bins + kRsScanCols - 1) / kRsScanCols : 0))), dim3(kBkThreads), 0,
-                     s, counts, ntile, K, totals, ticket, offsets, status, mirror, dcounts, nblk_sort, dtotals, sort_bins);
+                     s, counts, ntile, K, totals, ticket, offsets, status, mirror, dcounts, nblk_sort, dtotals, sort_bins, box_src,
+                     box_rows, box_dst);
 }
 
 int wcn_kmap_count(const uint32_t* mask, int64_t m, int32_t num_offsets, int32_t* counts, wcn_stream_t stream) {
@@ -507,7 +549,7 @@
                         int32_t* status, int32_t* host_mirror, int32_t* perm, void* sort_workspace,
                         size_t sort_workspace_bytes, const int32_t* coords, void* binned_workspace, int64_t binned_n,
                         int64_t max_blocks, int32_t compact, int32_t* in_maps, int32_t* out_maps, int64_t pair_capacity,
-                        wcn_stream_t stream) {
+                        int32_t* host_box, wcn_stream_t stream) {
   if (m < 0 || !valid_k(num_offsets) || !counts || !offsets || !status) return WCN_ERROR_INVALID_PARAMETERS;
   if (pair_capacity < 0 || ((in_maps == nullptr) != (out_maps == nullptr))) return WCN_ERROR_INVALID_PARAMETERS;
   if (compact && !wcn_kmap_compact_supported(num_offsets)) return WCN_ERROR_INVALID_PARAMETERS;
@@ -525,6 +567,7 @@
       sort_workspace_bytes < wcn_kmap_tally_sort_workspace(m))
     return WCN_ERROR_INVALID_PARAMETERS;
   if (binned_workspace && (!coords || binned_n != m || max_blocks < 1)) return WCN_ERROR_INVALID_PARAMETERS;
+  if (host_box && (!host_mirror || !binned_workspace)) return WCN_ERROR_INVALID_PARAMETERS;
   const int kc = tile_key_centre(num_offsets, wcn_kmap_mask_words(num_offsets));
   const SortPlan plan = sort_plan(sort_workspace, m, num_offsets < 32 ? num_offsets : 32, kc > 0);
   CellTable cells{};
@@ -532,7 +575,7 @@
   launch_tally(mask, nbr, m, num_offsets, counts, true, plan.nblk, plan.counts, coords, binned_workspace ? &cells : nullptr,
                status, kc, plan.shift0, plan.bits, s, compact != 0);
   launch_scan(counts, wcn_kmap_num_blocks(m), num_offsets, offsets, status, host_mirror, plan.nblk, plan.counts,
-              plan.totals, 1 << plan.bits, s);
+              plan.totals, 1 << plan.bits, s, host_box ? cells.ctr : nullptr, host_box ? cells.boxpart : nullptr, host_box);
   RsLaunch l[12];
   const int count = sort_launches(plan, mask, wcn_kmap_mask_words(num_offsets), m, perm, true, kc, l);
   sort_run_range(l, 0, count, s);
diff --git a/warpconvnet_amd/csrc/kmap_cells.h b/warpconvnet_amd/csrc/kmap_cells.h
--- a/warpconvnet_amd/csrc/kmap_cells.h
+++ b/warpconvnet_amd/csrc/kmap_cells.h
@@ -1,4 +1,6 @@
 #pragma once
+
+#include <limits.h>
 
 #include "wcn_common.h"
 
@@ -16,6 +18,9 @@
 constexpr int kCompactIds = kCompactPitch - 1;
 constexpr int kCompactFlag = (int)0x80000000;
 
+constexpr int kBoxCtr = 8;
+constexpr int kBoxRows = 1;
+constexpr int kBoxPartRows = 8192;
 constexpr int kIdLateBit = 1 << 30;
 
 struct __attribute__((aligned(16))) BSlot {
@@ -33,6 +38,7 @@
   int32_t* nbtab;
   int32_t* cells;
   int64_t max_blocks;
+  int32_t* boxpart;
   size_t bytes;
 };
 
@@ -88,6 +94,7 @@
   t.blk_key = (uint64_t*)take((size_t)max_blocks * 8);
   t.nbtab = (int32_t*)take((size_t)max_blocks * 32 * 4);
   t.cells = (int32_t*)take((size_t)max_blocks * kCells * 4);
+  t.boxpart = (int32_t*)take((size_t)kBoxPartRows * 8 * 4);
   t.bytes = off;
   return t;
 }
@@ -126,6 +133,51 @@
   return id < 0 ? -1 : (id & ~kIdLateBit);
 }
 
+struct BlockBox {
+  int b0, x0, y0, z0;
+  int nb, nx, ny, nz;
+};
+
+constexpr int kBlkCoordMax = (1 << (kBlkCoordBits - 1)) - 1;
+constexpr int kBlkCoordMin = -(1 << (kBlkCoordBits - 1));
+
+__host__ __device__ inline int64_t box_volume(const BlockBox& q) { return (int64_t)q.nb * q.nx * q.ny * q.nz; }
+
+__host__ __device__ inline bool box_usable(const BlockBox& q, int64_t max_blocks) {
+  if (q.nb < 1 || q.nx < 1 || q.ny < 1 || q.nz < 1) return false;
+  if (q.nb > kBatchMax + 1 || q.nx > (1 << kBlkCoordBits) || q.ny > (1 << kBlkCoordBits) || q.nz > (1 << kBlkCoordBits)) return false;
+  if (q.b0 < 0 || q.b0 + q.nb - 1 > kBatchMax) return false;
+  if (q.x0 <= kBlkCoordMin || q.y0 <= kBlkCoordMin || q.z0 <= kBlkCoordMin) return false;
+  if (q.x0 + q.nx - 1 >= kBlkCoordMax || q.y0 + q.ny - 1 >= kBlkCoordMax || q.z0 + q.nz - 1 >= kBlkCoordMax) return false;
+  return box_volume(q) <= max_blocks && box_volume(q) < (1ll << 30);
+}
+
+__host__ __device__ inline bool box_contains(const BlockBox& q, int b, int bx, int by, int bz) {
+  return (unsigned)(b - q.b0) < (unsigned)q.nb && (unsigned)(bx - q.x0) < (unsigned)q.nx && (unsigned)(by - q.y0) < (unsigned)q.ny &&
+         (unsigned)(bz - q.z0) < (unsigned)q.nz;
+}
+
+__host__ __device__ inline int box_id(const BlockBox& q, int b, int bx, int by, int bz) {
+  return (((b - q.b0) * q.nx + (bx - q.x0)) * q.ny + (by - q.y0)) * q.nz + (bz - q.z0);
+}
+__host__ __device__ inline void box_block(const BlockBox& q, int id, int& b, int& bx, int& by, int& bz) {
+  bz = q.z0 + id % q.nz; id /= q.nz;
+  by = q.y0 + id % q.ny; id /= q.ny;
+  bx = q.x0 + id % q.nx; id /= q.nx;
+  b = q.b0 + id;
+}
+__host__ __device__ inline uint64_t box_key(const BlockBox& q, int id) {
+  int b, bx, by, bz;
+  box_block(q, id, b, bx, by, bz);
+  return pack_key(b, bx, by, bz);
+}
+__host__ __device__ inline int box_neighbor(const BlockBox& q, int id, int dir) {
+  int b, bx, by, bz;
+  box_block(q, id, b, bx, by, bz);
+  bx += dir / 9 - 1; by += (dir / 3) % 3 - 1; bz += dir % 3 - 1;
+  return box_contains(q, b, bx, by, bz) ? box_id(q, b, bx, by, bz) : -1;
+}
+
 __device__ __forceinline__ int cell_index(int x, int y, int z) { return (x * kBlk + y) * kBlk + z; }
 __device__ __forceinline__ int cell_of(const int4& c) {
   return ((c.y & (kBlk - 1)) * kBlk + (c.z & (kBlk - 1))) * kBlk + (c.w & (kBlk - 1));
diff --git a/warpconvnet_amd/geometry/coords/search/torch_discrete.py b/warpconvnet_amd/geometry/coords/search/torch_discrete.py
--- a/warpconvnet_amd/geometry/coords/search/torch_discrete.py
+++ b/warpconvnet_amd/geometry/coords/search/torch_discrete.py
@@ -1,4 +1,5 @@
 import ctypes
+import dataclasses
 import os
 from typing import Literal, Optional, Sequence, Tuple
 
@@ -153,6 +154,15 @@
 _SPIN_POLLS = 4000
 
 
+@dataclasses.dataclass
+class _ClassBox:
+    bounds: tuple
+    volume: int
+    arg: object
+    last_n: int
+    occupied: Optional[int]
+
+
 class BuildHints:
 
     def __init__(self, div: int = 16, pairs_per_row: float = 12.0):
@@ -160,7 +170,58 @@
         self.pairs_per_row = float(pairs_per_row)
         self._by_volume = {}
         self._dense_volumes = set()
-        self.stats = {"builds": 0, "rebuilds": 0, "pair_rewrites": 0}
+        self.stats = {"builds": 0, "rebuilds": 0, "pair_rewrites": 0, "box_builds": 0}
+        self._boxes = {}
+
+    @staticmethod
+    def _size_class(n: int) -> int:
+        return max(int(n), 1).bit_length()
+
+    def _class_box(self, n: int, bounds, max_blocks: int, occupied):
+        lo, hi = bounds[:4], bounds[4:]
+        arg = (ctypes.c_int32 * 8)(*lo, *(h - l + 1 for l, h in zip(lo, hi)))
+        if not _lib.lib().wcn_kmap_box_usable(arg, int(max_blocks)):
+            return None
+        return _ClassBox(tuple(bounds), int(arg[4]) * int(arg[5]) * int(arg[6]) * int(arg[7]), arg, int(n), occupied)
+
+    def box(self, n: int, max_blocks: int):
+        e = self._boxes.get(self._size_class(n))
+        if e is None or e.volume > max_blocks:
+            return None
+        if e.last_n != n:
+            return None
+        if e.occupied is not None and e.volume - e.occupied > max(1024, e.occupied):
+            return None
+        return e.arg
+
+    def box_bounds(self, n: int):
+        e = self._boxes.get(self._size_class(n))
+        return e.bounds if e is not None else None
+
+    def observe_box(self, n: int, bounds, max_blocks: int, occupied: Optional[int] = None) -> None:
+        bounds = tuple(int(v) for v in bounds)
+        if any(l > h for l, h in zip(bounds[:4], bounds[4:])):
+            return
+        cls = self._size_class(n)
+        cur = self._boxes.get(cls)
+        if cur is not None and occupied is None:
+            occupied = cur.occupied
+        if cur is not None and cur.bounds == bounds:
+            cur.last_n, cur.occupied = int(n), occupied
+            return
+        new = None
+        if cur is not None:
+            union = tuple(map(min, cur.bounds[:4], bounds[:4])) + tuple(map(max, cur.bounds[4:], bounds[4:]))
+            if union == cur.bounds:
+                cur.last_n, cur.occupied = int(n), occupied
+                return
+            new = self._class_box(n, union, max_blocks, occupied)
+        if new is None:
+            new = self._class_box(n, bounds, max_blocks, occupied)
+        if new is None:
+            self._boxes.pop(cls, None)
+        else:
+            self._boxes[cls] = new
 
     def compact_rows(self, num_offsets: int) -> bool:
         return int(num_offsets) not in self._dense_volumes
@@ -281,6 +342,7 @@
     table_capacity = _next_power_of_2(max(16, 2 * N))
     compact_ok = use_binned and bool(L.wcn_kmap_compact_supported(K)) and os.environ.get("WARPCONVNET_AMD_KMAP_COMPACT", "1") != "0"
     state = {"max_blocks": hints.max_blocks(N), "strict": 0, "compact": bool(compact_ok and hints.compact_rows(K))}
+    use_box = use_binned and os.environ.get("WARPCONVNET_AMD_KMAP_BOX", "1") != "0"
     odd = all(k % 2 == 1 for k in ksize)
     cells = prebuilt = None
     if not use_binned and N > 0 and M > 0 and os.environ.get("WARPCONVNET_AMD_KMAP_METHOD", "auto").strip().lower() != "hash":
@@ -297,15 +359,18 @@
         block_counts = torch.empty(L.wcn_kmap_counts_bytes(M, K) // 4, dtype=torch.int32, device=dev)
         perm = torch.empty(M, dtype=torch.int32, device=dev)
         meta = (torch.empty if use_binned else torch.zeros)(K + 2, dtype=torch.int32, device=dev)
-        table, bin_ws = None, None
+        table, bin_ws, box = None, None, None
         stream = _lib.stream_handle(dev)
         if use_binned:
             ws_bytes = L.wcn_kmap_binned_workspace(N, max_blocks)
             bin_ws = torch.empty(ws_bytes, dtype=torch.uint8, device=dev)
+            box = hints.box(N, max_blocks) if use_box else None
+            if box is not None:
+                hints.stats["box_builds"] += 1
             _lib.check(
                 L.wcn_kmap_build_binned(_lib.ptr(in_coords), N, _lib.i3(ksize), _lib.i3(dilation), max_blocks, strict, int(compact),
                                         _lib.ptr(bin_ws), ws_bytes, _lib.ptr(nbr), _lib.ptr(mask), _lib.ptr(meta[K + 1 :]),
-                                        stream),
+                                        box, stream),
                 "wcn_kmap_build_binned",
             )
         elif prebuilt is not None:
@@ -324,7 +389,7 @@
                                  _lib.i3(stride), _lib.i3(dilation), _lib.ptr(nbr), _lib.ptr(mask), stream),
                 "wcn_kmap_probe",
             )
-        meta_host = torch.empty(K + 3, dtype=torch.int32, pin_memory=True)
+        meta_host = torch.empty(K + 3 + 9, dtype=torch.int32, pin_memory=True)
         ready = ctypes.c_int32.from_address(meta_host.data_ptr() + 4 * (K + 2))
         ready.value = 0
         sort_bytes = L.wcn_kmap_tally_sort_workspace(M)
@@ -337,13 +402,14 @@
                                   _lib.ptr(meta[K + 1 :]), ctypes.c_void_p(meta_host.data_ptr()), _lib.ptr(perm),
                                   _lib.ptr(sort_ws), sort_bytes, _lib.ptr(in_coords) if use_binned else None,
                                   _lib.ptr(bin_ws), N if use_binned else 0, max_blocks if use_binned else 0, int(compact),
-                                  _lib.ptr(spec_in), _lib.ptr(spec_out), spec_capacity, stream),
+                                  _lib.ptr(spec_in), _lib.ptr(spec_out), spec_capacity,
+                                  ctypes.c_void_p(meta_host.data_ptr() + 4 * (K + 3)) if use_box else None, stream),
             "wcn_kmap_tally_sort",
         )
         event = torch.cuda.Event()
         event.record(torch.cuda.current_stream(dev))
         return dict(nbr=nbr, mask=mask, perm=perm, block_counts=block_counts, meta=meta, meta_host=meta_host, ready=ready,
-                    event=event, table=table, keep=(bin_ws, sort_ws, cells), max_blocks=max_blocks, compact=compact,
+                    event=event, table=table, keep=(bin_ws, sort_ws, cells), max_blocks=max_blocks, compact=compact, box=box,
                     spec_pairs=(spec_in, spec_out, spec_capacity) if spec_capacity else None)
 
     def scatter(b, capacity):
@@ -368,7 +434,12 @@
             if not b["ready"].value:
                 b["event"].synchronize()
             flags = int(b["meta_host"][K + 1])
-            if use_binned and (flags & _lib.WCN_FLAG_TABLE_FULL) and state["max_blocks"] < N:
+            if use_box and not (flags & (_lib.WCN_FLAG_TABLE_FULL | _lib.WCN_FLAG_COORD_RANGE)):
+                seen = b["meta_host"][K + 3 : K + 12].tolist()
+                hints.observe_box(N, seen[:8], state["max_blocks"], occupied=seen[8] if b["box"] is None else None)
+            if b["box"] is not None and (flags & _lib.WCN_FLAG_BOX_MISS) and not (flags & _lib.WCN_FLAG_COORD_RANGE):
+                pass
+            elif use_binned and (flags & _lib.WCN_FLAG_TABLE_FULL) and state["max_blocks"] < N:
                 hints.div = 4 if hints.div > 4 else 1
                 state["max_blocks"] = max(1024, N // 4) if hints.div == 4 and state["max_blocks"] < max(1024, N // 4) else N
             elif use_binned and (flags & _lib.WCN_FLAG_ROW_OVERFLOW) and state["compact"]:
```

Measured after the change: 1110 M voxels/s, median of 6. 3.0% higher.
